# LANL-Bioinformatics/PCRamp

Hardware: AMD Instinct MI355X
Metric: primer-pair x target amplification evals/sec (higher is better)
Workload: dtype u32

## Files before the change

### pcramp_amd/csrc/pcr_device.hip

```cpp
#include <hip/hip_runtime.h>
#include <cstring>
#include <rocprim/device/device_radix_sort.hpp>

#include <stdint.h>
#include <string.h>
#include <math.h>
#include <stdlib.h>
#include <string>
#include <vector>
#include <chrono>
#include <algorithm>
#include <unordered_map>
#include <type_traits>
#include <thread>
#include <mutex>
#include <condition_variable>
#include <functional>
#include <memory>
#include <atomic>
#include <cassert>
#include <sched.h>
#include <pthread.h>

#include "../../include/pcramp_hip.h"
// ... 463 lines not shown
		for(uint32_t j = k >> 1;j > 0;j >>= 1){
			for(uint32_t i = tid;i < np2;i += FINBIG_THREADS){
				const uint32_t l = i ^ j;
				if(l > i){
					const uint64_t a = fin_keys[i], b = fin_keys[l];
					const bool up = ((i & k) == 0);
					if((a > b) == up){ fin_keys[i] = b; fin_keys[l] = a; }
				}
			}
			__syncthreads();
		}
	}
	const uint32_t chunk = (np2 + FINBIG_THREADS - 1)/FINBIG_THREADS;
	const uint32_t lo = min(np2, tid*chunk), hi = min(np2, lo + chunk);
	uint32_t cnt = 0;
	for(uint32_t i = lo;i < hi;++i){
		const uint64_t k = fin_keys[i];
		if(k != ~0ull && (i == 0 || fin_keys[i - 1] != k)) ++cnt;
	}
	part[tid] = cnt;
	__syncthreads();
	if(tid == 0){
		uint32_t run = 0;
		for(int t = 0;t < FINBIG_THREADS;++t){ const uint32_t c = part[t]; part[t] = run; run += c; }
		seg_hi[seq] = seq*cap + run;
	}
	__syncthreads();
	uint32_t rank = part[tid];
	for(uint32_t i = lo;i < hi;++i){
		const uint64_t k = fin_keys[i];
		if(k != ~0ull && (i == 0 || fin_keys[i - 1] != k)){
			DevEntry e;
			materialise_entry(k, planes, blk_off, irr, irr_off, e);
			db[(size_t)seq*cap + rank] = e;
			++rank;
		}
	}
}

#include "pcr_screen.inc"

#include "pcr_sw.inc"
#include "pcr_thermo.inc"

constexpr uint32_t N_TOUCHED_UNKNOWN = 0xFFFFFFFFu;
constexpr uint32_t EPOCH_LIMIT = (1u << 24) - 1;

struct SeqSet {
	uint32_t n = 0;
	std::vector<std::vector<uint8_t> > packed;
	std::vector<uint64_t> len, blk_off, nblk_real;
	std::vector<float> weight; DevBuf<float> d_weight; bool weight_dirty = true;
	std::vector<uint8_t> active;
	std::vector<std::vector<pcrhost::IrrEntry> > irr_host;
	uint64_t total_blocks = 0;
	uint32_t n_tiles = 0, n_irr = 0;
	bool ctrl_clean = false;
	bool touched_from_seg = false;
	uint32_t bucket_cap = 64;
	DevBuf<uint32_t> irr_perm; uint32_t irr_size_count[256];
	DevBuf<uint4> planes;
	DevBuf<uint32_t> valid, nib, tb, blk_seq, tile_seq, tile_pos0, irr_off, degen_tiles;
	uint32_t *valid_d() const { return valid.p + S2_VALID_FRONT; }
	uint32_t *tb_d() const { return tb.p + S2_TB_FRONT; }
	DevBuf<uint8_t> tile_degen; uint32_t n_degen_tiles = 0;
	DevBuf<TileDesc> tile_desc;
	DevBuf<uint64_t> d_len, d_blk_off, d_nblk_real;
	DevBuf<uint8_t> d_active;
	std::vector<uint8_t> has_eos; DevBuf<uint8_t> d_has_eos;
	DevBuf<IrrDev> irr;
	DevBuf<IrrScan> irr_scan;
	DevBuf<uint32_t> irx_first, irx_last, irx_words, irx_sums; bool irx_valid = false, irx_usable = false;
	uint32_t irr_n_multi = 0;
	DevBuf<uint32_t> pix_first, pix_last, pix_sums, blk_info, blk_local, blk_tile0; DevBuf<uint4> pix_ent; std::vector<uint32_t> pix_start_h; uint64_t pix_generation = 0; bool pix_valid = false, pix_usable = false;
	DevBuf<uint8_t> codes; DevBuf<uint64_t> d_code_off; bool have_codes = false;
	bool have_db = false;
	uint32_t n_entries = 0;
	uint32_t db_cap = 0;
	uint64_t n_slots = 0;
	DevBuf<DevEntry> db;
	DevBuf<uint32_t> touched;
	DevBuf<uint32_t> ctrl;
	uint32_t n_touched = 0;
	bool touched_built = false;
	uint32_t *d_seg_hi = nullptr;
};

}

struct HostPool {
	std::vector<std::thread> th;
	std::mutex m; std::condition_variable cv_go, cv_done;
	std::function<void(unsigned)> fn; unsigned n_parts = 0, next = 0, pending = 0; uint64_t gen = 0; bool stop = false;
	explicit HostPool(unsigned n_workers){ for(unsigned i = 0;i < n_workers;++i) th.emplace_back([this]{ work(); }); }
	~HostPool(){ { std::lock_guard<std::mutex> lk(m); stop = true; } cv_go.notify_all(); for(std::thread &t : th) t.join(); }
	unsigned size() const { return (unsigned)th.size(); }
	void work()
	{
		uint64_t seen = 0;
		std::unique_lock<std::mutex> lk(m);
		while(true){
			cv_go.wait(lk, [&]{ return stop || gen != seen; });
			if(stop) return;
			seen = gen;
			while(next < n_parts){ const unsigned p = next++; lk.unlock(); fn(p); lk.lock(); }
			if(--pending == 0) cv_done.notify_one();
		}
	}
	void run(unsigned parts, std::function<void(unsigned)> f)
	{
		std::unique_lock<std::mutex> lk(m);
		fn = std::move(f); n_parts = parts; next = 0; pending = (unsigned)th.size(); ++gen;
		cv_go.notify_all();
		while(next < n_parts){ const unsigned p = next++; lk.unlock(); fn(p); lk.lock(); }
		cv_done.wait(lk, [&]{ return pending == 0; });
	}
};

namespace { struct PassJob; struct Launcher; }

struct ItemBufs {
	DevBuf<uint8_t> *tmp; DevBuf<uint32_t> *cnt; DevBuf<uint64_t> *eoff; DevBuf<uint2> *items;
	DevBuf<uint64_t> *joff; DevBuf<float4> *res; DevBuf<uint2> *item_tm; DevBuf<uint32_t> *flag;
};
struct ItemScratch {
	DevBuf<uint8_t> in, tmp; DevBuf<uint32_t> cnt, flag; DevBuf<uint64_t> eoff, joff, ioff; DevBuf<uint2> items, item_tm; DevBuf<float4> res;
	ItemBufs bufs() { return ItemBufs{&tmp, &cnt, &eoff, &items, &joff, &res, &item_tm, &flag}; }
};

struct pcr_ctx {
	int device = 0;
	std::unique_ptr<HostPool> pool_;
	HostPool &host_pool()
	{
		if(!pool_){ const unsigned hw = std::max(1u, std::thread::hardware_concurrency()); pool_.reset(new HostPool(std::min(hw, 16u) - 1u)); }
		return *pool_;
	}
	Stream stream;
	Stream aux_stream;
	std::string design_text;
	DevBuf<uint64_t> split_where;
	pcr_params params;
	pcrhost::PackFilter filt;
	SeqSet sets[PCR_N_SETS];
	DevBuf<uint32_t> best, counters, mask, status;
	int scan_version = 3;
	bool force_seed1 = false;
	struct S2Key { uint32_t a, c, g, t, floor_; bool operator==(const S2Key &o) const { return a == o.a && c == o.c && g == o.g && t == o.t && floor_ == o.floor_; } };
	struct S2KeyHash { size_t operator()(const S2Key &k) const { uint64_t h = 0x9E3779B97F4A7C15ull; for(uint32_t v : {k.a, k.c, k.g, k.t, k.floor_}){ h ^= v; h *= 0x100000001B3ull; h ^= h >> 29; } return (size_t)h; } };
	struct S2Entry { std::vector<uint32_t> seeds;  uint32_t off_mask; bool seedable; uint4 mask;  };
	std::unordered_map<S2Key, S2Entry, S2KeyHash> s2_cache;
	std::vector<pcrhost::Seed> s2_tmp;
	static constexpr int S3_CHUNK_SETS = 4;
	struct S3Chunks { uint64_t gen = 0; uint32_t total = 0; std::vector<uint32_t> run; };
	struct S3Entry : S2Entry { std::vector<uint8_t> spans;  S3Chunks chunks[S3_CHUNK_SETS]; uint32_t next_slot = 0; };
	std::unordered_map<S2Key, S3Entry, S2KeyHash> s3_cache;
	std::vector<pcrhost::FoldSeed> s3_tmp;
	struct S3Launch { Seed3Slices W; uint32_t n_chunks, per_wg, slice_cap, n_irr_wg; };
	int pair_mode = 1; bool s3_pair_attr_set = false;
	bool no_seed3 = false, s3_attr_set = false;
	bool s3_next = true;
	bool s2_attr_set = false; uint32_t s2_dbg = 0; bool no_irr_index = false;
	std::unordered_map<S2Key, S2Entry, S2KeyHash> s1_cache;
	DevBuf<uint32_t> s1_image, s1_heads, s1_multi, s1_part;
	bool host_seed_tables = false;
	DevBuf<Hit> hits;
	DevBuf<uint64_t> bits_fr, bits_rf;
	DevBuf<OligoDev> oligos;
	DevBuf<SwJob> sw_jobs; DevBuf<SwOut> sw_out; DevBuf<uint8_t> sw_q, sw_qlen, sw_t, entry_codes, entry_lens;
	DevBuf<AmpRec> amp_recs, amp_recs2; DevBuf<BgPairDev> bg_pairs;
	DevBuf<uint64_t> amp_keys; DevBuf<uint32_t> amp_pkeys, amp_pair_start; DevBuf<uint8_t> sort_tmp;
	DevBuf<thermo::Job> th_jobs; DevBuf<thermo::JobOut> th_out; DevBuf<int> th_dg; DevBuf<uint2> th_map; DevBuf<uint32_t> th_bad;
	float th_dg_salt = -1.0f;
	DevBuf<unsigned long long> th_dbg; bool th_attr_set = false;
	std::vector<thermo::Job> th_host_jobs; std::vector<thermo::JobOut> th_host_res;
	MappedBuf<uint8_t> sw_pin; Event sw_done[2];
	DevBuf<pcr_amplicon> mx_amp;
	DevBuf<OligoDev> opt_oligos; DevBuf<uint2> opt_jobs; DevBuf<float> opt_cov; DevBuf<uint32_t> opt_loc, opt_tasks;
	DevBuf<Planes> mx_keys; uint32_t mx_n_keys = 0; DevBuf<uint32_t> mx_count;
	DevBuf<uint8_t> pool_in, pool_tmp; DevBuf<uint32_t> pool_cnt, pool_ord; DevBuf<uint64_t> pool_eoff, pool_ioff, pool_keys; DevBuf<uint2> pool_items; DevBuf<pcr_product> pool_rec;
	DevBuf<uint8_t> site_in, site_tmp; DevBuf<uint32_t> site_cnt, site_ord, site_flag; DevBuf<uint64_t> site_eoff, site_joff, site_keys; DevBuf<uint2> site_items; DevBuf<float4> site_res; DevBuf<pcr_site> site_rec;
	bool site_attr_set = false;
	DevBuf<uint8_t> sv_item; DevBuf<uint32_t> sv_ord, sv_var, sv_start, sv_vord, sv_map; DevBuf<pcr_site_variant> sv_rec; DevBuf<uint64_t> sv_vkeys;
	bool sv_attr_set = false;
	DevBuf<uint4> rp_foot; DevBuf<uint64_t> rp_keys; DevBuf<uint32_t> rp_u32; DevBuf<uint8_t> rp_state; DevBuf<pcr_repair_step> rp_rec;
	pcr_comm *shard_comm = nullptr; uint64_t shard_first = 0, shard_n_total = 0; int shard_mode = 0;
	DevBuf<uint64_t> sh_rec, sh_full; DevBuf<uint8_t> sh_stage;
	std::vector<uint64_t> shard_bounds; DevBuf<uint64_t> d_shard_bounds;
	bool design_ready = false; DevBuf<uint64_t> sh_bits;
	std::vector<std::vector<uint8_t> > samp_packed; std::vector<uint64_t> samp_len;
	void drop_shard(){ shard_comm = nullptr; shard_mode = 0; shard_bounds.clear(); design_ready = false; samp_packed.clear(); samp_len.clear(); }
	pcr_comm *trial_comm = nullptr;
	size_t amp_cap = size_t(1) << 20;
	uint32_t n_cu = 256;
	DevBuf<uint64_t> fin_scratch;
	std::vector<uint16_t> seed_count; std::vector<uint8_t> seed_fill, seed_own;
	uint32_t epoch = 0;
	uint32_t debug_epoch = 0;
	bool opt_pm_global = false;
	uint32_t opt_dbg_wg_tasks = 0, opt_dbg_task_cap = 0;
	uint64_t best_seen = 0;
	static constexpr int STAGE_RING = 4;
	struct StageSlot { MappedBuf<uint8_t> buf; Event done; bool busy = false;
	                   uint32_t guard_seq = 0;  };
	StageSlot stage[STAGE_RING]; int stage_next = 0;
	struct DirectSlot { DevBuf<uint8_t> buf{true}; uint32_t guard_seq = 0; };
	DirectSlot dstage[STAGE_RING]; int dstage_next = 0;
	bool direct_ok = false;
	typedef PassMail Mail;
	static constexpr uint32_t MAIL_RING = 8;
	MappedBuf<Mail> mail;
	uint32_t mail_seq = 0;
	MappedBuf<uint8_t> ret;
	MappedBuf<uint8_t> in;
	MappedBuf<uint32_t> ret_flag; uint32_t ret_seq = 0;
	struct Pending {
		uint32_t seq; int which; std::vector<pcr_pair> pairs; int opt5, opt3; float thr; uint32_t min_len;
		pcr_amplify_args args; uint64_t *d_fr, *d_rf;
	};
	std::vector<Pending> pending;
	bool launch_thread = true;
	Launcher *launcher = nullptr; pcrq::Client lq_client; uint64_t n_pipelined = 0;
	std::mutex job_m; std::vector<PassJob *> job_free, job_all;
	DevBuf<uint8_t> arena;
	const uint4 *d_cand_fwd = nullptr, *d_cand_rc = nullptr; const uint32_t *d_cand_floor = nullptr;
	const OligoDev *d_oligos = nullptr;
	bool debug_log = false;
	bool timing = false; double t_host[8] = {0, 0, 0, 0, 0, 0, 0, 0}; uint64_t n_timed = 0;
	bool prof = false; uint32_t prof_stride = 1, prof_pass = 0;
	std::vector<std::pair<Event, Event> > prof_events;
	double prof_ms = 0.0; uint64_t prof_launches = 0;
	std::vector<std::pair<Event, Event> > prof_events_k[PCR_PROF_KERNELS];
	double prof_ms_k[PCR_PROF_KERNELS] = {0.0, 0.0, 0.0}; uint64_t prof_launches_k[PCR_PROF_KERNELS] = {0, 0, 0};
	DevBuf<uint8_t> pdim_in, pdim_tmp; DevBuf<float4> pdim_res; DevBuf<pcr_pool_dimer> pdim_rec, pdim_out; DevBuf<uint32_t> pdim_keep, pdim_off, pdim_flag;
	bool pdim_attr_set = false;
	DevBuf<uint32_t> ptm_ord; DevBuf<uint64_t> ptm_keys, ptm_bits; DevBuf<pcr_product_tm> ptm_rec;
	DevBuf<uint32_t> pph_hcnt, pph_ord; DevBuf<uint64_t> pph_hoff, pph_keys, pph_bits; DevBuf<uint4> pph_prod; DevBuf<pcr_probe_hit> pph_rec;
	DevBuf<uint4> pam_iv, pam_stat; DevBuf<uint32_t> pam_u32; DevBuf<uint64_t> pam_u64; DevBuf<pcr_amplicon_info> pam_info; DevBuf<uint8_t> pam_tmp, pam_packed;
	uint32_t bg_max_pairs = 0;
	uint32_t amp_dbg_hash_bits = 0;
	DevBuf<uint4> ppc_iv; DevBuf<uint32_t> ppc_pos, ppc_u32; DevBuf<uint64_t> ppc_u64; DevBuf<pcr_probe_candidate> ppc_rec; DevBuf<uint8_t> ppc_tmp;
	DevBuf<uint32_t> anp_pairseq; DevBuf<uint64_t> anp_out; DevBuf<float> anp_melt;
	DevBuf<uint8_t> pcf_din; DevBuf<uint32_t> pcf_vals, pcf_ucell, pcf_dkeep, pcf_keep, pcf_koff;
	DevBuf<uint64_t> pcf_aoff, pcf_keys; DevBuf<float4> pcf_dres;
	DevBuf<uint4> pcf_uagg, pcf_dense; DevBuf<pcr_pool_dimer> pcf_drec; DevBuf<float> pcf_dmat; DevBuf<pcr_pool_conflict> pcf_rec, pcf_out;
	ItemScratch shared;
	DevBuf<uint2> pe3_end; DevBuf<uint32_t> pe3_before, pe3_ord; DevBuf<uint64_t> pe3_sum, pe3_keys, pe3_bits; DevBuf<uint8_t> pe3_tmp;
	DevBuf<pcr_product_end3> pe3_rec;
};

namespace {

int drain(pcr_ctx *ctx);
int flush_launcher(pcr_ctx *ctx);
void detach_launcher(pcr_ctx *ctx);
void free_jobs(pcr_ctx *ctx);

struct ProfScope {
	pcr_ctx *ctx; int k; Event e0, e1;
	ProfScope(pcr_ctx *c, int kernel, bool on = true) : ctx(c), k(kernel)
	{
		if(!on || !ctx->prof || k < 0 || k >= PCR_PROF_KERNELS) return;
		if(e0.create() != hipSuccess || e1.create() != hipSuccess){ e0.release(); return; }
		(void)hipEventRecord(e0, ctx->stream);
	}
	void finish()
	{
		if(!e0) return;
		(void)hipEventRecord(e1, ctx->stream);
		((k == PCR_PROF_SCAN) ? ctx->prof_events : ctx->prof_events_k[k]).emplace_back(std::move(e0), std::move(e1));
	}
	~ProfScope() { finish(); }
};
constexpr int PCR_SET_SCRATCH = 3;
inline bool set_ok(pcr_set which) { return (unsigned)which <= (unsigned)PCR_SET_MULTIPLEX; }
#define CHECK_SET(which) do{ if(!set_ok(which)){ g_err = "unknown sequence set (PCR_SET_TARGET, PCR_SET_BACKGROUND or PCR_SET_MULTIPLEX)"; return PCR_ERR_ARG; } }while(0)
#define FLUSH(ctx) do{ if((ctx)->launcher){ const int frc_ = flush_launcher(ctx); if(frc_ != PCR_OK) return frc_; } }while(0)
#define DRAIN(ctx) do{ FLUSH(ctx); if(!(ctx)->pending.empty()){ const int drc_ = drain(ctx); if(drc_ != PCR_OK) return drc_; } }while(0)

struct HostTimer {
	pcr_ctx *ctx; int slot; std::chrono::steady_clock::time_point t0;
	HostTimer(pcr_ctx *c, int s) : ctx(c), slot(s) { if(ctx->timing) t0 = std::chrono::steady_clock::now(); }
	void next(int s)
	{
		if(!ctx->timing) return;
		const auto t1 = std::chrono::steady_clock::now();
		ctx->t_host[slot] += std::chrono::duration<double, std::micro>(t1 - t0).count();
		slot = s; t0 = t1;
	}
	~HostTimer() { next(slot); }
};

__global__ void k_apply_splits(const uint64_t *__restrict__ where, uint32_t n, uint32_t *__restrict__ planes , uint32_t *__restrict__ nib)
{
	const uint32_t i = blockIdx.x*blockDim.x + threadIdx.x;
	if(i >= n) return;
	const uint64_t gb = where[2*(size_t)i];
	const uint32_t bit = (uint32_t)where[2*(size_t)i + 1];
	const uint32_t m = ~(1u << bit);
	for(int k = 0;k < 4;++k) atomicAnd(&planes[gb*4 + k], m);
	atomicAnd(&nib[gb*4 + (bit >> 3)], ~(0xFu << ((bit & 7u)*4u)));
}

int upload_irregular(pcr_ctx *ctx, SeqSet &S)
{
	const auto tu0 = std::chrono::steady_clock::now();
	auto ms_since = [&](){ return std::chrono::duration<double, std::milli>(std::chrono::steady_clock::now() - tu0).count(); };
	double t_flat = 0, t_sort = 0, t_scan = 0, t_copy1 = 0;
	size_t total = 0;
	for(uint32_t s = 0;s < S.n;++s) total += S.irr_host[s].size();
	std::vector<IrrDev> flat(total);
	std::vector<uint32_t> off(S.n + 1, 0);
	for(int k = 0;k < 256;++k) S.irr_size_count[k] = 0;
	{
		size_t at = 0;
		for(uint32_t s = 0;s < S.n;++s){
			off[s] = (uint32_t)at;
			const std::vector<pcrhost::IrrEntry> &v = S.irr_host[s];
			for(size_t k = 0;k < v.size();++k){
				const pcrhost::IrrEntry &e = v[k];
				IrrDev &d = flat[at++];
				d.w = e.w; d.loc = e.loc; d.seq = s;
				d.meta = (uint32_t)e.strand | ((uint32_t)e.cws << 8) | ((uint32_t)e.ord << 16);
				d.local_id = (uint32_t)k;
				++S.irr_size_count[e.cws & 0xFF];
			}
		}
	}
	off[S.n] = (uint32_t)flat.size();
	S.n_irr = (uint32_t)flat.size();
	t_flat = ms_since();
	std::vector<uint32_t> perm(flat.size());
	t_sort = ms_since();
	int rc;
	{
		auto spread = [](uint64_t v) -> uint64_t {
			v = (v | (v << 16)) & 0x0000FFFF0000FFFFull; v = (v | (v << 8)) & 0x00FF00FF00FF00FFull; v = (v | (v << 4)) & 0x0F0F0F0F0F0F0F0Full;
			v = (v | (v << 2)) & 0x3333333333333333ull; v = (v | (v << 1)) & 0x5555555555555555ull; return v;
		};
		uint32_t start[256];
		uint32_t run = 0;
		for(int k = 255;k >= 0;--k){ start[k] = run; run += S.irr_size_count[k]; }
		std::vector<IrrScan> scan(perm.size());
		uint32_t n_multi = 0;
		for(size_t i = 0;i < flat.size();++i){
			const IrrDev &d = flat[i];
			const uint32_t at = start[(d.meta >> 8) & 0xFF]++;
			perm[at] = (uint32_t)i;
			const uint32_t multi = (d.w.a & d.w.c) | (d.w.a & d.w.g) | (d.w.a & d.w.t) | (d.w.c & d.w.g) | (d.w.c & d.w.t) | (d.w.g & d.w.t);
			if(multi) ++n_multi;
			const uint32_t lo = d.w.c | d.w.t, hi = d.w.g | d.w.t;
			const uint64_t code = spread(lo) | (spread(hi) << 1);
			IrrScan r; r.w0 = (uint32_t)code; r.w1 = (uint32_t)(code >> 32); r.idx_flags = (uint32_t)i | (multi ? 0x80000000u : 0u); r.seq = d.seq;
			scan[at] = r;
		}
		S.irr_n_multi = n_multi; S.irx_valid = false;
		t_scan = ms_since();
		if((rc = S.irr_scan.ensure_slack(scan.size() + 1)) != PCR_OK) return rc;
		if(!scan.empty()) HIP_TRY(hipMemcpy(S.irr_scan.p, scan.data(), scan.size()*sizeof(IrrScan), hipMemcpyHostToDevice));
	}
	t_copy1 = ms_since();
	if((rc = S.irr_perm.ensure_slack(perm.size() + 1)) != PCR_OK) return rc;
	if(!perm.empty()) HIP_TRY(hipMemcpyAsync(S.irr_perm.p, perm.data(), perm.size()*sizeof(uint32_t), hipMemcpyHostToDevice, ctx->stream));
	if((rc = S.irr.ensure_slack(flat.size())) != PCR_OK) return rc;
	if((rc = S.irr_off.ensure(off.size())) != PCR_OK) return rc;
	if(!flat.empty()) HIP_TRY(hipMemcpyAsync(S.irr.p, flat.data(), flat.size()*sizeof(IrrDev), hipMemcpyHostToDevice, ctx->stream));
	HIP_TRY(hipMemcpyAsync(S.irr_off.p, off.data(), off.size()*sizeof(uint32_t), hipMemcpyHostToDevice, ctx->stream));
	HIP_TRY(hipStreamSynchronize(ctx->stream));
	if(ctx->timing && flat.size() > 100000) fprintf(stderr, "[pcramp] irregular list of %zu words: flat %.1f  order %.1f  scan records %.1f  first copy %.1f  other copies %.1f ms\n", flat.size(), t_flat, t_sort - t_flat, t_scan - t_sort, t_copy1 - t_scan, ms_since() - t_copy1);
	return PCR_OK;
}

void launch_exclusive_scan(pcr_ctx *ctx, uint32_t *counts, uint32_t *starts, uint32_t n, uint32_t *sums)
{
	const uint32_t n_blocks = (n + 4095u)/4096u;
	hipLaunchKernelGGL(k_scan_blocks, dim3(n_blocks), dim3(1024), 0, ctx->stream, counts, starts, n, sums);
	hipLaunchKernelGGL(k_scan_sums, dim3(1), dim3(1024), 0, ctx->stream, sums, n_blocks);
	hipLaunchKernelGGL(k_scan_add, dim3(n_blocks), dim3(1024), 0, ctx->stream, starts, counts, n, sums);
}

constexpr uint32_t IRX_MAX_RUN = 1024;
int ensure_irr_index(pcr_ctx *ctx, SeqSet &S)
{
	if(S.irx_valid) return PCR_OK;
	int rc;
	if((rc = S.irx_first.ensure(IRX_KEYS + 4)) != PCR_OK) return rc;
	if((rc = S.irx_last.ensure(IRX_KEYS + 4)) != PCR_OK) return rc;
	if((rc = S.irx_words.ensure_slack((size_t)24*S.n_irr + 4)) != PCR_OK) return rc;
	const uint32_t n_blocks = (IRX_KEYS + 4095u)/4096u;
	if((rc = S.irx_sums.ensure(n_blocks + 4)) != PCR_OK) return rc;
	HIP_TRY(hipMemsetAsync(S.irx_last.p, 0, (size_t)IRX_KEYS*sizeof(uint32_t), ctx->stream));
	if(S.n_irr){
		hipLaunchKernelGGL(k_irx_count, dim3((S.n_irr + 255)/256), dim3(256), 0, ctx->stream, S.irr.p, S.n_irr, S.irx_last.p);
		HIP_TRY(hipGetLastError());
	}
	{
		uint32_t longest = 0;
		HIP_TRY(hipMemsetAsync(S.irx_sums.p + n_blocks, 0, sizeof(uint32_t), ctx->stream));
		hipLaunchKernelGGL(k_irx_max, dim3(256), dim3(256), 0, ctx->stream, S.irx_last.p, IRX_KEYS, S.irx_sums.p + n_blocks);
		HIP_TRY(hipMemcpyAsync(&longest, S.irx_sums.p + n_blocks, sizeof(uint32_t), hipMemcpyDeviceToHost, ctx->stream));
		HIP_TRY(hipStreamSynchronize(ctx->stream));
		S.irx_usable = longest <= IRX_MAX_RUN;
		if(!S.irx_usable){ S.irx_valid = true; return PCR_OK; }
	}
	launch_exclusive_scan(ctx, S.irx_last.p, S.irx_first.p, IRX_KEYS, S.irx_sums.p);
	HIP_TRY(hipGetLastError());
	if(S.n_irr){
		hipLaunchKernelGGL(k_irx_scatter, dim3((S.n_irr + 255)/256), dim3(256), 0, ctx->stream, S.irr.p, S.n_irr, S.irx_last.p, S.irx_words.p);
		HIP_TRY(hipGetLastError());
	}
	S.irx_valid = true;
	return PCR_OK;
}

int ensure_pos_index(pcr_ctx *ctx, SeqSet &S)
{
	if(S.pix_valid) return PCR_OK;
	S.pix_valid = true; S.pix_usable = false;
	if(S.total_blocks == 0 || S.total_blocks*32 >= (uint64_t(1) << 32) - 64) return PCR_OK;
	int rc;
	if((rc = S.pix_first.ensure(PIX_KEYS + 4)) != PCR_OK) return rc;
	if((rc = S.pix_last.ensure(PIX_KEYS + 4)) != PCR_OK) return rc;
	const uint32_t n_blocks = (PIX_KEYS + 4095u)/4096u;
	if((rc = S.pix_sums.ensure(n_blocks + 4)) != PCR_OK) return rc;
	if((rc = S.pix_ent.ensure(S.total_blocks*32 + 64)) != PCR_OK) return rc;
	{
		if(S.n >= (1u << 30)){ return PCR_OK; }
		if((rc = S.blk_info.ensure(S.total_blocks + 1)) != PCR_OK) return rc;
		if((rc = S.blk_local.ensure(S.total_blocks + 1)) != PCR_OK) return rc;
		std::vector<uint32_t> tile0((size_t)S.n + 1);
		uint64_t t0 = 0;
		for(uint32_t q = 0;q < S.n;++q){ tile0[q] = (uint32_t)t0; t0 += (S.len[q] >= 32) ? (S.len[q] - 7 + TILE_POS - 1)/TILE_POS : 0; }
		tile0[S.n] = (uint32_t)t0;
		if(t0 >= (uint64_t(1) << 32)) return PCR_OK;
		if((rc = S.blk_tile0.ensure((size_t)S.n + 1)) != PCR_OK) return rc;
		HIP_TRY(hipMemcpyAsync(S.blk_tile0.p, tile0.data(), ((size_t)S.n + 1)*sizeof(uint32_t), hipMemcpyHostToDevice, ctx->stream));
		hipLaunchKernelGGL(k_blk_info, dim3((unsigned)((S.total_blocks + 255)/256)), dim3(256), 0, ctx->stream, S.blk_seq.p, S.d_blk_off.p, S.d_len.p,
			S.blk_tile0.p, S.tile_degen.p, S.d_active.p, S.total_blocks, S.blk_info.p, S.blk_local.p);
		HIP_TRY(hipGetLastError());
		HIP_TRY(hipStreamSynchronize(ctx->stream));
	}
	HIP_TRY(hipMemsetAsync(S.pix_last.p, 0, (size_t)PIX_KEYS*sizeof(uint32_t), ctx->stream));
	const unsigned grid = (unsigned)((S.total_blocks + 255)/256);
// ... 255 lines not shown
	HIP_TRY(hipMemcpyAsync(&n, S.ctrl.p + 3, sizeof(uint32_t), hipMemcpyDeviceToHost, ctx->stream));
	HIP_TRY(hipStreamSynchronize(ctx->stream));
	S.n_touched = n; S.n_entries = n ? 1 : 0; S.touched_built = true;
	return PCR_OK;
}

int amplify_launch(pcr_ctx *ctx, SeqSet &S, const pcr_pair *pairs, uint32_t n_pairs, const pcr_amplify_args *a,
	uint64_t *d_fr, uint64_t *d_rf, const FusedAmp *fa = nullptr)
{
	{ const int erc = ensure_touched(ctx, S); if(erc != PCR_OK) return erc; }
	if(!S.have_db){ g_err = "pcr_amplify: no word DB (call pcr_select_words first)"; return PCR_ERR_STATE; }
	const uint64_t words = (S.n + 63)/64;
	const size_t bits_bytes = (size_t)n_pairs*words*sizeof(uint64_t);
	if(S.n_entries == 0 || n_pairs == 0){
		if(bits_bytes){
			HIP_TRY(hipMemsetAsync(d_fr, 0, bits_bytes, ctx->stream));
			HIP_TRY(hipMemsetAsync(d_rf, 0, bits_bytes, ctx->stream));
		}
		return PCR_OK;
	}
	HostTimer timer(ctx, 4);
	int rc;
	const bool prestaged = fa && fa->staged;
	if(prestaged) ctx->d_oligos = fa->d_oligos;
	else{
		std::vector<OligoDev> ol;
		build_oligos(pairs, n_pairs, a, ol);
		Stager st(ctx);
		if((rc = st.begin(ol.size()*sizeof(OligoDev) + 64)) != PCR_OK) return rc;
		ctx->d_oligos = st.put(ol.data(), ol.size());
		const bool vec_ok = ((uintptr_t)d_fr % 16 == 0) && ((uintptr_t)d_rf % 16 == 0) && (bits_bytes % 16 == 0);
		if(!vec_ok){
			HIP_TRY(hipMemsetAsync(d_fr, 0, bits_bytes, ctx->stream));
			HIP_TRY(hipMemsetAsync(d_rf, 0, bits_bytes, ctx->stream));
		}
		if((rc = vec_ok ? st.ship(d_fr, bits_bytes, d_rf, bits_bytes) : st.ship()) != PCR_OK) return rc;
	}
	timer.next(5);
	const uint32_t mask_words = (2*n_pairs + 31)/32;
	if((rc = ctx->mask.ensure((size_t)S.n_slots*mask_words)) != PCR_OK) return rc;
	if((rc = ctx->status.ensure(1)) != PCR_OK) return rc;
	const bool dev_n = S.n_touched == N_TOUCHED_UNKNOWN;
	const uint32_t *n_dev = dev_n ? S.ctrl.p + 3 : nullptr;
	const uint32_t n_t = dev_n ? 0u : S.n_touched, n_db = n_t*S.db_cap;
	const unsigned threads = dev_n ? 256 : 128;
	const unsigned grid = dev_n ? (unsigned)std::min<uint64_t>(((uint64_t)S.n*S.db_cap + threads - 1)/threads, 1024) : (n_db + threads - 1)/threads;
	const unsigned mgrid = dev_n ? std::min<unsigned>((S.n + MATCH_WAVES - 1)/MATCH_WAVES, 1024u) : (n_t + MATCH_WAVES - 1)/MATCH_WAVES;
	hipLaunchKernelGGL(k_match, dim3(std::max(mgrid, 1u)), dim3(64*MATCH_WAVES), 0, ctx->stream, S.db.p, n_t, n_dev, S.db_cap,
		S.touched.p, S.d_seg_hi, ctx->d_oligos, 2*n_pairs, mask_words, ctx->mask.p, ctx->status.p,
		prestaged ? fa->pub_counters : (const uint32_t *)nullptr, prestaged ? ctx->mail.dev + (fa->pub_seq % pcr_ctx::MAIL_RING) : (pcr_ctx::Mail *)nullptr,
		prestaged ? fa->pub_seq : 0u);
	HIP_TRY(hipGetLastError());
	hipLaunchKernelGGL(k_pair, dim3(grid), dim3(threads), 0, ctx->stream, S.db.p, n_db, n_dev, S.db_cap, S.touched.p, S.d_seg_hi, ctx->mask.p,
		mask_words, ctx->d_oligos, n_pairs, S.planes.p, S.d_blk_off.p, S.d_len.p, S.d_active.p, a->amp_min, a->amp_max,
		a->ident_threshold, a->use_taq_mama, d_fr, d_rf, words, ctx->status.p);
	HIP_TRY(hipGetLastError());
	return PCR_OK;
}

template<int NSLOT, int KLO>
int launch_scan2_nw(pcr_ctx *ctx, SeqSet &S, uint32_t nw, uint32_t group0, uint32_t n_groups, uint32_t gw, uint32_t ncand, const HitSink &sink,
	const uint32_t *d_tab, const uint32_t *d_bias, const uint32_t *tile_ids, uint32_t n_tiles, const uint32_t *orient_ids)
{
#define SCAN2_ARGS S.nib.p, S.planes.p, S.valid_d(), S.d_blk_off.p, S.d_len.p, S.d_active.p, S.tile_seq.p, S.tile_pos0.p, \
	d_tab, d_bias, group0, gw, tile_ids, orient_ids, ctx->d_cand_fwd, ctx->d_cand_rc, ctx->d_cand_floor, ncand, sink
	const dim3 grid(n_tiles, n_groups), block(SCAN2_THREADS);
	switch(nw){
		case 1: hipLaunchKernelGGL((k_scan2<1, NSLOT, KLO>), grid, block, 0, ctx->stream, SCAN2_ARGS); break;
		case 2: hipLaunchKernelGGL((k_scan2<2, NSLOT, KLO>), grid, block, 0, ctx->stream, SCAN2_ARGS); break;
		case 3: hipLaunchKernelGGL((k_scan2<3, NSLOT, KLO>), grid, block, 0, ctx->stream, SCAN2_ARGS); break;
		case 4: hipLaunchKernelGGL((k_scan2<4, NSLOT, KLO>), grid, block, 0, ctx->stream, SCAN2_ARGS); break;
		case 5: hipLaunchKernelGGL((k_scan2<5, NSLOT, KLO>), grid, block, 0, ctx->stream, SCAN2_ARGS); break;
		case 6: hipLaunchKernelGGL((k_scan2<6, NSLOT, KLO>), grid, block, 0, ctx->stream, SCAN2_ARGS); break;
		case 7: hipLaunchKernelGGL((k_scan2<7, NSLOT, KLO>), grid, block, 0, ctx->stream, SCAN2_ARGS); break;
		default: hipLaunchKernelGGL((k_scan2<8, NSLOT, KLO>), grid, block, 0, ctx->stream, SCAN2_ARGS); break;
	}
#undef SCAN2_ARGS
	HIP_TRY(hipGetLastError());
	return PCR_OK;
}

int launch_scan2(pcr_ctx *ctx, SeqSet &S, const Scan2Tables &T, uint32_t ncand, const HitSink &sink,
	const uint32_t *d_tab, const uint32_t *d_bias, const uint32_t *tile_ids, uint32_t n_tiles, const uint32_t *orient_ids)
{
	if(n_tiles == 0 || T.n_groups == 0) return PCR_OK;
	const uint32_t full = (T.last_words == T.gw) ? T.n_groups : T.n_groups - 1;
	int rc = PCR_OK;
	if(full){
		rc = (T.nslot == 26) ? launch_scan2_nw<26, 3>(ctx, S, T.gw, 0, full, T.gw, ncand, sink, d_tab, d_bias, tile_ids, n_tiles, orient_ids)
			: launch_scan2_nw<32, 0>(ctx, S, T.gw, 0, full, T.gw, ncand, sink, d_tab, d_bias, tile_ids, n_tiles, orient_ids);
		if(rc != PCR_OK) return rc;
	}
	if(full < T.n_groups){
		rc = (T.nslot == 26) ? launch_scan2_nw<26, 3>(ctx, S, T.last_words, full, 1, T.gw, ncand, sink, d_tab, d_bias, tile_ids, n_tiles, orient_ids)
			: launch_scan2_nw<32, 0>(ctx, S, T.last_words, full, 1, T.gw, ncand, sink, d_tab, d_bias, tile_ids, n_tiles, orient_ids);
	}
	return rc;
}

int count_entries(pcr_ctx *ctx, SeqSet &S)
{
	uint64_t total = 0;
	if(S.n_touched){
		std::vector<uint32_t> hi(S.n);
		HIP_TRY(hipMemcpyAsync(hi.data(), S.d_seg_hi, S.n*sizeof(uint32_t), hipMemcpyDeviceToHost, ctx->stream));
		HIP_TRY(hipStreamSynchronize(ctx->stream));
		for(uint32_t q = 0;q < S.n;++q){ if(hi[q]) total += hi[q] - (uint64_t)q*S.db_cap; }
	}
	S.n_entries = (uint32_t)total;
	return PCR_OK;
}

}

extern "C" {

const char *pcr_last_error(void) { return g_err.c_str(); }

pcr_ctx *pcr_create(int device, void *hip_stream, const pcr_params *params)
{
	int count = 0;
	if(hipGetDeviceCount(&count) != hipSuccess || count <= 0){
		g_err = "pcr_create: no HIP device available (this library has no CPU fallback)";
		return nullptr;
	}
	if(device < 0 || device >= count){ g_err = "pcr_create: bad device index"; return nullptr; }
	if(hipSetDevice(device) != hipSuccess){ g_err = "pcr_create: hipSetDevice failed"; return nullptr; }
	hipDeviceProp_t prop;
	if(hipGetDeviceProperties(&prop, device) != hipSuccess){ g_err = "pcr_create: hipGetDeviceProperties failed"; return nullptr; }
	if(std::string(prop.gcnArchName).find("gfx950") == std::string::npos){
		g_err = std::string("pcr_create: device is ") + prop.gcnArchName + ", this build targets gfx950 only";
		return nullptr;
	}
	pcr_ctx *ctx = new pcr_ctx();
	ctx->device = device;
	if(hip_stream) ctx->stream.borrow((hipStream_t)hip_stream);
	else if(ctx->stream.create() != hipSuccess){ g_err = "pcr_create: hipStreamCreate failed"; delete ctx; return nullptr; }
	if(params){ ctx->params = *params; }
	else{ ctx->params.pack_max_degen = 256; ctx->params.pack_min_gc = 0.0f; ctx->params.pack_max_gc = 1.0f; }
	{ hipDeviceProp_t prop; if(hipGetDeviceProperties(&prop, device) == hipSuccess && prop.multiProcessorCount > 0) ctx->n_cu = (uint32_t)prop.multiProcessorCount; }
	if(const char *v = getenv("PCRAMP_TIMING")) ctx->timing = v[0] == '1';
	ctx->debug_log = getenv("PCRAMP_DEBUG") != nullptr;
	if(const char *v = getenv("PCRAMP_DEBUG_EPOCH")) ctx->debug_epoch = (uint32_t)strtoul(v, nullptr, 0);
	if(const char *v = getenv("PCRAMP_OPT_PM")) ctx->opt_pm_global = v[0] == 'g';
	if(const char *v = getenv("PCRAMP_DEBUG_OPT_TASKS")){ unsigned a = 0, b = 0; if(sscanf(v, "%u,%u", &a, &b) >= 1){ ctx->opt_dbg_wg_tasks = a; ctx->opt_dbg_task_cap = b; } }
	if(const char *v = getenv("PCRAMP_DEBUG_AMP_HASH_BITS")) ctx->amp_dbg_hash_bits = (uint32_t)strtoul(v, nullptr, 0);
	if(const char *v = getenv("PCRAMP_DEBUG_AMP_CAP")) ctx->amp_cap = std::max<size_t>(16, (size_t)strtoull(v, nullptr, 0));
	if(const char *v = getenv("PCRAMP_SEED")) ctx->force_seed1 = v[0] == '1';
	if(const char *v = getenv("PCRAMP_SEED_TABLES")) ctx->host_seed_tables = v[0] == 'h';
	if(const char *v = getenv("PCRAMP_S2DBG")) ctx->s2_dbg = (uint32_t)atoi(v);
	if(const char *v = getenv("PCRAMP_IRR_INDEX")) ctx->no_irr_index = v[0] == '0';
	if(const char *v = getenv("PCRAMP_SEED3")) ctx->no_seed3 = v[0] == '0';
	if(const char *v = getenv("PCRAMP_S3_NEXT")) ctx->s3_next = v[0] != '0';
	if(const char *v = getenv("PCRAMP_LAUNCH_THREAD")) ctx->launch_thread = v[0] != '0';
	if(const char *v = getenv("PCRAMP_PAIR")) ctx->pair_mode = (v[0] == '0') ? 0 : (strcmp(v, "force") == 0) ? 2 : 1;
	if(const char *v = getenv("PCRAMP_SCAN")){ if(v[0] == '1') ctx->scan_version = 1; else if(v[0] == '2') ctx->scan_version = 2; }
	{
		const char *v = getenv("PCRAMP_STAGE");
		if(!(v && v[0] == 'k') && prop.isLargeBar){
			DevBuf<uint32_t> probe(true); MappedBuf<uint32_t> back; const std::string err_before = g_err;
			constexpr uint32_t PROBE_WORDS = 1024;
			if(probe.ensure(PROBE_WORDS) == PCR_OK && back.ensure(PROBE_WORDS*sizeof(uint32_t)) == PCR_OK){
				hipPointerAttribute_t at;
				bool ok = hipPointerGetAttributes(&at, probe.p) == hipSuccess;
				for(int round = 0;ok && round < 2;++round){
					volatile uint32_t *w = (volatile uint32_t *)probe.p;
					for(uint32_t i = 0;i < PROBE_WORDS;++i){ w[i] = 0x9E3779B9u*(i + 1) + (uint32_t)round; back.host[i] = 0; }
					__builtin_ia32_sfence();
					hipLaunchKernelGGL(k_stage, dim3(1), dim3(256), 0, ctx->stream, (const uint4 *)probe.p, (uint4 *)back.dev, PROBE_WORDS/4,
						(uint4 *)nullptr, 0u, (uint4 *)nullptr, 0u, (uint4 *)nullptr, 0u);
					ok = hipGetLastError() == hipSuccess && hipStreamSynchronize(ctx->stream) == hipSuccess;
					for(uint32_t i = 0;ok && i < PROBE_WORDS;++i) ok = back.host[i] == 0x9E3779B9u*(i + 1) + (uint32_t)round;
				}
				ctx->direct_ok = ok;
			}
			else{ (void)hipGetLastError(); g_err = err_before; }
		}
	}
	ctx->filt.max_degen = ctx->params.pack_max_degen;
	ctx->filt.set_gc(ctx->params.pack_min_gc, ctx->params.pack_max_gc);
	if(hipMemcpyToSymbol(HIP_SYMBOL(c_taq_mama), h_taq_mama, sizeof(h_taq_mama)) != hipSuccess ||
	   hipMemcpyToSymbol(HIP_SYMBOL(thermo::c_H), PCR_NN_H, sizeof(PCR_NN_H)) != hipSuccess ||
	   hipMemcpyToSymbol(HIP_SYMBOL(thermo::c_S), PCR_NN_S, sizeof(PCR_NN_S)) != hipSuccess ||
	   hipMemcpyToSymbol(HIP_SYMBOL(thermo::c_loop_S), PCR_LOOP_S, sizeof(PCR_LOOP_S)) != hipSuccess ||
	   hipMemcpyToSymbol(HIP_SYMBOL(thermo::c_bulge_S), PCR_BULGE_S, sizeof(PCR_BULGE_S)) != hipSuccess ||
	   hipMemcpyToSymbol(HIP_SYMBOL(thermo::c_hairpin_S), PCR_HAIRPIN_S, sizeof(PCR_HAIRPIN_S)) != hipSuccess ||
	   hipMemcpyToSymbol(HIP_SYMBOL(thermo::c_special_H), PCR_SPECIAL_H, sizeof(PCR_SPECIAL_H)) != hipSuccess ||
	   hipMemcpyToSymbol(HIP_SYMBOL(thermo::c_special_S), PCR_SPECIAL_S, sizeof(PCR_SPECIAL_S)) != hipSuccess ||
	   hipMemcpyToSymbol(HIP_SYMBOL(thermo::c_special_key), PCR_SPECIAL_KEY, sizeof(PCR_SPECIAL_KEY)) != hipSuccess ||
	   hipMemcpyToSymbol(HIP_SYMBOL(thermo::c_wc), PCR_WC, sizeof(PCR_WC)) != hipSuccess){
		g_err = "pcr_create: hipMemcpyToSymbol failed"; delete ctx; return nullptr;
	}
	if(ctx->mail.ensure(sizeof(pcr_ctx::Mail)*pcr_ctx::MAIL_RING) != PCR_OK){ g_err = "pcr_create: mapped host allocation failed"; delete ctx; return nullptr; }
	memset((void *)ctx->mail.host, 0, sizeof(pcr_ctx::Mail)*pcr_ctx::MAIL_RING);
	return ctx;
}

void pcr_destroy(pcr_ctx *ctx)
{
	if(!ctx) return;
	(void)hipSetDevice(ctx->device);
	(void)flush_launcher(ctx);
	detach_launcher(ctx);
	(void)hipStreamSynchronize(ctx->stream);
	if(ctx->aux_stream) (void)hipStreamSynchronize(ctx->aux_stream);
	ctx->pending.clear();
	free_jobs(ctx);
	if(ctx->timing && ctx->n_timed){
		const double n = (double)ctx->n_timed;
		fprintf(stderr, "[pcramp] host us/pass by stage: A (plan, caller's thread) %.1f  B (stage + launch, %s) %.1f  (%llu of %llu passes pipelined, queue depth <= %u)\n",
			ctx->t_host[0]/n, ctx->n_pipelined ? "launcher thread" : "caller's thread", (ctx->t_host[1] + ctx->t_host[2])/n,
			(unsigned long long)ctx->n_pipelined, (unsigned long long)ctx->n_timed, ctx->lq_client.max_depth);
		fprintf(stderr, "[pcramp] host us/pass: plan %.1f  stage %.1f  launch %.1f  wait %.1f | amplify prep %.1f  launch %.1f  (%llu passes)\n",
			ctx->t_host[0]/n, ctx->t_host[1]/n, ctx->t_host[2]/n, ctx->t_host[3]/n, ctx->t_host[4]/n, ctx->t_host[5]/n, (unsigned long long)ctx->n_timed);
	}
	delete ctx;
}

uint32_t pcr_num_sequences(pcr_ctx *ctx, pcr_set which) { return (ctx && set_ok(which)) ? ctx->sets[which].n : 0; }
uint64_t pcr_bitset_words(pcr_ctx *ctx, pcr_set which) { return (ctx && set_ok(which)) ? (ctx->sets[which].n + 63)/64 : 0; }

int pcr_staging_mode(pcr_ctx *ctx) { return (ctx && ctx->direct_ok) ? 1 : 0; }

int pcr_launcher_stats(pcr_ctx *ctx, uint64_t *passes_pipelined, uint32_t *max_queue_depth)
{
	if(!ctx){ g_err = "null ctx"; return PCR_ERR_ARG; }
	if(passes_pipelined) *passes_pipelined = ctx->n_pipelined;
	if(max_queue_depth) *max_queue_depth = ctx->lq_client.max_depth;
	return PCR_OK;
}

int pcr_live_resources(uint64_t out[4])
{
	if(!out){ g_err = "pcr_live_resources: bad argument"; return PCR_ERR_ARG; }
	for(int k = 0;k < 4;++k) out[k] = pcrown::g_live[k].load();
	return PCR_OK;
}

int pcr_synchronize(pcr_ctx *ctx)
{
	if(!ctx){ g_err = "null ctx"; return PCR_ERR_ARG; }
	HIP_TRY(hipSetDevice(ctx->device));
	DRAIN(ctx);
	HIP_TRY(hipStreamSynchronize(ctx->stream));
	return PCR_OK;
}

static int load_sequences_impl(pcr_ctx *ctx, int which, const uint8_t *packed4, const uint64_t *byte_offsets,
	const uint64_t *lengths, const float *weights, uint32_t n);

int pcr_load_sequences(pcr_ctx *ctx, pcr_set which, const uint8_t *packed4, const uint64_t *byte_offsets,
	const uint64_t *lengths, const float *weights, uint32_t n)
{
	if(!set_ok(which)){ g_err = "pcr_load_sequences: unknown sequence set"; return PCR_ERR_ARG; }
	return load_sequences_impl(ctx, (int)which, packed4, byte_offsets, lengths, weights, n);
}

static int load_sequences_impl(pcr_ctx *ctx, int which, const uint8_t *packed4, const uint64_t *byte_offsets,
	const uint64_t *lengths, const float *weights, uint32_t n)
{
	if(!ctx || which < 0 || which >= PCR_N_SETS || (n && (!packed4 || !byte_offsets || !lengths))){
		g_err = "pcr_load_sequences: bad argument"; return PCR_ERR_ARG;
	}
	DRAIN(ctx);
	if(n >= (1u << 24)){ g_err = "pcr_load_sequences: at most 2^24-1 sequences per GPU shard"; return PCR_ERR_CAPACITY; }
	HIP_TRY(hipSetDevice(ctx->device));
	HIP_TRY(hipStreamSynchronize(ctx->stream));
	SeqSet &S = ctx->sets[which];
	S.have_db = false; S.n_entries = 0; S.have_codes = false;
	S.n = n;
	S.packed.assign(n, std::vector<uint8_t>());
	S.len.assign(lengths, lengths + n);
	if(which == PCR_SET_TARGET) ctx->drop_shard();
	if(which == PCR_SET_TARGET || which == PCR_SET_BACKGROUND) ctx->trial_comm = nullptr;
	S.weight.assign(n, 1.0f);
	if(weights) S.weight.assign(weights, weights + n);
	S.weight_dirty = true;
	S.ctrl_clean = false; S.touched_from_seg = false;
	S.active.assign(n, 1);
	S.has_eos.assign(n, 0);
	S.blk_off.assign(n + 1, 0);
	S.nblk_real.assign(n, 0);
	S.irr_host.assign(n, std::vector<pcrhost::IrrEntry>());
	uint64_t total_bytes = 0, total_blocks = 0, n_tiles = 0;
	std::vector<uint64_t> dev_byte_off(n);
	for(uint32_t s = 0;s < n;++s){
		if(lengths[s] >= (uint64_t(1) << 31)){ g_err = "pcr_load_sequences: sequence longer than 2^31-1 bases"; return PCR_ERR_CAPACITY; }
		const uint64_t nb = (lengths[s] + 1)/2;
		S.packed[s].assign(packed4 + byte_offsets[s], packed4 + byte_offsets[s] + nb);
		if((lengths[s] & 1) && nb) S.packed[s][nb - 1] &= 0xF0;
		{
			const std::vector<uint8_t> &b = S.packed[s];
			bool eos = false;
			const uint64_t full = lengths[s]/2;
			for(uint64_t k = 0;k < full && !eos;++k) eos = ((b[k] & 0xF0) == 0) || ((b[k] & 0x0F) == 0);
			if(!eos && (lengths[s] & 1)) eos = ((b[full] & 0xF0) == 0);
			S.has_eos[s] = eos ? 1 : 0;
		}
		dev_byte_off[s] = total_bytes;
		total_bytes += nb;
		S.blk_off[s] = total_blocks;
		S.nblk_real[s] = (lengths[s] + 31)/32;
		total_blocks += S.nblk_real[s] + 2;
		if(lengths[s] >= 32) n_tiles += (lengths[s] - 7 + TILE_POS - 1)/TILE_POS;
	}
	S.blk_off[n] = total_blocks;
	S.total_blocks = total_blocks;
	if(n_tiles >= (uint64_t(1) << 31)){ g_err = "pcr_load_sequences: too many tiles"; return PCR_ERR_CAPACITY; }
	S.n_tiles = (uint32_t)n_tiles;

	std::vector<uint32_t> blk_seq(total_blocks), tile_seq(n_tiles), tile_pos0(n_tiles);
	uint64_t t = 0;
	S.pix_valid = false; S.pix_usable = false;
	for(uint32_t s = 0;s < n;++s){
		for(uint64_t b = S.blk_off[s];b < S.blk_off[s + 1];++b) blk_seq[b] = s;
		if(lengths[s] >= 32){
			const uint64_t nt = (lengths[s] - 7 + TILE_POS - 1)/TILE_POS;
			for(uint64_t k = 0;k < nt;++k, ++t){ tile_seq[t] = s; tile_pos0[t] = (uint32_t)(k*TILE_POS); }
		}
		pcrhost::PackedSeq q; q.buf = S.packed[s].data(); q.len = lengths[s];
		if(!pcrhost::irregular_words(q, ctx->filt, S.irr_host[s])){
			g_err = "pcr_load_sequences: more than 64 irregular words share one (loc, strand)"; return PCR_ERR_CAPACITY;
		}
	}

	int rc;
	DevBuf<uint8_t> d_packed; DevBuf<uint64_t> d_byte_off;
	if((rc = d_packed.ensure(total_bytes)) != PCR_OK) return rc;
	if((rc = d_byte_off.ensure(n)) != PCR_OK) return rc;
	if((rc = S.planes.ensure(total_blocks)) != PCR_OK) return rc;
	if((rc = S.valid.ensure(S2_VALID_FRONT + total_blocks + S2_TAIL_BLOCKS)) != PCR_OK) return rc;
	if((rc = S.nib.ensure(total_blocks*4 + 8)) != PCR_OK) return rc;
	if((rc = S.tb.ensure(S2_TB_FRONT + (total_blocks + S2_TAIL_BLOCKS)*2 + 8)) != PCR_OK) return rc;
	if((rc = S.tile_degen.ensure(n_tiles + 1)) != PCR_OK) return rc;
	if((rc = S.degen_tiles.ensure(n_tiles + 1)) != PCR_OK) return rc;
	if((rc = S.blk_seq.ensure(total_blocks)) != PCR_OK) return rc;
	if((rc = S.tile_seq.ensure(n_tiles)) != PCR_OK) return rc;
	if((rc = S.tile_pos0.ensure(n_tiles)) != PCR_OK) return rc;
	if((rc = S.d_len.ensure(n)) != PCR_OK) return rc;
	if((rc = S.d_blk_off.ensure(n + 1)) != PCR_OK) return rc;
	if((rc = S.d_nblk_real.ensure(n)) != PCR_OK) return rc;
	if((rc = S.d_active.ensure(n)) != PCR_OK) return rc;
	if((rc = S.d_has_eos.ensure(n)) != PCR_OK) return rc;
#define H2D(dst, src, bytes) do{ if((bytes) > 0){ hipError_t e_ = hipMemcpy(dst, src, bytes, hipMemcpyHostToDevice); \
	if(e_ != hipSuccess){ g_err = std::string("hipMemcpy: ") + hipGetErrorString(e_); return PCR_ERR_DEVICE; } } }while(0)
	{
		std::vector<uint8_t> flat(total_bytes);
		for(uint32_t s = 0;s < n;++s){ if(!S.packed[s].empty()) memcpy(flat.data() + dev_byte_off[s], S.packed[s].data(), S.packed[s].size()); }
		H2D(d_packed.p, flat.data(), flat.size());
	}
	H2D(d_byte_off.p, dev_byte_off.data(), n*sizeof(uint64_t));
	H2D(S.blk_seq.p, blk_seq.data(), total_blocks*sizeof(uint32_t));
	H2D(S.tile_seq.p, tile_seq.data(), n_tiles*sizeof(uint32_t));
	H2D(S.tile_pos0.p, tile_pos0.data(), n_tiles*sizeof(uint32_t));
	H2D(S.d_len.p, S.len.data(), n*sizeof(uint64_t));
	H2D(S.d_blk_off.p, S.blk_off.data(), (n + 1)*sizeof(uint64_t));
	H2D(S.d_nblk_real.p, S.nblk_real.data(), n*sizeof(uint64_t));
	H2D(S.d_active.p, S.active.data(), n);
	H2D(S.d_has_eos.p, S.has_eos.data(), n);
#undef H2D
	{
		hipError_t e_ = hipMemsetAsync(S.valid.p, 0, S2_VALID_FRONT*sizeof(uint32_t), ctx->stream);
		if(e_ == hipSuccess) e_ = hipMemsetAsync(S.valid_d() + total_blocks, 0, S2_TAIL_BLOCKS*sizeof(uint32_t), ctx->stream);
		if(e_ == hipSuccess) e_ = hipMemsetAsync(S.tb.p, 0, S2_TB_FRONT*sizeof(uint32_t), ctx->stream);
		if(e_ == hipSuccess) e_ = hipMemsetAsync(S.tb_d() + total_blocks*2, 0, (S2_TAIL_BLOCKS*2 + 8)*sizeof(uint32_t), ctx->stream);
		if(e_ != hipSuccess){ g_err = std::string("load: padding memset: ") + hipGetErrorString(e_); return PCR_ERR_DEVICE; }
	}
// ... 444 lines not shown
```

### pcramp_amd/csrc/pcr_host.hpp

```cpp
#ifndef PCR_HOST_HPP
#define PCR_HOST_HPP

#include <stdint.h>
#include <algorithm>
#include <deque>
#include <vector>

namespace pcrhost {

struct Planes {
	uint32_t a, c, g, t;
};

inline uint32_t bitrev32(uint32_t v)
{
	v = ((v >> 1) & 0x55555555u) | ((v & 0x55555555u) << 1);
	v = ((v >> 2) & 0x33333333u) | ((v & 0x33333333u) << 2);
	v = ((v >> 4) & 0x0F0F0F0Fu) | ((v & 0x0F0F0F0Fu) << 4);
	v = ((v >> 8) & 0x00FF00FFu) | ((v & 0x00FF00FFu) << 8);
	return (v >> 16) | (v << 16);
}

inline unsigned word_get(const uint64_t w[2], int k) { return (unsigned)(w[k >> 4] >> ((15 - (k & 15))*4)) & 0xF; }

// ... 524 lines not shown
	}
};

inline bool orientation_seeds(const Planes &m, uint32_t floor_, uint32_t orient, std::vector<Seed> &out, int *max_exact_pos = nullptr, int Q = SEED_Q)
{
	if(max_exact_pos) *max_exact_pos = -1;
	const uint32_t occ = m.a | m.c | m.g | m.t;
	const int size = __builtin_popcount(occ);
	if(size == 0 || floor_ == 0 || floor_ > (uint32_t)size) return floor_ > (uint32_t)size;
	const int k = size - (int)floor_;
	const int first = __builtin_ctz(occ);
	if((occ >> first) != ((size == 32) ? 0xFFFFFFFFu : ((1u << size) - 1u))) return false;
	unsigned slot_set[32];
	for(int j = 0;j < first;++j) slot_set[j] = 0;
	for(int j = first;j < first + size;++j) slot_set[j] = planes_nibble(m, j);
	for(int j = first + size;j < 32;++j) slot_set[j] = 0;

	auto window = [&](int pos, int len, unsigned *sets) -> int {
		const int ws = std::min(pos, 32 - Q);
		for(int j = 0;j < Q;++j){ const int sl = ws + j; sets[j] = (sl >= pos && sl < pos + len) ? slot_set[sl] : 15u; }
		return ws;
	};
	SeedLayout best = { 0, 0, 0, 0 }; bool have = false; unsigned best_codes = 0;
	for(int n2 = 0;3*(n2 - 1) < k + 1;++n2){
		for(int n1 = 0;3*n2 + 2*(n1 - 1) < k + 1;++n1){
			const int n0 = std::max(0, k + 1 - 3*n2 - 2*n1);
			if(n0 + n1 + n2 == 0) continue;
			for(int n1s = 0;n1s <= n1;++n1s){
				const int rest = size - Q*(n1 - n1s) - (Q - 1)*n1s - Q*n2;
				if(rest < 0 || (n0 > 0 && rest/n0 < MIN_SEED_BLOCK)) continue;
				const SeedLayout lay = { n0, n1, n1s, n2 };
				unsigned codes = 0;
				lay.each(first, size, Q, [&](int pos, int len, int budget){
					unsigned sets[SEED_Q_MAX];
					window(pos, len, sets);
					if(codes <= MAX_SEED_CODES) codes += seed_block_codes(sets, Q, budget);
				});
				if(codes > MAX_SEED_CODES) continue;
				if(!have || codes < best_codes){ have = true; best = lay; best_codes = codes; }
			}
		}
	}
	if(!have) return false;
	best.each(first, size, Q, [&](int pos, int len, int budget){
		unsigned sets[SEED_Q_MAX];
		const int ws = window(pos, len, sets);
		seed_emit_block(sets, Q, orient, (uint32_t)ws, budget, out);
		if(len < Q && max_exact_pos) *max_exact_pos = std::max(*max_exact_pos, pos);
	});
	return true;
}

struct FoldSeed { uint32_t code; uint8_t off, lo, hi; };

inline unsigned seed_block_fold_cost(const unsigned *sets, int budget, unsigned &n_seeds)
{
	unsigned d[9], n[3] = { 1, 0, 0 };
	for(int j = 0;j < 9;++j){ d[j] = (unsigned)__builtin_popcount(sets[j]); n[0] *= d[j]; }
	if(n[0] == 0 || sets[9] == 0){ n_seeds = 0; return 0; }
	if(budget >= 1){
		for(int j = 0;j < 9;++j){
			if(d[j] == 4) continue;
			const unsigned cj = n[0]/d[j]*(4 - d[j]);
			n[1] += cj;
			if(budget >= 2){ for(int i = j + 1;i < 9;++i){ if(d[i] < 4) n[2] += cj/d[i]*(4 - d[i]); } }
		}
	}
	const unsigned last = sets[9];
	const unsigned span = (unsigned)(32 - __builtin_clz(last)) - (unsigned)__builtin_ctz(last);
	unsigned cost = 0; n_seeds = 0;
	for(int m = 0;m <= budget;++m){ n_seeds += n[m]; cost += n[m]*((m < budget && last != 15u) ? 4u : span); }
	return cost;
}

inline void fold_seeds(const std::vector<Seed> &q10, std::vector<FoldSeed> &out)
{
	std::vector<uint32_t> key(q10.size());
	for(size_t i = 0;i < q10.size();++i) key[i] = ((uint32_t)q10[i].off << 20) | ((q10[i].code & 0x3FFFFu) << 2) | (q10[i].code >> 18);
	std::sort(key.begin(), key.end());
	for(size_t i = 0;i < key.size();){
		unsigned set = 0; size_t j = i;
		for(;j < key.size() && (key[j] >> 2) == (key[i] >> 2);++j) set |= 1u << (key[j] & 3u);
		FoldSeed f; f.code = (key[i] >> 2) & 0x3FFFFu; f.off = (uint8_t)(key[i] >> 20);
		f.lo = (uint8_t)__builtin_ctz(set); f.hi = (uint8_t)(31 - __builtin_clz(set));
		out.push_back(f);
		i = j;
	}
}

inline bool orientation_fold_seeds(const Planes &m, uint32_t floor_, std::vector<FoldSeed> &out, std::vector<Seed> &tmp, unsigned *cost4 = nullptr)
{
	const int Q = 10;
	if(cost4) *cost4 = 0;
	const uint32_t occ = m.a | m.c | m.g | m.t;
	const int size = __builtin_popcount(occ);
	if(size == 0 || floor_ == 0 || floor_ > (uint32_t)size) return floor_ > (uint32_t)size;
	const int k = size - (int)floor_, first = __builtin_ctz(occ);
	if(size < Q || (occ >> first) != ((size == 32) ? 0xFFFFFFFFu : ((1u << size) - 1u))) return false;
	unsigned slot_set[32];
	for(int j = 0;j < 32;++j) slot_set[j] = (j >= first && j < first + size) ? planes_nibble(m, j) : 0u;
	auto window = [&](int pos, int len, unsigned *sets) -> int {
		const int ws = std::min(pos, 32 - Q);
		for(int j = 0;j < Q;++j){ const int sl = ws + j; sets[j] = (sl >= pos && sl < pos + len) ? slot_set[sl] : 15u; }
		return ws;
	};
	SeedLayout best = { 0, 0, 0, 0 }; bool have = false; unsigned best_cost = 0;
	for(int n2 = 0;3*(n2 - 1) < k + 1;++n2){
		for(int n1 = 0;3*n2 + 2*(n1 - 1) < k + 1;++n1){
			const int n0 = std::max(0, k + 1 - 3*n2 - 2*n1);
			if(n0 + n1 + n2 == 0) continue;
			for(int n1s = 0;n1s <= n1;++n1s){
				const int rest = size - Q*(n1 - n1s) - (Q - 1)*n1s - Q*n2;
				if(rest < 0 || (n0 > 0 && rest/n0 < MIN_SEED_BLOCK)) continue;
				const SeedLayout lay = { n0, n1, n1s, n2 };
				unsigned seeds = 0, cost = 0;
				lay.each(first, size, Q, [&](int pos, int len, int budget){
					unsigned sets[SEED_Q_MAX], ns = 0;
					window(pos, len, sets);
					if(seeds <= MAX_SEED_CODES){ cost += seed_block_fold_cost(sets, budget, ns); seeds += ns; }
				});
				if(seeds > MAX_SEED_CODES) continue;
				if(!have || cost < best_cost){ have = true; best = lay; best_cost = cost; }
			}
		}
	}
	if(!have) return false;
	tmp.clear();
	best.each(first, size, Q, [&](int pos, int len, int budget){
		unsigned sets[SEED_Q_MAX];
		const int ws = window(pos, len, sets);
		seed_emit_block(sets, Q, 0, (uint32_t)ws, budget, tmp);
	});
	fold_seeds(tmp, out);
	if(cost4) *cost4 = best_cost;
	return true;
}

inline bool orientation_index_seeds(const Planes &m, uint32_t floor_, bool fold, std::vector<FoldSeed> &out, std::vector<Seed> &tmp, unsigned *cost4 = nullptr)
{
	tmp.clear();
	if(!orientation_seeds(m, floor_, 0, tmp, nullptr, 9)) return false;
	const size_t at = out.size();
	const unsigned plain_cost = 4u*(unsigned)tmp.size();
	for(const Seed &sd : tmp){ FoldSeed f; f.code = sd.code; f.off = sd.off; f.lo = 0; f.hi = 3; out.push_back(f); }
	if(cost4) *cost4 = plain_cost;
	if(!fold || tmp.empty()) return true;
	std::vector<FoldSeed> folded; unsigned c4 = 0;
	if(orientation_fold_seeds(m, floor_, folded, tmp, &c4) && c4 < plain_cost){
		out.resize(at);
		out.insert(out.end(), folded.begin(), folded.end());
		if(cost4) *cost4 = c4;
	}
	return true;
}

inline bool move_trials(const Planes &cur, int move, double max_degen, int primer_min, int primer_max, std::vector<Planes> &out)
{
	const int first = planes_start(cur), last = planes_stop(cur), len = planes_size(cur);
	auto with_nibble = [](Planes w, int k, unsigned v){
		const uint32_t bit = 1u << k;
		w.a = (w.a & ~bit) | ((v & 1u) ? bit : 0u); w.c = (w.c & ~bit) | ((v & 2u) ? bit : 0u);
		w.g = (w.g & ~bit) | ((v & 4u) ? bit : 0u); w.t = (w.t & ~bit) | ((v & 8u) ? bit : 0u);
		return w;
	};
	switch(move){
		case 0:
			if(planes_degeneracy(cur) >= max_degen) return true;
			for(int i = first;i <= last;++i){
				const unsigned c = planes_nibble(cur, i);
				for(unsigned b = 1;b <= 8;b <<= 1){
					if(c & b) continue;
					const Planes w = with_nibble(cur, i, c | b);
					if(planes_degeneracy(w) > max_degen) continue;
					out.push_back(w);
				}
			}
			return true;
		case 1:
			for(int i = first;i <= last;++i){
				const unsigned c = planes_nibble(cur, i);
				for(unsigned b = 1;b <= 8;b <<= 1){
					const unsigned d = c & ~b;
					if(!d || d == c) continue;
					out.push_back(with_nibble(cur, i, d));
				}
			}
			return true;
		case 2: if(len != primer_min){ out.push_back(first < 32 ? with_nibble(cur, first, 0) : cur); } return true;
		case 3: if(len != primer_min){ out.push_back(last >= 0 ? with_nibble(cur, last, 0) : cur); } return true;
		case 4:
			if(len == primer_max) return true;
			for(unsigned b = 1;b <= 8;b <<= 1) out.push_back(first - 1 >= 0 && first < 32 ? with_nibble(cur, first - 1, b) : cur);
			return true;
		case 5:
			if(len == primer_max) return true;
			for(unsigned b = 1;b <= 8;b <<= 1) out.push_back(last + 1 < 32 ? with_nibble(cur, last + 1, b) : cur);
			return true;
		default: return false;
	}
}

}
#endif
```

### pcramp_amd/csrc/pcr_scan_seed3.inc

```

constexpr uint32_t PIX_CODES = 1u << 18;
constexpr uint32_t PIX_KEYS = PIX_CODES << 2;
constexpr uint32_t S3_BATCH = 8;

template<bool SCATTER>
__global__ void k_pix_build(const uint32_t *__restrict__ tb, const uint32_t *__restrict__ blk_seq, const uint64_t *__restrict__ blk_off,
	const uint64_t *__restrict__ len, uint64_t total_blocks, uint32_t *__restrict__ count_or_cursor, uint4 *__restrict__ ent)
{
	const uint64_t b = (uint64_t)blockIdx.x*blockDim.x + threadIdx.x;
	if(b >= total_blocks) return;
	const uint32_t seq = blk_seq[b];
	const int64_t p0 = (int64_t)(b - blk_off[seq])*32, L = (int64_t)len[seq];
	uint32_t w[8];
#pragma unroll
	for(int k = 0;k < 8;++k) w[k] = tb[(int64_t)2*(int64_t)b - 2 + k];
#pragma unroll
	for(int i = 0;i < 32;++i){
		if(p0 + i + 9 > L) break;
		const uint32_t ten = (i < 16) ? funnel(w[2], w[3], 2*i) : funnel(w[3], w[4], 2*(i - 16));
		const uint32_t code = ((ten & S2_CODE_MASK) << 2) | ((ten >> 18) & 3u);
		if(SCATTER){
			const uint32_t at = atomicAdd(&count_or_cursor[code], 1u);
			const int jl = (i + 9) >> 4, sl = 2*((i + 9) & 15);
			const int jr = (i + 41) >> 4, sr = 2*((i + 41) & 15);
			const uint32_t l_lo = funnel(w[jl], w[jl + 1], sl), l_hi = funnel(w[jl + 1], w[jl + 2], sl) & 0x3FFFu;
			const uint32_t r_lo = funnel(w[jr], w[jr + 1], sr), r_hi = funnel(w[jr + 1], w[jr + 2], sr) & 0x3FFFu;
			ent[at] = make_uint4((uint32_t)(b*32 + (uint64_t)i), l_lo, l_hi | (r_lo << 14), (r_lo >> 18) | (r_hi << 14));
		}
		else atomicAdd(&count_or_cursor[code], 1u);
	}
}

struct Seed3Tables {
	const uint32_t *seeds;
	const uint32_t *chunk_prefix;
	const uint8_t *spans;
	const uint4 *masks; const uint8_t *floors;
	uint32_t n_seeds, n_or, or_base;
	const uint32_t *pix_first, *pix_last; const uint4 *pix_ent;
	uint32_t n_chunks, per_wg, slice_cap;
	uint32_t n_irr_wg;
};
constexpr uint32_t S3_MAX_WG = 512;
constexpr uint32_t S3_MAX_OR = 448, S3_MAX_SEEDS = 1u << 16;
struct Seed3Slices { uint32_t start[S3_MAX_WG + 1]; };
struct Seed3Set {
	const uint32_t *valid, *blk_info, *blk_local; const uint8_t *active;
};
constexpr uint32_t BLK_SEQ_MASK = 0x3FFFFFFFu, BLK_INACTIVE = 0x40000000u, BLK_DEGEN = 0x80000000u;

__global__ void k_blk_info(const uint32_t *__restrict__ blk_seq, const uint64_t *__restrict__ blk_off, const uint64_t *__restrict__ len,
	const uint32_t *__restrict__ tile0, const uint8_t *__restrict__ tile_degen, const uint8_t *__restrict__ active, uint64_t total_blocks,
	uint32_t *__restrict__ blk_info, uint32_t *__restrict__ blk_local)
{
	const uint64_t b = (uint64_t)blockIdx.x*blockDim.x + threadIdx.x;
	if(b >= total_blocks) return;
	const uint32_t q = blk_seq[b];
	const uint64_t bl = b - blk_off[q], tile = bl >> 5;
	const uint32_t nt = tile0[q + 1] - tile0[q];
	const bool degen = tile < nt && tile_degen[tile0[q] + tile];
	blk_info[b] = q | (degen ? 0x80000000u : 0u) | (active[q] ? 0u : 0x40000000u);
	blk_local[b] = (uint32_t)bl;
}

__global__ void k_blk_active(uint32_t *__restrict__ blk_info, const uint32_t *__restrict__ blk_seq, const uint8_t *__restrict__ active, uint64_t total_blocks)
{
	const uint64_t b = (uint64_t)blockIdx.x*blockDim.x + threadIdx.x;
	if(b >= total_blocks) return;
	const uint32_t v = blk_info[b] & ~BLK_INACTIVE;
	blk_info[b] = v | (active[blk_seq[b]] ? 0u : BLK_INACTIVE);
}

__device__ __forceinline__ void s3_irregular(const Seed3Tables &T3, const Seed3Set &Q, const IrrArgs2 &IA, const uint4 *__restrict__ cand_fwd,
	const uint32_t *__restrict__ cand_floor, HitSink sink, uint32_t gw, uint32_t n_gw, uint32_t lane)
{
	for(uint32_t i0 = gw*16u;i0 < T3.n_seeds;i0 += n_gw*16u){
		const uint32_t i = i0 + lane;
		const uint32_t sdv = (lane < 16u && i < T3.n_seeds) ? T3.seeds[i] : S2_END;
		const uint32_t orient = T3.or_base + (sdv & 0x1FFu);
		uint32_t first = 0, cnt = 0;
		if(sdv != S2_END && !(orient & 1u)){
			const uint32_t key = (((sdv >> 9) & 31u) << 18) | (sdv >> 14);
			first = IA.ix_first[key]; cnt = IA.ix_last[key] - first;
		}
		const uint32_t incl = s2_scan(cnt);
		const uint32_t total = s2_rl(incl, 63);
		for(uint32_t t0 = 0;t0 < total;t0 += 64u){
			const uint32_t t = t0 + lane;
			uint32_t lo = 0;
#pragma unroll
			for(uint32_t stp = 32u;stp;stp >>= 1){ if((uint32_t)__shfl((int)incl, (int)(lo + stp - 1u)) <= t) lo += stp; }
			const int sl = (int)min(lo, 63u);
			const uint32_t s_incl = (uint32_t)__shfl((int)incl, sl), s_cnt = (uint32_t)__shfl((int)cnt, sl), s_first = (uint32_t)__shfl((int)first, sl);
			const uint32_t c = (uint32_t)__shfl((int)orient, sl) >> 1;
			if(t >= total) continue;
			const IrrDev e = IA.irr[IA.ix_words[s_first + (t - (s_incl - s_cnt))]];
			if(((e.meta >> 8) & 0xFFu) < IA.min_cws || !Q.active[e.seq]) continue;
			const uint32_t n = match_count(e.w.a, e.w.c, e.w.g, e.w.t, cand_fwd[c]);
			if(n >= cand_floor[c]) record_hit(sink, e.seq, c, make_key(e.seq, e.loc, e.meta & 0xFF, 1, (e.meta >> 16) & 0xFF), n);
		}
	}
}

template<uint32_t S3_THREADS>
__global__ __launch_bounds__(S3_THREADS) __attribute__((amdgpu_waves_per_eu(8, 8))) void k_seed3(Seed3Tables T3, Seed3Set Q, IrrArgs2 IA, const uint4 *__restrict__ cand_fwd, const uint32_t *__restrict__ cand_floor,
	HitSink sink, S2Clear Z, Seed3Slices W)
{
#include "pcr_scan_seed3_pass.inc"
}

struct Seed3Row {
	Seed3Tables T3; Seed3Set Q; IrrArgs2 IA; const uint4 *cand_fwd; const uint32_t *cand_floor; HitSink sink; S2Clear Z;
};
struct Seed3HalfSlices { uint32_t start[S3_MAX_WG/2 + 1]; };
template<uint32_t S3_THREADS>
__global__ __launch_bounds__(S3_THREADS) __attribute__((amdgpu_waves_per_eu(8, 8))) void k_seed3_pair(Seed3Row A, Seed3HalfSlices WA, Seed3Row B, Seed3HalfSlices WB)
{
	if(blockIdx.y == 0){
		const Seed3Tables &T3 = A.T3; const Seed3Set &Q = A.Q; const IrrArgs2 &IA = A.IA; const uint4 *const cand_fwd = A.cand_fwd; const uint32_t *const cand_floor = A.cand_floor;
		const HitSink &sink = A.sink; const S2Clear &Z = A.Z; const Seed3HalfSlices &W = WA;
#include "pcr_scan_seed3_pass.inc"
	}
	else{
		const Seed3Tables &T3 = B.T3; const Seed3Set &Q = B.Q; const IrrArgs2 &IA = B.IA; const uint4 *const cand_fwd = B.cand_fwd; const uint32_t *const cand_floor = B.cand_floor;
		const HitSink &sink = B.sink; const S2Clear &Z = B.Z; const Seed3HalfSlices &W = WB;
#include "pcr_scan_seed3_pass.inc"
	}
}
```

### pcramp_amd/csrc/pcr_scan_seed3_pass.inc

```
	extern __shared__ uint4 s3_dyn[];
	uint4 *const masks = s3_dyn;
	uint32_t *const prefix = (uint32_t *)(masks + T3.n_or);
	uint32_t *const seeds = prefix + T3.slice_cap;
	uint8_t *const floors = (uint8_t *)(seeds + T3.slice_cap);
	uint8_t *const spans = floors + ((T3.n_or + 15u) & ~15u);
	const uint32_t wave = (uint32_t)__builtin_amdgcn_readfirstlane((int)(threadIdx.x >> 6)), lane = threadIdx.x & 63u;
	for(uint32_t i = blockIdx.x*S3_THREADS + threadIdx.x;i < Z.n0;i += gridDim.x*S3_THREADS) Z.z0[i] = make_uint4(0, 0, 0, 0);
	for(uint32_t i = blockIdx.x*S3_THREADS + threadIdx.x;i < Z.n1;i += gridDim.x*S3_THREADS) Z.z1[i] = make_uint4(0, 0, 0, 0);
	if(Z.ctrl && blockIdx.x == 0 && threadIdx.x == 0){ Z.ctrl[1] = 0; Z.ctrl[3] = 0; }
	for(uint32_t i = threadIdx.x;i < T3.n_or;i += S3_THREADS){ masks[i] = T3.masks[i]; floors[i] = T3.floors[i]; }
	constexpr uint32_t S3_WAVES = S3_THREADS/64;
	if(blockIdx.x < T3.n_irr_wg){
		if(IA.ix_first) s3_irregular(T3, Q, IA, cand_fwd, cand_floor, sink, blockIdx.x*S3_WAVES + wave, T3.n_irr_wg*S3_WAVES, lane);
		return;
	}
	const uint32_t wg = blockIdx.x - T3.n_irr_wg, n_wg = gridDim.x - T3.n_irr_wg;
	const uint32_t s_lo = W.start[wg];
	const uint32_t n_slice = min(min(W.start[wg + 1] + 2u, T3.n_seeds + 1u) - s_lo, T3.slice_cap);
	for(uint32_t i = threadIdx.x;i < n_slice;i += S3_THREADS){ prefix[i] = T3.chunk_prefix[s_lo + i]; const bool in = s_lo + i < T3.n_seeds; seeds[i] = in ? T3.seeds[s_lo + i] : 0u; spans[i] = in ? T3.spans[s_lo + i] : (uint8_t)0; }
	__syncthreads();
	const uint32_t gw = wg*S3_WAVES + wave, n_gw = n_wg*S3_WAVES;
	const uint32_t q_lo = wg*T3.per_wg, q_hi = min(q_lo + T3.per_wg, T3.n_chunks);
	for(uint32_t q0 = q_lo + wave;q0 < q_hi;q0 += S3_WAVES*S3_BATCH){
		uint32_t c_first = 0, c_cnt = 0, c_sd = 0;
		{
			const uint32_t q = q0 + lane*S3_WAVES;
			if(lane < S3_BATCH && q < q_hi){
				uint32_t lo = 0, hi = n_slice - 1u;
				while(hi - lo > 1u){ const uint32_t mid = (lo + hi) >> 1; if(prefix[mid] <= q) lo = mid; else hi = mid; }
				c_sd = seeds[lo];
				const uint32_t key = (c_sd >> 14) << 2, sp = spans[lo];
				const uint32_t f = T3.pix_first[key + (sp & 3u)], e = T3.pix_last[key + (sp >> 2)], j0 = (q - prefix[lo])*64u;
				c_first = f + j0; c_cnt = (e - f) - j0;
			}
		}
		uint4 en[S3_BATCH];
#pragma unroll
		for(int b = 0;b < (int)S3_BATCH;++b){
			const uint32_t first = s2_rl(c_first, b), cnt = s2_rl(c_cnt, b);
			en[b] = make_uint4(0xFFFFFFFFu, 0, 0, 0);
			if(lane < cnt) en[b] = T3.pix_ent[first + lane];
		}
		uint32_t cnt_b[S3_BATCH], g[S3_BATCH]; bool pass_b[S3_BATCH];
#pragma unroll
		for(int b = 0;b < (int)S3_BATCH;++b){
			const uint32_t sdv = s2_rl(c_sd, b);
			const uint32_t off = (sdv >> 9) & 31u, local = sdv & 0x1FFu, code = sdv >> 14;
			g[b] = en[b].x;
			const uint32_t r_lo = funnel(en[b].z, en[b].w, 14);
			const uint4 cx = make_uint4(en[b].y << 2, (funnel(en[b].y, en[b].z, 30) & 0xFFFFu) | (code << 16), (code >> 16) | (r_lo << 2), en[b].w >> 12);
			const uint32_t in = 24u - off, sh = 2u*(in & 15u);
			const uint32_t a0 = (in < 16u) ? funnel(cx.x, cx.y, sh) : funnel(cx.y, cx.z, sh);
			const uint32_t a1 = (in < 16u) ? funnel(cx.y, cx.z, sh) : funnel(cx.z, cx.w, sh);
			cnt_b[b] = (uint32_t)__popc(s2_mux(a0, a1, masks[local]));
			pass_b[b] = g[b] != 0xFFFFFFFFu && cnt_b[b] >= floors[local] && g[b] >= off;
		}
		uint32_t vw[S3_BATCH], info[S3_BATCH], bl[S3_BATCH];
#pragma unroll
		for(int b = 0;b < (int)S3_BATCH;++b){
			vw[b] = 0; info[b] = 0; bl[b] = 0;
			if(pass_b[b]){
				const uint32_t ws = g[b] - ((s2_rl(c_sd, b) >> 9) & 31u);
				vw[b] = Q.valid[ws >> 5]; info[b] = Q.blk_info[ws >> 5]; bl[b] = Q.blk_local[ws >> 5];
			}
		}
#pragma unroll
		for(int b = 0;b < (int)S3_BATCH;++b){
			if(!pass_b[b]) continue;
			const uint32_t sdv = s2_rl(c_sd, b);
			const uint32_t ws = g[b] - ((sdv >> 9) & 31u), seq = info[b] & BLK_SEQ_MASK;
			if(!((vw[b] >> (ws & 31u)) & 1u) || (info[b] & (BLK_DEGEN | BLK_INACTIVE))) continue;
			const uint32_t p_local = bl[b]*32u + (ws & 31u);
			const uint32_t orient = T3.or_base + (sdv & 0x1FFu), c = orient >> 1;
			if(orient & 1u) record_hit(sink, seq, c, make_key(seq, (int32_t)p_local + 31, 2, 0, 0), cnt_b[b]);
			else record_hit(sink, seq, c, make_key(seq, (int32_t)p_local, 1, 0, 0), cnt_b[b]);
		}
	}
	if(IA.ix_first && T3.n_irr_wg == 0) s3_irregular(T3, Q, IA, cand_fwd, cand_floor, sink, gw, n_gw, lane);
```

### pcramp_amd/csrc/pcr_select.inc

```
namespace {

struct PlanLists {
	std::vector<uint32_t> s2_seeds; std::vector<uint4> s2_masks; std::vector<uint8_t> s2_floors;
	std::vector<uint32_t> s2_group_end, s2_group_offmask, s2_group_or, s2_group_nor;
	std::vector<pcr_ctx::S3Launch> s3_launch;
	std::vector<uint32_t> s3_prefix;
	std::vector<uint8_t> s3_spans;
	std::vector<uint32_t> s1_seeds;
	void clear()
	{
		s2_seeds.clear(); s2_masks.clear(); s2_floors.clear(); s2_group_end.clear(); s2_group_offmask.clear(); s2_group_or.clear(); s2_group_nor.clear();
		s3_launch.clear(); s3_prefix.clear(); s3_spans.clear(); s1_seeds.clear();
	}
};

inline uint32_t spread16(uint32_t v)
{
	v &= 0xFFFFu;
	v = (v | (v << 8)) & 0x00FF00FFu; v = (v | (v << 4)) & 0x0F0F0F0Fu;
	v = (v | (v << 2)) & 0x33333333u; return (v | (v << 1)) & 0x55555555u;
}

constexpr uint32_t S2_MAX_GROUPS = 4096;
bool plan_seed2(pcr_ctx *ctx, PlanLists &L, const std::vector<pcrhost::Candidate> &cand, std::vector<uint32_t> &or_seed, std::vector<uint32_t> &or_plain, uint32_t &irr_off_mask,
	const SeqSet *S3 = nullptr)
{
	std::vector<uint32_t> &pf = L.s3_prefix;
	pf.clear();
	uint32_t pf_run = 0;
	const uint32_t n_or = 2*(uint32_t)cand.size();
	std::vector<uint32_t> &out = L.s2_seeds;
	out.clear(); L.s2_group_end.clear(); L.s2_group_offmask.clear(); L.s2_group_or.clear(); L.s2_group_nor.clear();
	irr_off_mask = 0;
	L.s2_masks.resize(n_or);
	if(ctx->s2_cache.size() > 16384) ctx->s2_cache.clear();
	size_t group_begin = 0; uint32_t group_mask = 0, group_or0 = 0, group_last = 0;
	auto fits = [&](size_t n, uint32_t g_or){
		if(S3) return g_or <= S3_MAX_OR && n <= S3_MAX_SEEDS;
		return g_or <= S2_MAX_OR && n <= S2_MAX_SEEDS && sizeof(S2Shared) + 17*(size_t)g_or + 8*n + 1024 <= 160*1024;
	};
	auto mask_of = [](const Planes &m){
		return make_uint4(spread16(m.a) | (spread16(m.a >> 16) << 1), spread16(m.c) | (spread16(m.c >> 16) << 1),
		                  spread16(m.g) | (spread16(m.g >> 16) << 1), spread16(m.t) | (spread16(m.t >> 16) << 1));
	};
	std::vector<uint8_t> &spans = L.s3_spans;
	spans.clear();
	if(ctx->s3_cache.size() > 16384) ctx->s3_cache.clear();
	for(uint32_t o = 0;o < n_or;++o){
		const pcrhost::Candidate &c = cand[o >> 1];
		const Planes &m = (o & 1u) ? c.rc : c.fwd;
		const pcr_ctx::S2Key key = {m.a, m.c, m.g, m.t, c.floor_};
		pcr_ctx::S3Entry *e3 = nullptr; const pcr_ctx::S2Entry *e2 = nullptr;
		if(S3){
			auto it = ctx->s3_cache.find(key);
			if(it == ctx->s3_cache.end()){
				pcr_ctx::S3Entry e; e.off_mask = 0;
				ctx->s3_tmp.clear(); ctx->s2_tmp.clear();
				e.seedable = pcrhost::orientation_index_seeds(m, c.floor_, ctx->s3_next, ctx->s3_tmp, ctx->s2_tmp);
				e.mask = mask_of(m);
				e.seeds.reserve(ctx->s3_tmp.size()); e.spans.reserve(ctx->s3_tmp.size());
				for(const pcrhost::FoldSeed &sd : ctx->s3_tmp){
					e.seeds.push_back((sd.code << 14) | ((uint32_t)sd.off << 9)); e.spans.push_back((uint8_t)(sd.lo | (sd.hi << 2))); e.off_mask |= 1u << sd.off;
				}
				it = ctx->s3_cache.emplace(key, std::move(e)).first;
			}
			e3 = &it->second; e2 = e3;
		}
		else{
			auto it = ctx->s2_cache.find(key);
			if(it == ctx->s2_cache.end()){
				pcr_ctx::S2Entry e; e.off_mask = 0;
				ctx->s2_tmp.clear();
				e.seedable = pcrhost::orientation_seeds(m, c.floor_, 0, ctx->s2_tmp, nullptr, S2_Q);
				e.mask = mask_of(m);
				e.seeds.reserve(ctx->s2_tmp.size());
				for(const pcrhost::Seed &sd : ctx->s2_tmp){ e.seeds.push_back((sd.code << 14) | ((uint32_t)sd.off << 9)); e.off_mask |= 1u << sd.off; }
				it = ctx->s2_cache.emplace(key, std::move(e)).first;
			}
			e2 = &it->second;
		}
		const pcr_ctx::S2Entry &e = *e2;
		L.s2_masks[o] = e.mask;
		if(!e.seedable){ or_plain.push_back(o); continue; }
		or_seed.push_back(o);
		if(!fits(out.size() - group_begin + e.seeds.size(), o - group_or0 + 1)){
			if(!fits(e.seeds.size(), 1) || L.s2_group_end.size() + 1 >= S2_MAX_GROUPS) return false;
			L.s2_group_end.push_back((uint32_t)out.size()); L.s2_group_offmask.push_back(group_mask); L.s2_group_or.push_back(group_or0); L.s2_group_nor.push_back(group_last - group_or0 + 1);
			group_begin = out.size(); group_mask = 0; group_or0 = o;
			if(S3){ pf.push_back(pf_run); pf_run = 0; }
		}
		group_last = o;
		const size_t at = out.size();
		out.resize(at + e.seeds.size());
		for(size_t k = 0;k < e.seeds.size();++k) out[at + k] = e.seeds[k] | (o - group_or0);
		if(S3){
			spans.insert(spans.end(), e3->spans.begin(), e3->spans.end());
			pcr_ctx::S3Chunks *ch = nullptr;
			for(pcr_ctx::S3Chunks &x : e3->chunks){ if(x.gen == S3->pix_generation){ ch = &x; break; } }
			if(!ch){
				ch = &e3->chunks[e3->next_slot]; e3->next_slot = (e3->next_slot + 1u) % pcr_ctx::S3_CHUNK_SETS;
				ch->run.resize(e.seeds.size());
				const uint32_t *const start = S3->pix_start_h.data();
				uint32_t run = 0;
				for(size_t k = 0;k < e.seeds.size();++k){
					const uint32_t key4 = (e.seeds[k] >> 14) << 2, sp = e3->spans[k];
					ch->run[k] = run; run += (start[key4 + (sp >> 2) + 1u] - start[key4 + (sp & 3u)] + 63u) >> 6;
				}
				ch->total = run; ch->gen = S3->pix_generation;
			}
			const size_t pa = pf.size();
			pf.resize(pa + ch->run.size());
			for(size_t k = 0;k < ch->run.size();++k) pf[pa + k] = pf_run + ch->run[k];
			pf_run += ch->total;
		}
		if(!(o & 1u)){ irr_off_mask |= e.off_mask; group_mask |= e.off_mask; }
	}
	L.s2_group_end.push_back((uint32_t)out.size()); L.s2_group_offmask.push_back(group_mask); L.s2_group_or.push_back(group_or0);
	L.s2_group_nor.push_back(or_seed.empty() ? 0u : group_last - group_or0 + 1);
	if(S3) pf.push_back(pf_run);
	return true;
}

constexpr size_t S3_LDS_BUDGET = 120*1024;
constexpr uint32_t S3_WG_THREADS = 1024;
uint32_t seed3_grid(const pcr_ctx *ctx) { return std::min<uint32_t>(2*ctx->n_cu, S3_MAX_WG); }
bool plan_seed3_slices(pcr_ctx *ctx, PlanLists &PL, bool with_irr)
{
	const uint32_t G_all = seed3_grid(ctx), seeds_per_turn = 16u*(S3_WG_THREADS/64);
	PL.s3_launch.resize(PL.s2_group_end.size());
	size_t g_begin = 0, g_prefix = 0;
	for(size_t g = 0;g < PL.s2_group_end.size();++g){
		const uint32_t ns = PL.s2_group_end[g] - (uint32_t)g_begin;
		g_begin = PL.s2_group_end[g];
		const uint32_t *P = PL.s3_prefix.data() + g_prefix;
		g_prefix += (size_t)ns + 1;
		pcr_ctx::S3Launch &L = PL.s3_launch[g];
		L.n_irr_wg = with_irr ? std::min<uint32_t>((ns + seeds_per_turn - 1u)/seeds_per_turn, G_all/4u) : 0u;
		const uint32_t G = (G_all - L.n_irr_wg) & ~1u;
		L.n_chunks = P[ns]; L.per_wg = std::max<uint32_t>(1u, (L.n_chunks + G - 1u)/G); L.slice_cap = 2;
		if(ns == 0) continue;
		uint32_t at = 0;
		for(uint32_t w = 0;w <= G;++w){
			const uint64_t target = (uint64_t)w*L.per_wg;
			while(at + 1u < ns && P[at + 1u] <= target) ++at;
			L.W.start[w] = at;
		}
		for(uint32_t w = G + 1;w <= S3_MAX_WG;++w) L.W.start[w] = at;
		for(uint32_t w = 0;w < G;++w) L.slice_cap = std::max(L.slice_cap, std::min(L.W.start[w + 1] + 2u, ns + 1u) - L.W.start[w]);
		if(17*(size_t)PL.s2_group_nor[g] + 9*(size_t)L.slice_cap + 64 > S3_LDS_BUDGET) return false;
	}
	return true;
}

void plan_seed1(pcr_ctx *ctx, PlanLists &L, const std::vector<pcrhost::Candidate> &cand, std::vector<uint32_t> &or_seed, std::vector<uint32_t> &or_plain, uint32_t &irr_off_mask)
{
	const uint32_t n_or = 2*(uint32_t)cand.size();
	std::vector<uint32_t> &out = L.s1_seeds;
	out.clear();
	irr_off_mask = 0;
	if(ctx->s1_cache.size() > 16384) ctx->s1_cache.clear();
	std::vector<const pcr_ctx::S2Entry *> ent(n_or);
	size_t total = 0;
	for(uint32_t o = 0;o < n_or;++o){
		const pcrhost::Candidate &c = cand[o >> 1];
		const Planes &m = (o & 1u) ? c.rc : c.fwd;
		const pcr_ctx::S2Key key = {m.a, m.c, m.g, m.t, c.floor_};
		auto it = ctx->s1_cache.find(key);
		if(it == ctx->s1_cache.end()){
			pcr_ctx::S2Entry e; e.off_mask = 0;
			ctx->s2_tmp.clear();
			e.seedable = pcrhost::orientation_seeds(m, c.floor_, 0, ctx->s2_tmp);
			e.seeds.reserve(ctx->s2_tmp.size());
			for(const pcrhost::Seed &sd : ctx->s2_tmp){ e.seeds.push_back(sd.code | ((uint32_t)sd.off << 16)); e.off_mask |= 1u << sd.off; }
			it = ctx->s1_cache.emplace(key, std::move(e)).first;
		}
		ent[o] = &it->second;
		if(ent[o]->seedable) total += ent[o]->seeds.size();
	}
	std::vector<uint8_t> drop(n_or, 0);
	if(total > S1_MAX_SEEDS){
		std::vector<uint32_t> by_len;
		for(uint32_t o = 0;o < n_or;++o){ if(ent[o]->seedable) by_len.push_back(o); }
		std::stable_sort(by_len.begin(), by_len.end(), [&](uint32_t x, uint32_t y){ return ent[x]->seeds.size() > ent[y]->seeds.size(); });
		for(size_t i = 0;i < by_len.size() && total > S1_MAX_SEEDS;++i){ drop[by_len[i]] = 1; total -= ent[by_len[i]]->seeds.size(); }
	}
	out.resize(total);
	size_t at = 0;
	for(uint32_t o = 0;o < n_or;++o){
		const pcr_ctx::S2Entry &e = *ent[o];
		if(!e.seedable || drop[o]){ or_plain.push_back(o); continue; }
		or_seed.push_back(o);
		const uint32_t tag = o << 21;
		for(size_t k = 0;k < e.seeds.size();++k) out[at + k] = e.seeds[k] | tag;
		at += e.seeds.size();
		if(!(o & 1u)) irr_off_mask |= e.off_mask;
	}
}

struct HostSeedPlan {
	std::vector<pcrhost::Seed> seeds;
	std::vector<std::vector<std::pair<uint16_t, int8_t> > > inheritors;
	size_t n_inherited = 0;
	std::vector<uint32_t> image, heads, multi;
};

int plan_seed_host(pcr_ctx *ctx, const std::vector<pcrhost::Candidate> &cand, HostSeedPlan &H, std::vector<uint32_t> &or_seed, std::vector<uint32_t> &or_plain,
	uint32_t &irr_off_mask)
{
	const uint32_t n_or = 2*(uint32_t)cand.size();
	struct OrientInfo { uint32_t begin, end; int max_exact_pos; bool seeded; };
	std::vector<OrientInfo> info;
	std::vector<pcrhost::Seed> &seeds = H.seeds;
	std::vector<std::vector<std::pair<uint16_t, int8_t> > > &inheritors = H.inheritors;
	size_t &n_inherited = H.n_inherited;
	std::vector<uint32_t> &image = H.image, &heads = H.heads, &multi = H.multi;
	info.assign(n_or, OrientInfo());
	inheritors.assign(n_or, std::vector<std::pair<uint16_t, int8_t> >());
	seeds.reserve((size_t)n_or*32);
	for(uint32_t o = 0;o < n_or;++o){
		const pcrhost::Candidate &c = cand[o >> 1];
		OrientInfo &me = info[o];
		me.begin = (uint32_t)seeds.size(); me.max_exact_pos = -1;
		const uint32_t bo = 2*c.base + (o & 1u);
		const int32_t sh = (o & 1u) ? -c.shift : c.shift;
		if(c.base != (o >> 1) && info[bo].seeded && info[bo].max_exact_pos <= 24 && info[bo].max_exact_pos + sh <= 24){
			inheritors[bo].push_back(std::make_pair((uint16_t)o, (int8_t)sh));
			n_inherited += info[bo].end - info[bo].begin;
			me.seeded = true; me.max_exact_pos = (info[bo].max_exact_pos < 0) ? -1 : info[bo].max_exact_pos + sh;
		}
		else me.seeded = pcrhost::orientation_seeds((o & 1) ? c.rc : c.fwd, c.floor_, o, seeds, &me.max_exact_pos);
		me.end = (uint32_t)seeds.size();
		if(me.seeded) or_seed.push_back(o); else or_plain.push_back(o);
	}
	if(or_seed.empty()) return PCR_OK;
	if(ctx->seed_count.size() != 65536){ ctx->seed_count.assign(65536, 0); ctx->seed_own.assign(65536, 0); }
	std::vector<uint16_t> &count = ctx->seed_count;
	bool overflow = false;
	uint32_t distinct = 0;
	std::vector<uint8_t> &own = ctx->seed_own;
	for(;;){
		image.assign(SEED_IMAGE_WORDS, 0u);
		overflow = false; distinct = 0;
		for(const pcrhost::Seed &sd : seeds){
			uint16_t &c = count[sd.code];
			if(c == 0){ image[sd.code >> 5] |= 1u << (sd.code & 31); ++distinct; }
			c = (uint16_t)(c + 1 + (inheritors.empty() ? 0 : inheritors[sd.orient].size()));
			if(c > 255){ overflow = true; break; }
			++own[sd.code];
		}
		if(distinct > SEED_MAX_DISTINCT) overflow = true;
		if(!overflow || n_inherited || or_seed.size() < 2) break;
		for(const pcrhost::Seed &sd : seeds){ count[sd.code] = 0; own[sd.code] = 0; }
		std::vector<uint32_t> by_len(or_seed);
		std::stable_sort(by_len.begin(), by_len.end(), [&](uint32_t x, uint32_t y){ return info[x].end - info[x].begin > info[y].end - info[y].begin; });
		const size_t n_drop = (by_len.size() + 3)/4;
		std::vector<uint8_t> drop(n_or, 0);
		for(size_t i = 0;i < n_drop;++i) drop[by_len[i]] = 1;
		std::vector<pcrhost::Seed> kept; kept.reserve(seeds.size());
		for(uint32_t o = 0;o < n_or;++o){
			const uint32_t b = info[o].begin, e = info[o].end;
			info[o].begin = (uint32_t)kept.size();
			if(!drop[o]) kept.insert(kept.end(), seeds.begin() + b, seeds.begin() + e);
			info[o].end = (uint32_t)kept.size();
			if(drop[o]) info[o].seeded = false;
		}
		seeds.swap(kept);
		or_seed.clear(); or_plain.clear();
		for(uint32_t o = 0;o < n_or;++o){ if(info[o].seeded) or_seed.push_back(o); else or_plain.push_back(o); }
	}
	for(const pcrhost::Seed &sd : seeds){
		if(sd.orient & 1u) continue;
		irr_off_mask |= 1u << sd.off;
		if(!inheritors.empty()){ for(const std::pair<uint16_t, int8_t> &in : inheritors[sd.orient]) irr_off_mask |= 1u << (sd.off + in.second); }
	}
	if(overflow){
		or_plain.clear(); or_seed.clear(); image.clear();
		for(uint32_t o = 0;o < n_or;++o) or_plain.push_back(o);
	}
	else{
		uint16_t *rank16 = (uint16_t *)(image.data() + SEED_BITMAP_WORDS);
		uint32_t run = 0;
		for(uint32_t w = 0;w < SEED_BITMAP_WORDS;++w){ rank16[w] = (uint16_t)run; run += (uint32_t)__builtin_popcount(image[w]); }
		heads.assign(distinct, 0u);
		uint32_t n_multi = 0;
		for(const pcrhost::Seed &sd : seeds){
			const uint32_t h = rank16[sd.code >> 5] + (uint32_t)__builtin_popcount(image[sd.code >> 5] & ((1u << (sd.code & 31)) - 1u));
			if(count[sd.code] == 1){ heads[h] = SEED_SINGLE | ((uint32_t)sd.orient << 8) | sd.off; continue; }
			if(heads[h] == 0){ heads[h] = 0x40000000u | n_multi; n_multi += own[sd.code]; }
		}
		std::vector<uint32_t> raw(n_multi, 0u);
		std::vector<uint8_t> &fill = ctx->seed_fill; fill.assign(distinct, 0);
		for(const pcrhost::Seed &sd : seeds){
			if(count[sd.code] == 1) continue;
			const uint32_t h = rank16[sd.code >> 5] + (uint32_t)__builtin_popcount(image[sd.code >> 5] & ((1u << (sd.code & 31)) - 1u));
			const uint32_t start = heads[h] & 0x3FFFFFFFu;
			raw[start + fill[h]++] = (uint32_t)sd.orient | ((uint32_t)sd.off << 24);
		}
		multi.clear(); multi.reserve(n_multi + n_multi/2 + 16);
		for(uint32_t h = 0;h < distinct;++h){
			if(heads[h] & SEED_SINGLE) continue;
			const uint32_t start = heads[h] & 0x3FFFFFFFu, n = fill[h];
			const uint32_t out0 = (uint32_t)multi.size();
			uint32_t header_at = 0, members = 0, cur_base = 0xFFFFFFFFu; int32_t cur_boff = -1;
			for(uint32_t e = 0;e < n;++e){
				const uint32_t sd = raw[start + e], orient = sd & 0xFFFFu, off = sd >> 24;
				const pcrhost::Candidate &c = cand[orient >> 1];
				const int32_t sh = (orient & 1u) ? -c.shift : c.shift;
				int32_t boff = (int32_t)off - sh;
				uint32_t base_orient = 2*c.base + (orient & 1u);
				if(boff < 0 || boff > 24){ boff = (int32_t)off; base_orient = orient; }
				if(members && base_orient == cur_base && boff == cur_boff && members < 256){
					multi.push_back(sd); ++members;
					multi[header_at] = SEED_GROUP | cur_base | ((uint32_t)cur_boff << 16) | ((members - 1) << 21);
				}
				else{
					header_at = (uint32_t)multi.size(); members = 1; cur_base = base_orient; cur_boff = boff;
					multi.push_back(SEED_GROUP | cur_base | ((uint32_t)cur_boff << 16));
					multi.push_back(sd);
				}
				if(!inheritors.empty()){
					for(const std::pair<uint16_t, int8_t> &in : inheritors[orient]){
						if(members == 256){
							header_at = (uint32_t)multi.size(); members = 0;
							multi.push_back(SEED_GROUP | cur_base | ((uint32_t)cur_boff << 16));
						}
						multi.push_back((uint32_t)in.first | ((uint32_t)((int32_t)off + in.second) << 24)); ++members;
						multi[header_at] = SEED_GROUP | cur_base | ((uint32_t)cur_boff << 16) | ((members - 1) << 21);
					}
				}
			}
			heads[h] = (out0 << 9) | ((uint32_t)multi.size() - out0);
		}
		n_multi = (uint32_t)multi.size();
		if(n_multi >= (1u << 22)){ ctx->seed_count.clear(); g_err = "pcr_select_words: seed table too large"; return PCR_ERR_CAPACITY; }
	}
	return PCR_OK;
}


enum class ScanForm { Popcount, BitSliced, Seed1Host, Seed1Dev, Seed2, Seed3 };
inline const char *form_name(ScanForm f)
{
	static const char *const names[] = { "popcount", "bitsliced", "seed1-host", "seed1-dev", "seed2", "seed3" };
	return names[(int)f];
}
inline bool is_seed1(ScanForm f) { return f == ScanForm::Seed1Host || f == ScanForm::Seed1Dev; }
inline bool is_seed2(ScanForm f) { return f == ScanForm::Seed2 || f == ScanForm::Seed3; }

struct ScanPlan {
	ScanForm form = ScanForm::BitSliced;
	std::vector<uint32_t> or_seed, or_plain;
	uint32_t irr_off_mask = 0;
	HostSeedPlan H;
	bool s3_with_irr = false;
	bool need_plain = false, need_seedset = false;
	size_t n_seeds = 0;
	uint32_t n_live = 0, min_len = 0;
	void reset()
	{
		form = ScanForm::BitSliced; or_seed.clear(); or_plain.clear(); irr_off_mask = 0;
		H.seeds.clear(); H.inheritors.clear(); H.n_inherited = 0; H.image.clear(); H.heads.clear(); H.multi.clear();
		s3_with_irr = need_plain = need_seedset = false; n_seeds = 0; n_live = min_len = 0;
	}
};

inline uint32_t live_irregular(const SeqSet &S, uint32_t min_oligo_length)
{
	uint32_t n_live = 0;
	for(uint32_t k = std::min<uint32_t>(min_oligo_length, 256);k < 256;++k) n_live += S.irr_size_count[k];
	return n_live;
}

int irr_index_usable(pcr_ctx *ctx, SeqSet &S, bool &usable)
{
	usable = false;
	if(S.irr_n_multi != 0 || (uint64_t)24*S.n_irr >= (uint64_t(1) << 32)) return PCR_OK;
	const int rc = ensure_irr_index(ctx, S);
	usable = rc == PCR_OK && S.irx_usable;
	return rc;
}

int choose_scan_form(pcr_ctx *ctx, SeqSet &S, const std::vector<pcrhost::Candidate> &cand, int optimize_5, int optimize_3, uint32_t min_oligo_length, ScanPlan &P, PlanLists &L)
{
	const uint32_t n_or = 2*(uint32_t)cand.size();
	std::vector<uint32_t> &or_seed = P.or_seed, &or_plain = P.or_plain;
	P.min_len = min_oligo_length; P.n_live = live_irregular(S, min_oligo_length);
	int rc;
	const bool no_shifts = ctx->scan_version == 3 && !optimize_5 && !optimize_3;
	const bool seed2_ok = no_shifts && !ctx->force_seed1 && n_or <= 65535;
	bool want_seed3 = false;
	if(seed2_ok && !ctx->no_seed3 && !ctx->no_irr_index && ctx->s2_dbg == 0){
		bool worth = true;
		if(!S.pix_valid){
			std::vector<uint32_t> os, op; uint32_t om = 0;
			worth = plan_seed2(ctx, L, cand, os, op, om, nullptr) && op.empty() && !os.empty();
		}
		if(worth){
			if((rc = ensure_pos_index(ctx, S)) != PCR_OK) return rc;
			bool irr_ok = P.n_live == 0;
			if(S.pix_usable && !irr_ok && (rc = irr_index_usable(ctx, S, irr_ok)) != PCR_OK) return rc;
			want_seed3 = S.pix_usable && irr_ok; P.s3_with_irr = P.n_live > 0;
		}
	}
	bool use_seed2 = false;
	if(seed2_ok){
		use_seed2 = plan_seed2(ctx, L, cand, or_seed, or_plain, P.irr_off_mask, want_seed3 ? &S : nullptr);
		if(want_seed3 && !(use_seed2 && or_plain.empty() && !or_seed.empty() && plan_seed3_slices(ctx, L, P.s3_with_irr))){
			or_seed.clear(); or_plain.clear();
			use_seed2 = plan_seed2(ctx, L, cand, or_seed, or_plain, P.irr_off_mask, nullptr);
		}
		if(use_seed2 && !or_plain.empty() && (n_or <= S1_MAX_OR || or_seed.empty())) use_seed2 = false;
		if(!use_seed2){ or_seed.clear(); or_plain.clear(); P.irr_off_mask = 0; }
	}
	const bool use_seed3 = use_seed2 && want_seed3 && or_plain.empty() && !or_seed.empty()
		&& L.s3_prefix.size() == L.s2_seeds.size() + L.s2_group_end.size() && L.s3_spans.size() == L.s2_seeds.size();
	if(use_seed2){ P.form = use_seed3 ? ScanForm::Seed3 : ScanForm::Seed2; P.n_seeds = L.s2_seeds.size(); }
	else if(no_shifts && !ctx->host_seed_tables && n_or <= S1_MAX_OR){
		plan_seed1(ctx, L, cand, or_seed, or_plain, P.irr_off_mask);
		P.form = ScanForm::Seed1Dev; P.n_seeds = L.s1_seeds.size();
	}
	else if(ctx->scan_version == 3 && n_or <= 65535){
		const int prc = plan_seed_host(ctx, cand, P.H, or_seed, or_plain, P.irr_off_mask);
		if(ctx->seed_count.size() == 65536){ for(const pcrhost::Seed &sd : P.H.seeds){ ctx->seed_count[sd.code] = 0; ctx->seed_own[sd.code] = 0; } }
		if(prc != PCR_OK) return prc;
		P.form = ScanForm::Seed1Host; P.n_seeds = P.H.seeds.size() + P.H.n_inherited;
	}
	else{
		for(uint32_t o = 0;o < n_or;++o) or_plain.push_back(o);
		P.form = (ctx->scan_version == 1) ? ScanForm::Popcount : ScanForm::BitSliced;
	}
	if(or_seed.empty() && P.form != ScanForm::Popcount) P.form = ScanForm::BitSliced;
	P.need_plain = (ctx->scan_version != 1) && !or_plain.empty();
	P.need_seedset = !or_seed.empty() && S.n_degen_tiles > 0;
	return PCR_OK;
}

struct PassJob {
	pcr_ctx *ctx = nullptr; int which = 0, opt5 = 0, opt3 = 0; float thr = 0.0f; uint32_t min_len = 0; bool async = false;
	pcr_amplify_args args = {}; FusedAmp fa = {}; bool has_fa = false;
	uint32_t seq = 0;
	bool begun = false, ctrl_was_clean = false;
	std::vector<pcrhost::Candidate> cand; ScanPlan P; PlanLists L;
	std::vector<uint4> hf, hr; std::vector<uint32_t> hfl;
	std::vector<OligoDev> ol;
	bool fuse = false; size_t bits_bytes = 0;
	Seed3HalfSlices pair_W; uint32_t pair_slice_cap = 0;
	void reset()
	{
		seq = 0; begun = ctrl_was_clean = false; has_fa = false; fa = FusedAmp(); async = false;
		cand.clear(); P.reset(); L.clear(); hf.clear(); hr.clear(); hfl.clear(); ol.clear(); fuse = false; bits_bytes = 0;
	}
};

struct Scan2Staged { Scan2Tables T; const uint32_t *d_tab = nullptr, *d_bias = nullptr, *d_map = nullptr; };
struct StagedTables {
	SeedTables ST = {};
	Seed2Tables ST2 = {};
	const uint32_t *d_s3_prefix = nullptr; const uint8_t *d_s3_spans = nullptr;
	Scan2Staged plain, seedset;
	bool lean = false, fuse = false;
	size_t bits_bytes = 0;
};

void stage_scan2(Stager &st, const std::vector<uint32_t> &orients, Scan2Staged &B)
{
	B.d_tab = st.put(B.T.tab.data(), B.T.tab.size());
	B.d_bias = st.put(B.T.bias.data(), B.T.bias.size());
	std::vector<uint32_t> m(orients);
	m.resize((m.size() + 255) & ~size_t(255), 0xFFFFFFFFu);
	B.d_map = st.put(m.data(), m.size());
}

void prepare_tables(const SeqSet &S, PassJob &J, FusedAmp *fa)
{
	const std::vector<pcrhost::Candidate> &cand = J.cand;
	const uint32_t ncand = (uint32_t)cand.size(), n_or = 2*ncand;
	J.hf.resize(ncand); J.hr.resize(ncand); J.hfl.resize(ncand);
	for(uint32_t c = 0;c < ncand;++c){
		J.hf[c] = make_uint4(cand[c].fwd.a, cand[c].fwd.c, cand[c].fwd.g, cand[c].fwd.t);
		J.hr[c] = make_uint4(cand[c].rc.a, cand[c].rc.c, cand[c].rc.g, cand[c].rc.t);
		J.hfl[c] = cand[c].floor_;
	}
	if(is_seed2(J.P.form)){
		std::vector<uint8_t> &floors2 = J.L.s2_floors;
		floors2.assign(((size_t)n_or + 15) & ~size_t(15), 0);
		for(uint32_t o = 0;o < n_or;++o) floors2[o] = (uint8_t)std::min<uint32_t>(cand[o >> 1].floor_, 255u);
	}
	J.fuse = false; J.bits_bytes = 0; J.ol.clear();
	if(fa && fa->n_pairs){
		J.bits_bytes = (size_t)fa->n_pairs*((S.n + 63)/64)*sizeof(uint64_t);
		J.fuse = ((uintptr_t)fa->d_fr % 16 == 0) && ((uintptr_t)fa->d_rf % 16 == 0) && (J.bits_bytes % 16 == 0);
		if(J.fuse) build_oligos(fa->pairs, fa->n_pairs, fa->a, J.ol);
	}
}

int stage_tables(pcr_ctx *ctx, SeqSet &S, const PassJob &J, FusedAmp *fa, bool async, bool ctrl_was_clean, StagedTables &T)
{
	const std::vector<pcrhost::Candidate> &cand = J.cand;
	const ScanPlan &P = J.P; const PlanLists &L = J.L;
	const uint32_t ncand = (uint32_t)cand.size(), n_or = 2*ncand;
	const bool seed2 = is_seed2(P.form), seed3 = P.form == ScanForm::Seed3;
	const bool build_tables = P.form == ScanForm::Seed1Dev;
	const HostSeedPlan &H = P.H;
	int rc;
	if(P.need_plain) build_scan2_tables(cand, P.or_plain, T.plain.T);
	if(P.need_seedset) build_scan2_tables(cand, P.or_seed, T.seedset.T);
	size_t bytes = ncand*(2*sizeof(uint4) + sizeof(uint32_t)) + 1024;
	bytes += (T.plain.T.tab.size() + T.plain.T.bias.size() + P.or_plain.size() + 256)*sizeof(uint32_t);
	bytes += (T.seedset.T.tab.size() + T.seedset.T.bias.size() + P.or_seed.size() + 256)*sizeof(uint32_t);
	bytes += (H.image.size() + H.heads.size() + H.multi.size() + 64)*sizeof(uint32_t);
	if(seed2){
		bytes += L.s2_masks.size()*sizeof(uint4) + L.s2_floors.size() + L.s2_seeds.size()*sizeof(uint32_t) + 512;
		if(seed3) bytes += L.s3_prefix.size()*sizeof(uint32_t) + L.s3_spans.size() + 128;
	}
	if(build_tables) bytes += L.s1_seeds.size()*sizeof(uint32_t) + 256;
	T.bits_bytes = J.bits_bytes; T.fuse = J.fuse;
	if(T.fuse) bytes += J.ol.size()*sizeof(OligoDev) + 64;
	const uint32_t guard_seq = J.seq ? J.seq : ctx->mail_seq + 1;
	const uint64_t gen = S.ctrl.generation;
	if((rc = S.ctrl.ensure(8 + 2*(size_t)S.n + 4)) != PCR_OK) return rc;
	T.lean = ctx->direct_ok && async && T.fuse && seed2 && !P.or_seed.empty() && ctrl_was_clean && gen == S.ctrl.generation
		&& S.bucket_cap == POST_CAP && 2*fa->n_pairs <= 32*POST_MASK_WORDS;
	if(ctx->debug_log) fprintf(stderr, "[pcramp] staging: %s\n", T.lean ? "lean (tables written into device memory, no staging launch)" : "k_stage");
	Stager st(ctx);
	if((rc = T.lean ? st.begin_direct(bytes) : st.begin(bytes)) != PCR_OK) return rc;
	ctx->d_cand_fwd = st.put(J.hf.data(), ncand);
	ctx->d_cand_rc = st.put(J.hr.data(), ncand);
	ctx->d_cand_floor = st.put(J.hfl.data(), ncand);
	if(P.need_plain) stage_scan2(st, P.or_plain, T.plain);
	if(P.need_seedset) stage_scan2(st, P.or_seed, T.seedset);
	if(!H.image.empty()){
		T.ST.image = st.put(H.image.data(), H.image.size());
		T.ST.heads = st.put(H.heads.data(), H.heads.size());
		T.ST.multi = H.multi.empty() ? T.ST.heads : st.put(H.multi.data(), H.multi.size());
	}
	const uint32_t *d_s1_seeds = nullptr;
	if(build_tables){
		d_s1_seeds = st.put(L.s1_seeds.data(), L.s1_seeds.size());
		if((rc = ctx->s1_image.ensure(SEED_IMAGE_WORDS)) != PCR_OK) return rc;
		if((rc = ctx->s1_heads.ensure(2*(size_t)S1_MAX_SEEDS)) != PCR_OK) return rc;
		if((rc = ctx->s1_multi.ensure(S1_MAX_SEEDS)) != PCR_OK) return rc;
		T.ST.image = ctx->s1_image.p; T.ST.heads = ctx->s1_heads.p; T.ST.multi = ctx->s1_multi.p; T.ST.flat = 1;
	}
	if(seed2){
		T.ST2.seeds = st.put(L.s2_seeds.data(), L.s2_seeds.size());
		T.ST2.masks = st.put(L.s2_masks.data(), L.s2_masks.size());
		T.ST2.floors = st.put(L.s2_floors.data(), L.s2_floors.size());
		T.ST2.n_seeds = (uint32_t)L.s2_seeds.size(); T.ST2.n_or = n_or;
		if(seed3){ T.d_s3_prefix = st.put(L.s3_prefix.data(), L.s3_prefix.size()); T.d_s3_spans = st.put(L.s3_spans.data(), L.s3_spans.size()); }
	}
	const size_t ctrl_bytes = (8 + 2*(size_t)S.n)*sizeof(uint32_t);
	if(T.fuse){
		fa->d_oligos = st.put(J.ol.data(), J.ol.size());
		fa->staged = true;
		if(T.lean) st.seal(guard_seq);
		else if((rc = st.ship(S.ctrl.p, ctrl_bytes, fa->d_fr, T.bits_bytes, fa->d_rf, T.bits_bytes, guard_seq)) != PCR_OK) return rc;
	}
	else if((rc = st.ship(S.ctrl.p, ctrl_bytes, nullptr, 0, nullptr, 0, guard_seq)) != PCR_OK) return rc;
	if(build_tables){
		if((rc = ctx->s1_part.ensure(2*S1_GROUPS)) != PCR_OK) return rc;
		hipLaunchKernelGGL(k_seed_tables<false>, dim3(S1_GROUPS), dim3(S1_BUILD_THREADS), 0, ctx->stream, d_s1_seeds, (uint32_t)L.s1_seeds.size(),
			ctx->s1_part.p, ctx->s1_image.p, ctx->s1_heads.p, ctx->s1_multi.p);
		hipLaunchKernelGGL(k_seed_tables<true>, dim3(S1_GROUPS), dim3(S1_BUILD_THREADS), 0, ctx->stream, d_s1_seeds, (uint32_t)L.s1_seeds.size(),
			ctx->s1_part.p, ctx->s1_image.p, ctx->s1_heads.p, ctx->s1_multi.p);
		HIP_TRY(hipGetLastError());
	}
	return PCR_OK;
}


int launch_popcount(pcr_ctx *ctx, SeqSet &S, const HitSink &sink)
{
	hipLaunchKernelGGL(k_scan, dim3(S.n_tiles), dim3(SCAN_THREADS), 0, ctx->stream, S.planes.p, S.valid_d(),
		S.d_blk_off.p, S.d_len.p, S.d_active.p, S.tile_seq.p, S.tile_pos0.p, ctx->d_cand_fwd, ctx->d_cand_rc,
		ctx->d_cand_floor, sink.ncand, sink);
	HIP_TRY(hipGetLastError());
	return PCR_OK;
}

int launch_seed1(pcr_ctx *ctx, SeqSet &S, const ScanPlan &P, const StagedTables &T, const HitSink &sink)
{
	const uint32_t ncand = sink.ncand;
	const bool cand_lds = ncand <= SEED_CAND_LDS;
	const auto kernel = cand_lds ? k_seed<true> : k_seed<false>;
	const size_t dyn = cand_lds ? (size_t)ncand*(2*sizeof(uint4) + sizeof(uint32_t)) : 0;
	int per_cu = 0;
	const hipError_t oe = hipOccupancyMaxActiveBlocksPerMultiprocessor(&per_cu, kernel, SEED_THREADS, dyn);
	const size_t lds_wg = ((sizeof(SeedShared) + dyn + 4095)/4096)*4096;
	per_cu = std::max(1, std::min<int>(per_cu, (int)((160*1024)/lds_wg)));
	const uint32_t resident = (oe == hipSuccess) ? (uint32_t)per_cu*ctx->n_cu : SEED_MAX_GRID;
	const uint32_t tiles_per_wg = SEED_WAVES*SEED_TILES_PER_WAVE;
	const dim3 sgrid(std::min<uint32_t>((S.n_tiles + tiles_per_wg - 1)/tiles_per_wg, resident)), sblock(SEED_THREADS);
	IrrArgs IA; IA.irr = S.irr.p; IA.perm = S.irr_perm.p; IA.n_live = P.n_live; IA.off_mask = P.or_plain.empty() ? P.irr_off_mask : 0u;
	const uint32_t irr_wgs = (P.n_live + IRR_THREADS*IRR_PER_LANE - 1)/(IRR_THREADS*IRR_PER_LANE);
	const dim3 fgrid(sgrid.x + irr_wgs);
	if(ctx->debug_log) fprintf(stderr, "[pcramp] k_seed: %d workgroups per CU x %u CUs\n", per_cu, ctx->n_cu);
	hipLaunchKernelGGL(kernel, fgrid, sblock, dyn, ctx->stream, S.tb_d(), S.planes.p, S.valid_d(), S.d_blk_off.p, S.d_nblk_real.p, S.d_len.p, S.d_active.p,
		S.tile_seq.p, S.tile_pos0.p, S.tile_degen.p, S.n_tiles, T.ST, ctx->d_cand_fwd, ctx->d_cand_rc, ctx->d_cand_floor, ncand, IA, sgrid.x, sink);
	HIP_TRY(hipGetLastError());
	return PCR_OK;
}

void seed3_args(SeqSet &S, const Seed2Tables &Tg, const uint32_t *d_chunk_prefix, const uint8_t *d_spans, const pcr_ctx::S3Launch &L3, const IrrArgs2 &IA, Seed3Tables &T3, Seed3Set &Q3)
{
	T3.seeds = Tg.seeds; T3.spans = d_spans; T3.chunk_prefix = d_chunk_prefix; T3.masks = Tg.masks; T3.floors = Tg.floors;
	T3.n_seeds = Tg.n_seeds; T3.n_or = Tg.n_or; T3.or_base = Tg.or_base;
	T3.pix_first = S.pix_first.p; T3.pix_last = S.pix_last.p; T3.pix_ent = S.pix_ent.p;
	Q3 = Seed3Set{ S.valid_d(), S.blk_info.p, S.blk_local.p, S.d_active.p };
	T3.n_chunks = L3.n_chunks; T3.per_wg = L3.per_wg; T3.slice_cap = L3.slice_cap;
	T3.n_irr_wg = IA.ix_first ? L3.n_irr_wg : 0u;
}
inline size_t seed3_lds(const Seed3Tables &T3)
{
	return (size_t)T3.n_or*sizeof(uint4) + 2*(size_t)T3.slice_cap*sizeof(uint32_t) + (((size_t)T3.n_or + 15) & ~size_t(15)) + (((size_t)T3.slice_cap + 15) & ~size_t(15)) + 16;
}

int launch_seed3_group(pcr_ctx *ctx, SeqSet &S, const Seed2Tables &Tg, const uint32_t *d_chunk_prefix, const uint8_t *d_spans, const pcr_ctx::S3Launch &L3, const IrrArgs2 &IA,
	const HitSink &sink, const S2Clear &Z)
{
	Seed3Tables T3; Seed3Set Q3;
	seed3_args(S, Tg, d_chunk_prefix, d_spans, L3, IA, T3, Q3);
	const size_t dyn3 = seed3_lds(T3);
	if(!ctx->s3_attr_set){
		HIP_TRY(hipFuncSetAttribute((const void *)k_seed3<S3_WG_THREADS>, hipFuncAttributeMaxDynamicSharedMemorySize, 128*1024));
		ctx->s3_attr_set = true;
	}
	hipLaunchKernelGGL(k_seed3<S3_WG_THREADS>, dim3(seed3_grid(ctx)), dim3(S3_WG_THREADS), dyn3, ctx->stream, T3, Q3, IA, ctx->d_cand_fwd, ctx->d_cand_floor, sink, Z, L3.W);
	return PCR_OK;
}

IrrArgs2 group_irr_args(SeqSet &S, const ScanPlan &P, uint32_t group_offmask, bool first_launch, bool irr_by_index)
{
	IrrArgs2 IA; IA.scan = S.irr_scan.p; IA.irr = S.irr.p; IA.n_live = P.n_live;
	IA.off_mask = group_offmask;
	IA.exhaustive = first_launch ? 1u : 0u;
	IA.ix_first = IA.ix_last = IA.ix_words = nullptr; IA.min_cws = std::min<uint32_t>(P.min_len, 255u);
	if(!P.or_plain.empty()){
		IA.off_mask = 0;
		if(!first_launch) IA.n_live = 0;
	}
	else if(irr_by_index){
		IA.ix_first = S.irx_first.p; IA.ix_last = S.irx_last.p; IA.ix_words = S.irx_words.p; IA.n_live = 0;
	}
	return IA;
}
S2Clear group_clear(const StagedTables &T, const FusedAmp *fa, const HitSink &sink, bool first_launch)
{
	S2Clear Z = { nullptr, 0u, nullptr, 0u, nullptr };
	if(T.lean && first_launch){
		Z.z0 = (uint4 *)fa->d_fr; Z.z1 = (uint4 *)fa->d_rf; Z.n0 = Z.n1 = (uint32_t)(T.bits_bytes/16); Z.ctrl = sink.counters;
	}
	return Z;
}

int launch_seed_groups(pcr_ctx *ctx, SeqSet &S, const ScanPlan &P, const PlanLists &L, const StagedTables &T, const FusedAmp *fa, const HitSink &sink)
{
	const bool seed3 = P.form == ScanForm::Seed3;
	const uint32_t tiles_per_wg = S2_WAVES*2;
	const dim3 sgrid(std::max<uint32_t>(1u, std::min<uint32_t>((S.n_tiles + tiles_per_wg - 1)/tiles_per_wg, ctx->n_cu))), sblock(S2_THREADS);
	int rc;
	if(!ctx->s2_attr_set){
		HIP_TRY(hipFuncSetAttribute((const void *)k_seed2<false>, hipFuncAttributeMaxDynamicSharedMemorySize, (int)(160*1024 - sizeof(S2Shared))));
		HIP_TRY(hipFuncSetAttribute((const void *)k_seed2<true>, hipFuncAttributeMaxDynamicSharedMemorySize, (int)(160*1024 - sizeof(S2Shared))));
		ctx->s2_attr_set = true;
	}
	const auto k_seed2_of_ctx = ctx->s2_dbg ? k_seed2<true> : k_seed2<false>;
	bool irr_by_index = P.s3_with_irr;
	if(!seed3){
		irr_by_index = P.or_plain.empty() && P.n_live > 0 && !ctx->no_irr_index;
		for(size_t g = 0, b = 0;g < L.s2_group_end.size();++g){ if((size_t)L.s2_group_end[g] - b > (size_t)sgrid.x*S2_THREADS) irr_by_index = false; b = L.s2_group_end[g]; }
		if(irr_by_index && (rc = irr_index_usable(ctx, S, irr_by_index)) != PCR_OK) return rc;
	}
	uint32_t g_begin = 0, g_prefix = 0;
	bool first_launch = true;
	for(size_t g = 0;g < L.s2_group_end.size();++g){
		Seed2Tables Tg = T.ST2;
		const uint32_t or0 = L.s2_group_or[g], g_or = L.s2_group_nor[g];
		const uint8_t *const d_spans = seed3 ? T.d_s3_spans + g_begin : nullptr;
		Tg.seeds = T.ST2.seeds + g_begin; Tg.n_seeds = L.s2_group_end[g] - g_begin;
		Tg.masks = T.ST2.masks + (size_t)or0; Tg.floors = T.ST2.floors + or0; Tg.n_or = g_or; Tg.or_base = or0;
		g_begin = L.s2_group_end[g];
		if(Tg.n_seeds == 0){ g_prefix += 1u; continue; }
		const size_t dyn = (size_t)g_or*sizeof(uint4) + (((size_t)g_or + 15) & ~size_t(15)) + 8*((size_t)Tg.n_seeds + 64) + 16;
		const IrrArgs2 IA = group_irr_args(S, P, L.s2_group_offmask[g], first_launch, irr_by_index);
		if(ctx->debug_log) fprintf(stderr, "[pcramp] k_seed2: %u workgroups, %u seeds of orientations %u..%u (group %zu of %zu), %zu + %zu B of LDS\n", sgrid.x, Tg.n_seeds,
			or0, or0 + g_or - 1, g + 1, L.s2_group_end.size(), sizeof(S2Shared), dyn);
		const S2Clear Z = group_clear(T, fa, sink, first_launch);
		if(seed3){
			if((rc = launch_seed3_group(ctx, S, Tg, T.d_s3_prefix + g_prefix, d_spans, L.s3_launch[g], IA, sink, Z)) != PCR_OK) return rc;
			g_prefix += Tg.n_seeds + 1u;
		}
		else hipLaunchKernelGGL(k_seed2_of_ctx, sgrid, sblock, dyn, ctx->stream, S.tb_d(), S.valid_d(), S.tile_desc.p, S.n_tiles, Tg, S.d_active.p, ctx->d_cand_fwd, ctx->d_cand_floor,
			sink.ncand, IA, sink, ctx->s2_dbg, Z);
		HIP_TRY(hipGetLastError());
		first_launch = false;
	}
	return PCR_OK;
}

int launch_irregular(pcr_ctx *ctx, SeqSet &S, const ScanPlan &P, const HitSink &sink)
{
	const unsigned irr_grid = (P.n_live + IRR_THREADS*IRR_PER_LANE - 1)/(IRR_THREADS*IRR_PER_LANE);
	hipLaunchKernelGGL(k_scan_irr, dim3(irr_grid), dim3(IRR_THREADS), 0, ctx->stream, S.irr.p, S.irr_perm.p, P.n_live,
		S.d_active.p, ctx->d_cand_fwd, ctx->d_cand_floor, sink.ncand, sink);
	HIP_TRY(hipGetLastError());
	return PCR_OK;
}

int launch_scans(pcr_ctx *ctx, SeqSet &S, const ScanPlan &P, const PlanLists &L, const StagedTables &T, const FusedAmp *fa, const HitSink &sink)
{
	int rc = PCR_OK;
	const uint32_t ncand = sink.ncand;
	if(S.n_tiles){
		ProfScope scan_prof(ctx, PCR_PROF_SCAN, ctx->prof && (ctx->prof_pass++ % ctx->prof_stride) == 0);
		if(P.need_plain && (rc = launch_scan2(ctx, S, T.plain.T, ncand, sink, T.plain.d_tab, T.plain.d_bias, nullptr, S.n_tiles, T.plain.d_map)) != PCR_OK) return rc;
		if(P.form == ScanForm::Popcount) rc = launch_popcount(ctx, S, sink);
		else if(is_seed1(P.form)) rc = launch_seed1(ctx, S, P, T, sink);
		else if(is_seed2(P.form)) rc = launch_seed_groups(ctx, S, P, L, T, fa, sink);
		if(rc != PCR_OK) return rc;
		if(P.need_seedset && (rc = launch_scan2(ctx, S, T.seedset.T, ncand, sink, T.seedset.d_tab, T.seedset.d_bias, S.degen_tiles.p, S.n_degen_tiles,
			T.seedset.d_map)) != PCR_OK) return rc;
		scan_prof.finish();
	}
	const bool irr_taken = S.n_tiles && (is_seed1(P.form) || is_seed2(P.form));
	if(P.n_live && !irr_taken) rc = launch_irregular(ctx, S, P, sink);
	return rc;
}


PostRow post_row_args(pcr_ctx *ctx, SeqSet &S, const HitSink &sink, const FusedAmp *fa, uint32_t seq)
{
	PostRow R;
	R.hits = sink.hits; R.seq_count = sink.seq_count; R.best = sink.best; R.ncand = sink.ncand; R.planes = S.planes.p; R.blk_off = S.d_blk_off.p;
	R.irr = S.irr.p; R.irr_off = S.irr_off.p; R.db = S.db.p; R.seg_hi = S.d_seg_hi; R.counters = sink.counters; R.epoch = sink.epoch; R.n_seq = S.n;
	R.oligos = fa->d_oligos; R.n_pairs = fa->n_pairs; R.mask_words = (2*fa->n_pairs + 31)/32; R.len = S.d_len.p; R.active = S.d_active.p;
	R.amp_min = fa->a->amp_min; R.amp_max = fa->a->amp_max; R.ident_thr = fa->a->ident_threshold; R.use_taq = fa->a->use_taq_mama;
	R.bits_fr = fa->d_fr; R.bits_rf = fa->d_rf; R.bit_words = (uint64_t)((S.n + 63)/64); R.pub_mail = ctx->mail.dev + (seq % pcr_ctx::MAIL_RING); R.pub_seq = seq;
	return R;
}
template<class K>
void launch_post(K kernel, uint32_t waves, pcr_ctx *ctx, SeqSet &S, const HitSink &sink, const FusedAmp *fa, uint32_t seq)
{
	const PostRow R = post_row_args(ctx, S, sink, fa, seq);
	hipLaunchKernelGGL(kernel, dim3((S.n + waves - 1)/waves), dim3(64*waves), 0, ctx->stream, R.hits, R.seq_count, R.best, R.ncand, R.planes,
		R.blk_off, R.irr, R.irr_off, R.db, R.seg_hi, R.counters, R.epoch, R.n_seq,
		R.oligos, R.n_pairs, R.mask_words, R.len, R.active, R.amp_min, R.amp_max,
		R.ident_thr, R.use_taq, R.bits_fr, R.bits_rf, R.bit_words, R.pub_mail, R.pub_seq);
}
int fused_tail(pcr_ctx *ctx, SeqSet &S, const HitSink &sink, FusedAmp *fa, uint32_t reserved_seq)
{
	const uint32_t seq = reserved_seq ? reserved_seq : ++ctx->mail_seq;
	if(sink.cap == POST_CAP){
		launch_post(k_post<8>, 8, ctx, S, sink, fa, seq);
		S.ctrl_clean = true; S.touched_from_seg = true;
	}
	else if(sink.cap == 128) launch_post(k_post_big<128, 4>, 4, ctx, S, sink, fa, seq);
	else launch_post(k_post_big<256, 4>, 4, ctx, S, sink, fa, seq);
	HIP_TRY(hipGetLastError());
	fa->posted = true;
	S.touched_built = false;
	return PCR_OK;
}

template<class K, class... Extra>
void launch_finalize(K kernel, dim3 grid, dim3 block, size_t lds, pcr_ctx *ctx, SeqSet &S, const HitSink &sink, Extra... extra)
{
	hipLaunchKernelGGL(kernel, grid, block, lds, ctx->stream, sink.hits, sink.seq_count, sink.cap, sink.best, sink.ncand, S.planes.p, S.d_blk_off.p, S.irr.p,
		S.irr_off.p, S.db.p, S.d_seg_hi, sink.counters, sink.epoch, S.touched.p, extra...);
}
template<bool ALL = false>
int plain_tail(pcr_ctx *ctx, SeqSet &S, const HitSink &sink, bool async, FusedAmp *fa)
{
	int rc;
	hipLaunchKernelGGL(k_touched, dim3((S.n + 255)/256), dim3(256), 0, ctx->stream, sink.seq_count, S.n, sink.counters, S.touched.p);
	HIP_TRY(hipGetLastError());
	S.touched_built = true;
	uint32_t np2 = 1; while(np2 < sink.cap) np2 <<= 1;
	if(np2 <= 1024) launch_finalize(k_finalize<FIN_WAVES, ALL>, dim3((S.n + FIN_WAVES - 1)/FIN_WAVES), dim3(64*FIN_WAVES), (size_t)FIN_WAVES*np2*sizeof(uint64_t), ctx, S, sink);
	else if(np2 <= MAX_BUCKET_CAP) launch_finalize(k_finalize<1, ALL>, dim3(S.n), dim3(64), (size_t)np2*sizeof(uint64_t), ctx, S, sink);
	else{
		if((rc = ctx->fin_scratch.ensure((size_t)S.n*np2)) != PCR_OK) return rc;
		launch_finalize(k_finalize_big<ALL>, dim3(S.n), dim3(FINBIG_THREADS), 0, ctx, S, sink, ctx->fin_scratch.p);
	}
	HIP_TRY(hipGetLastError());
	++ctx->mail_seq;
	if(async && fa && fa->staged){ fa->pub_seq = ctx->mail_seq; fa->pub_counters = sink.counters; }
	else{
		hipLaunchKernelGGL(k_publish, dim3(1), dim3(64), 0, ctx->stream, sink.counters, ctx->mail.dev + (ctx->mail_seq % pcr_ctx::MAIL_RING), ctx->mail_seq);
		HIP_TRY(hipGetLastError());
	}
	return PCR_OK;
}

uint32_t resized_buckets(bool overflowed, uint32_t cap, uint32_t largest_fill, int attempt)
{
	if(overflowed){
		uint32_t want = cap*2;
		while(want < largest_fill && want < MAX_BUCKET_CAP_GLOBAL) want *= 2;
		return want;
	}
	if(cap <= 64 || attempt >= 12) return 0;
	uint32_t want = 64;
	while(want < largest_fill + largest_fill/16) want *= 2;
	return (want*4 <= cap) ? want : 0;
}

inline bool fused_tail_fits(uint32_t cap, uint32_t n_pairs) { return (cap == POST_CAP || cap == 128 || cap == 256) && 2*n_pairs <= 32*POST_MASK_WORDS; }
inline bool buckets_fit(uint64_t n_slots) { return n_slots < (uint64_t(1) << 32) && n_slots*(sizeof(Hit) + sizeof(DevEntry)) <= (uint64_t(96) << 30); }

inline bool begin_pass(SeqSet &S)
{
	S.have_db = false; S.n_entries = 0;
	const bool ctrl_was_clean = S.ctrl_clean;
	S.ctrl_clean = false; S.touched_from_seg = false;
	return ctrl_was_clean;
}

int plan_pass(pcr_ctx *ctx, PassJob &J, const pcr_pair *pairs, uint32_t n_pairs)
{
	SeqSet &S = ctx->sets[J.which];
	HostTimer timer(ctx, 0);
	if(ctx->timing) ++ctx->n_timed;
	pcrhost::build_candidates((const uint64_t *)pairs, n_pairs, J.opt5 != 0, J.opt3 != 0, J.thr, J.cand);
	const uint32_t ncand = (uint32_t)J.cand.size();
	if(S.n == 0 || ncand == 0) return PCR_OK;
	int rc;
	if((rc = choose_scan_form(ctx, S, J.cand, J.opt5, J.opt3, J.min_len, J.P, J.L)) != PCR_OK) return rc;
	if(ctx->debug_log) fprintf(stderr, "[pcramp] scan plan: form=%s, %u candidates, %zu seeded orientations (%zu seeds), %zu plain, %u/%u IUPAC tiles, %u-slot buckets\n",
		form_name(J.P.form), ncand, J.P.or_seed.size(), J.P.n_seeds, J.P.or_plain.size(), S.n_degen_tiles, S.n_tiles, S.bucket_cap);
	prepare_tables(S, J, J.has_fa ? &J.fa : nullptr);
	return PCR_OK;
}

bool plans_without_device_work(const pcr_ctx *ctx, const SeqSet &S, int opt5, int opt3, uint32_t min_len)
{
	if(ctx->scan_version != 3 || opt5 || opt3 || ctx->force_seed1) return false;
	const bool may_want_seed3 = !ctx->no_seed3 && !ctx->no_irr_index && ctx->s2_dbg == 0;
	if(may_want_seed3 && !S.pix_valid) return false;
	if(live_irregular(S, min_len) == 0 || ctx->no_irr_index) return true;
	return S.irr_n_multi != 0 || (uint64_t)24*S.n_irr >= (uint64_t(1) << 32) || S.irx_valid;
}

bool pass_is_pipelinable(const pcr_ctx *ctx, const PassJob &J)
{
	const SeqSet &S = ctx->sets[J.which];
	return J.async && J.has_fa && J.fuse && S.n != 0 && !J.cand.empty() && is_seed2(J.P.form)
		&& fused_tail_fits(S.bucket_cap, J.fa.n_pairs) && buckets_fit((uint64_t)S.n*S.bucket_cap);
}


int stage_pass(pcr_ctx *ctx, PassJob &J, bool ctrl_was_clean, StagedTables &T)
{
	SeqSet &S = ctx->sets[J.which];
	int rc;
	if((rc = ctx->best.ensure((size_t)S.n*J.cand.size())) != PCR_OK) return rc;
	if(ctx->best.generation != ctx->best_seen){
		HIP_TRY(hipMemsetAsync(ctx->best.p, 0, ctx->best.cap*sizeof(uint32_t), ctx->stream));
		ctx->best_seen = ctx->best.generation; ctx->epoch = std::min(ctx->debug_epoch, EPOCH_LIMIT);
	}
	if((rc = stage_tables(ctx, S, J, J.has_fa ? &J.fa : nullptr, J.async, ctrl_was_clean, T)) != PCR_OK) return rc;
	if((rc = S.touched.ensure(S.n)) != PCR_OK) return rc;
	S.d_seg_hi = S.ctrl.p + 8 + S.n;
	return PCR_OK;
}

int size_attempt(pcr_ctx *ctx, SeqSet &S, const PassJob &J, int attempt, HitSink &sink)
{
	int rc;
	const uint32_t cap = S.bucket_cap;
	const uint64_t n_slots = (uint64_t)S.n*cap;
	if(!buckets_fit(n_slots)){
		assert(J.seq == 0);
		S.bucket_cap = 64;
		g_err = "pcr_select_words: the per-sequence hit buckets would not fit (too many tied sites per sequence)"; return PCR_ERR_CAPACITY;
	}
	if((rc = ctx->hits.ensure(n_slots)) != PCR_OK) return rc;
	if((rc = S.db.ensure(n_slots)) != PCR_OK) return rc;
	if(attempt > 0) HIP_TRY(hipMemsetAsync(S.ctrl.p, 0, (8 + 2*(size_t)S.n)*sizeof(uint32_t), ctx->stream));
	if(ctx->epoch >= EPOCH_LIMIT){
		HIP_TRY(hipMemsetAsync(ctx->best.p, 0, ctx->best.cap*sizeof(uint32_t), ctx->stream));
		ctx->epoch = 0;
	}
	++ctx->epoch;
	sink.best = ctx->best.p; sink.hits = ctx->hits.p; sink.seq_count = S.ctrl.p + 8;
	sink.counters = S.ctrl.p; sink.cap = cap; sink.ncand = (uint32_t)J.cand.size(); sink.epoch = ctx->epoch;
	return PCR_OK;
}

inline void pass_enqueued(SeqSet &S, uint32_t cap)
{
	S.db_cap = cap; S.n_slots = (uint64_t)S.n*cap;
	S.n_touched = N_TOUCHED_UNKNOWN; S.n_entries = 1; S.have_db = true;
}

int run_pass(pcr_ctx *ctx, PassJob &J, uint64_t *n_entries_out)
{
	SeqSet &S = ctx->sets[J.which];
	FusedAmp *const fa = J.has_fa ? &J.fa : nullptr;
	const bool async = J.async;
	const bool ctrl_was_clean = J.begun ? J.ctrl_was_clean : begin_pass(S);
	const ScanPlan &P = J.P;
	const uint32_t ncand = (uint32_t)J.cand.size();
	if(S.n == 0 || ncand == 0){ S.have_db = true; S.n_touched = 0; return PCR_OK; }
	HostTimer timer(ctx, 1);
	int rc;
	StagedTables T;
	if((rc = stage_pass(ctx, J, ctrl_was_clean, T)) != PCR_OK) return rc;

	timer.next(2);
	uint32_t h_counters[4];
	for(int attempt = 0;;++attempt){
		const uint32_t cap = S.bucket_cap;
		const uint64_t n_slots = (uint64_t)S.n*cap;
		HitSink sink;
		if((rc = size_attempt(ctx, S, J, attempt, sink)) != PCR_OK) return rc;
		const bool fused = async && fa && fa->staged && fused_tail_fits(cap, fa->n_pairs);
		if(J.seq && !fused){ g_err = "pcr_screen_device: a pipelined pass lost its fused tail"; return PCR_ERR_STATE; }
		if((rc = launch_scans(ctx, S, P, J.L, T, fa, sink)) != PCR_OK) return rc;
		if((rc = fused ? fused_tail(ctx, S, sink, fa, J.seq) : plain_tail(ctx, S, sink, async, fa)) != PCR_OK) return rc;
		if(async){ pass_enqueued(S, cap); return PCR_OK; }
		timer.next(3);
		if((rc = mail_wait(ctx, ctx->mail_seq, h_counters)) != PCR_OK) return rc;
		timer.next(2);
		S.db_cap = cap; S.n_slots = n_slots;
		const bool overflowed = (h_counters[0] & 1u) != 0;
		if(overflowed && (attempt >= 12 || cap >= MAX_BUCKET_CAP_GLOBAL)){ g_err = "pcr_select_words: more than 65536 candidate sites in one sequence (per-sequence bucket limit)"; return PCR_ERR_CAPACITY; }
		const uint32_t want = resized_buckets(overflowed, cap, h_counters[2], attempt);
		if(!want) break;
		S.bucket_cap = want;
	}
	if(ctx->debug_log) fprintf(stderr, "[pcramp] pass done: %u-slot buckets, largest fill %u, %u sequences with entries\n", S.db_cap, h_counters[2], h_counters[3]);
	S.n_touched = h_counters[3];
	S.n_entries = S.n_touched ? 1 : 0;
	S.have_db = true;
	if(n_entries_out){
		if((rc = count_entries(ctx, S)) != PCR_OK) return rc;
		*n_entries_out = S.n_entries;
	}
	return PCR_OK;
}


bool pass_is_pairable(const pcr_ctx *ctx, const PassJob &J)
{
	const SeqSet &S = ctx->sets[J.which];
	return ctx->pair_mode != 0 && pass_is_pipelinable(ctx, J) && J.P.form == ScanForm::Seed3 && J.L.s2_group_end.size() == 1 && J.L.s2_group_end[0] != 0
		&& !J.P.need_plain && !J.P.need_seedset && S.n_tiles != 0 && S.bucket_cap == POST_CAP
		&& !(ctx->prof && ctx->prof_pass % ctx->prof_stride == 0);
}

bool pair_slices(const pcr_ctx *ctx, PassJob &J)
{
	const pcr_ctx::S3Launch &L3 = J.L.s3_launch[0];
	const uint32_t ns = J.L.s2_group_end[0], G = (seed3_grid(ctx) - L3.n_irr_wg) & ~1u, Gh = G/2;
	uint32_t *const st = J.pair_W.start;
	for(uint32_t w = 0;w <= Gh;++w) st[w] = L3.W.start[2*w];
	for(uint32_t w = Gh + 1;w <= S3_MAX_WG/2;++w) st[w] = st[Gh];
	uint32_t cap = 2;
	for(uint32_t w = 0;w < Gh;++w) cap = std::max(cap, std::min(st[w + 1] + 2u, ns + 1u) - st[w]);
	J.pair_slice_cap = cap;
	return 17*(size_t)J.L.s2_group_nor[0] + 9*(size_t)cap + 64 <= S3_LDS_BUDGET;
}

bool passes_can_pair(PassJob &A, PassJob &B)
{
	if(A.ctx == B.ctx || !pass_is_pairable(A.ctx, A) || !pass_is_pairable(B.ctx, B)) return false;
	const uintptr_t a[2] = { (uintptr_t)A.fa.d_fr, (uintptr_t)A.fa.d_rf }, b[2] = { (uintptr_t)B.fa.d_fr, (uintptr_t)B.fa.d_rf };
	for(int i = 0;i < 2;++i) for(int j = 0;j < 2;++j){ if(a[i] < b[j] + B.bits_bytes && b[j] < a[i] + A.bits_bytes) return false; }
	return pair_slices(A.ctx, A) && pair_slices(B.ctx, B);
}

struct PairHalf { pcr_ctx *ctx; PassJob *J; SeqSet *S; StagedTables T; HitSink sink; Seed3Row scan; PostRow post; };
int prepare_half(PairHalf &H)
{
	pcr_ctx *const ctx = H.ctx; PassJob &J = *H.J; SeqSet &S = *H.S;
	const bool ctrl_was_clean = begin_pass(S);
	int rc;
	HostTimer timer(ctx, 1);
	if((rc = stage_pass(ctx, J, ctrl_was_clean, H.T)) != PCR_OK) return rc;
	timer.next(2);
	if((rc = size_attempt(ctx, S, J, 0, H.sink)) != PCR_OK) return rc;
	if(!J.fa.staged || H.sink.cap != POST_CAP){ g_err = "pcr_screen_device: a paired pass lost its fused tail"; return PCR_ERR_STATE; }
	if(ctx->prof) ++ctx->prof_pass;
	const PlanLists &L = J.L;
	Seed2Tables Tg = H.T.ST2;
	Tg.n_seeds = L.s2_group_end[0]; Tg.masks = H.T.ST2.masks + (size_t)L.s2_group_or[0]; Tg.floors = H.T.ST2.floors + L.s2_group_or[0];
	Tg.n_or = L.s2_group_nor[0]; Tg.or_base = L.s2_group_or[0];
	H.scan.IA = group_irr_args(S, J.P, L.s2_group_offmask[0], true, J.P.s3_with_irr);
	seed3_args(S, Tg, H.T.d_s3_prefix, H.T.d_s3_spans, L.s3_launch[0], H.scan.IA, H.scan.T3, H.scan.Q);
	H.scan.T3.per_wg *= 2u; H.scan.T3.slice_cap = J.pair_slice_cap; H.scan.T3.n_irr_wg = (H.scan.T3.n_irr_wg + 1u)/2u;
	H.scan.cand_fwd = ctx->d_cand_fwd; H.scan.cand_floor = ctx->d_cand_floor; H.scan.sink = H.sink;
	H.scan.Z = group_clear(H.T, &J.fa, H.sink, true);
	H.post = post_row_args(ctx, S, H.sink, &J.fa, J.seq);
	return PCR_OK;
}

int run_pass_pair(PassJob &JA, PassJob &JB)
{
	PairHalf H[2];
	H[0].ctx = JA.ctx; H[0].J = &JA; H[1].ctx = JB.ctx; H[1].J = &JB;
	int rc;
	for(PairHalf &h : H){
		h.S = &h.ctx->sets[h.J->which];
		if((rc = prepare_half(h)) != PCR_OK) return rc;
	}
	pcr_ctx *const ctx = JA.ctx;
	HostTimer timer(ctx, 2);
	const uint32_t Gx = seed3_grid(ctx)/2;
	const size_t dyn3 = std::max(seed3_lds(H[0].scan.T3), seed3_lds(H[1].scan.T3));
	if(!ctx->s3_pair_attr_set){
		HIP_TRY(hipFuncSetAttribute((const void *)k_seed3_pair<S3_WG_THREADS>, hipFuncAttributeMaxDynamicSharedMemorySize, 128*1024));
		ctx->s3_pair_attr_set = true;
	}
	const uint32_t Px = (std::max(H[0].S->n, H[1].S->n) + 7u)/8u;
	if(ctx->debug_log) fprintf(stderr, "[pcramp] paired launch: passes %u + %u, scan grid %u x 2 (irregular workgroups %u + %u, slice_cap' %u + %u, %zu B of LDS), tail grid %u x 2\n",
		JA.seq, JB.seq, Gx, H[0].scan.T3.n_irr_wg, H[1].scan.T3.n_irr_wg, H[0].scan.T3.slice_cap, H[1].scan.T3.slice_cap, dyn3, Px);
	hipLaunchKernelGGL(k_seed3_pair<S3_WG_THREADS>, dim3(Gx, 2), dim3(S3_WG_THREADS), dyn3, ctx->stream, H[0].scan, JA.pair_W, H[1].scan, JB.pair_W);
	HIP_TRY(hipGetLastError());
	hipLaunchKernelGGL(k_post_pair<8>, dim3(Px, 2), dim3(64*8), 0, ctx->stream, H[0].post, H[1].post);
	HIP_TRY(hipGetLastError());
	for(PairHalf &h : H){
		h.S->ctrl_clean = true; h.S->touched_from_seg = true;
		h.J->fa.posted = true; h.S->touched_built = false;
		pass_enqueued(*h.S, POST_CAP);
	}
	return PCR_OK;
}

void fill_job(pcr_ctx *ctx, PassJob &J, pcr_set which, int optimize_5, int optimize_3, float threshold, uint32_t min_oligo_length, bool async, const FusedAmp *fa)
{
	J.ctx = ctx; J.which = (int)which; J.opt5 = optimize_5; J.opt3 = optimize_3; J.thr = threshold; J.min_len = min_oligo_length; J.async = async;
	J.has_fa = fa != nullptr;
	if(fa){ J.fa = *fa; J.args = *fa->a; J.fa.a = &J.args; }
}

void quiesce_stream(pcr_ctx *ctx);

int select_impl(pcr_ctx *ctx, pcr_set which, const pcr_pair *pairs, uint32_t n_pairs, int optimize_5, int optimize_3,
	float threshold, uint32_t min_oligo_length, uint64_t *n_entries_out, bool async, FusedAmp *fa = nullptr)
{
	if(!ctx || (n_pairs && !pairs)){ g_err = "pcr_select_words: bad argument"; return PCR_ERR_ARG; }
	if(min_oligo_length < 1 || min_oligo_length > 32){ g_err = "pcr_select_words: min_oligo_length must be in [1,32]"; return PCR_ERR_ARG; }
	HIP_TRY(hipSetDevice(ctx->device));
	if(n_entries_out) *n_entries_out = 0;
	assert(ctx->lq_client.queued.load() == 0);
	quiesce_stream(ctx);
	PassJob J;
	fill_job(ctx, J, which, optimize_5, optimize_3, threshold, min_oligo_length, async, fa);
	J.ctrl_was_clean = begin_pass(ctx->sets[which]); J.begun = true;
	int rc = plan_pass(ctx, J, pairs, n_pairs);
	if(rc == PCR_OK) rc = run_pass(ctx, J, n_entries_out);
	if(fa){ const pcr_amplify_args *a = fa->a; *fa = J.fa; fa->a = a; }
	return rc;
}


struct Launcher {
	int device; hipStream_t stream; unsigned refs = 0;
	cpu_set_t near; bool have_near = false;
	struct InFlight { const pcr_ctx *ctx; const PassMail *slot; uint32_t seq; };
	std::mutex inflight_m; std::vector<InFlight> inflight;
	pcrq::LaunchQueue q;
	Launcher(int dev, hipStream_t st, unsigned spin_us);
	void forget_published()
	{
		inflight.erase(std::remove_if(inflight.begin(), inflight.end(), [](const InFlight &f){
			const uint32_t v = __atomic_load_n((const uint32_t *)&f.slot->seq, __ATOMIC_ACQUIRE);
			return v >= f.seq && (v - f.seq) % pcr_ctx::MAIL_RING == 0; }), inflight.end());
	}
	void launched(const PassJob &J)
	{
		std::lock_guard<std::mutex> lk(inflight_m);
		if(inflight.size() >= 4*pcr_ctx::MAIL_RING){ forget_published(); if(inflight.size() >= 4*pcr_ctx::MAIL_RING) inflight.erase(inflight.begin()); }
		inflight.push_back(InFlight{ J.ctx, J.ctx->mail.host + (J.seq % pcr_ctx::MAIL_RING), J.seq });
	}
	size_t backlog()
	{
		std::lock_guard<std::mutex> lk(inflight_m);
		forget_published();
		return inflight.size();
	}
	void forget_handle(const pcr_ctx *ctx)
	{
		std::lock_guard<std::mutex> lk(inflight_m);
		inflight.erase(std::remove_if(inflight.begin(), inflight.end(), [&](const InFlight &f){ return f.ctx == ctx; }), inflight.end());
	}
};
constexpr unsigned PAIR_HOLD_CAP_US = 20000;
std::mutex g_launchers_m;
std::vector<Launcher *> g_launchers;

PassJob *acquire_job(pcr_ctx *ctx)
{
	PassJob *J = nullptr;
	{
		std::lock_guard<std::mutex> lk(ctx->job_m);
		if(!ctx->job_free.empty()){ J = ctx->job_free.back(); ctx->job_free.pop_back(); }
	}
	if(!J){ J = new PassJob(); ctx->job_all.push_back(J); }
	return J;
}
void release_job(pcr_ctx *ctx, PassJob *J)
{
	J->reset();
	std::lock_guard<std::mutex> lk(ctx->job_m);
	ctx->job_free.push_back(J);
}
void free_jobs(pcr_ctx *ctx)
{
	for(PassJob *J : ctx->job_all) delete J;
	ctx->job_all.clear(); ctx->job_free.clear();
}

constexpr unsigned LAUNCH_SPIN_US = 200;

bool read_cpu_list(const std::string &path, cpu_set_t &set)
{
	CPU_ZERO(&set);
	FILE *f = fopen(path.c_str(), "r");
	if(!f) return false;
	char buf[4096]; const bool got = fgets(buf, sizeof(buf), f) != nullptr;
	fclose(f);
	if(!got) return false;
	for(const char *p = buf;*p && *p != '\n';){
		char *e; const long a = strtol(p, &e, 10);
		if(e == p) return false;
		long b = a;
		if(*e == '-'){ p = e + 1; b = strtol(p, &e, 10); if(e == p) return false; }
		for(long c = a;c <= b && c < CPU_SETSIZE;++c) CPU_SET((int)c, &set);
		p = (*e == ',') ? e + 1 : e;
	}
	return true;
}
bool near_cpus(cpu_set_t &out)
{
	const int cpu = sched_getcpu();
	if(cpu < 0) return false;
	const std::string base = "/sys/devices/system/cpu/cpu" + std::to_string(cpu);
	cpu_set_t llc, core, allowed;
	if(!read_cpu_list(base + "/cache/index3/shared_cpu_list", llc)) return false;
	if(!read_cpu_list(base + "/topology/thread_siblings_list", core)) CPU_ZERO(&core);
	CPU_SET(cpu, &core);
	if(sched_getaffinity(0, sizeof(allowed), &allowed) != 0) return false;
	CPU_ZERO(&out);
	for(int c = 0;c < CPU_SETSIZE;++c){ if(CPU_ISSET(c, &llc) && CPU_ISSET(c, &allowed) && !CPU_ISSET(c, &core)) CPU_SET(c, &out); }
	return CPU_COUNT(&out) > 0;
}

Launcher::Launcher(int dev, hipStream_t st, unsigned spin_us) : device(dev), stream(st),
	q([this](void *job, std::string &err) -> int {
		PassJob &J = *(PassJob *)job;
		assert(J.seq != 0 && J.ctx->launcher);
		if(J.ctx->debug_log) fprintf(stderr, "[pcramp] single launch: pass %u of handle %p (%s)\n", J.seq, (void *)J.ctx, pass_is_pairable(J.ctx, J) ? "pairable" : "not pairable");
		const int rc = run_pass(J.ctx, J, nullptr);
		if(rc != PCR_OK) err = g_err;
		else launched(J);
		return rc;
	},
	[](void *job){ PassJob *J = (PassJob *)job; release_job(J->ctx, J); },
	[this]{
		if(have_near) (void)pthread_setaffinity_np(pthread_self(), sizeof(near), &near);
		(void)hipSetDevice(device);
	},
	spin_us)
{
	const char *v = getenv("PCRAMP_LAUNCH_PIN");
	have_near = !(v && v[0] == '0') && near_cpus(near);
	pcrq::LaunchQueue::Pairing pr;
	pr.holdable = [](void *job){ const PassJob &J = *(const PassJob *)job; return pass_is_pairable(J.ctx, J); };
	pr.may_hold = [this](void *job){ return ((const PassJob *)job)->ctx->pair_mode == 2 || backlog() >= 2; };
	pr.can_pair = [](void *a, void *b){
		PassJob &A = *(PassJob *)a, &B = *(PassJob *)b;
		const bool ok = passes_can_pair(A, B);
		if(!ok && A.ctx->debug_log) fprintf(stderr, "[pcramp] pass %u of handle %p does not pair with pass %u of handle %p behind it\n", A.seq, (void *)A.ctx, B.seq, (void *)B.ctx);
		return ok;
	};
	pr.run_pair = [this](void *a, void *b, std::string &err) -> int {
		PassJob &A = *(PassJob *)a, &B = *(PassJob *)b;
		const int rc = run_pass_pair(A, B);
		if(rc != PCR_OK) err = g_err;
		else{ launched(A); launched(B); }
		return rc;
	};
	pr.cap_us = PAIR_HOLD_CAP_US;
	q.set_pairing(std::move(pr));
}

Launcher *attach_launcher(pcr_ctx *ctx)
{
	if(ctx->launcher) return ctx->launcher;
	std::lock_guard<std::mutex> lk(g_launchers_m);
	for(Launcher *L : g_launchers){ if(L->device == ctx->device && L->stream == ctx->stream){ ++L->refs; return ctx->launcher = L; } }
	unsigned spin = LAUNCH_SPIN_US;
	if(const char *v = getenv("PCRAMP_LAUNCH_SPIN_US")) spin = (unsigned)std::min<unsigned long>(strtoul(v, nullptr, 0), 10000ul);
	Launcher *L = new Launcher(ctx->device, ctx->stream, spin);
	if(ctx->debug_log || ctx->timing) fprintf(stderr, "[pcramp] launcher thread for stream %p: caller on cpu %d, launcher %s (%d cpus), spin %u us\n", (void *)ctx->stream,
		sched_getcpu(), L->have_near ? "pinned beside it" : "not pinned", L->have_near ? CPU_COUNT(&L->near) : 0, spin);
	L->refs = 1;
	g_launchers.push_back(L);
	return ctx->launcher = L;
}
void detach_launcher(pcr_ctx *ctx)
{
	Launcher *L = ctx->launcher;
	if(!L) return;
	ctx->launcher = nullptr;
	L->forget_handle(ctx);
	{
		std::lock_guard<std::mutex> lk(g_launchers_m);
		if(--L->refs) return;
		g_launchers.erase(std::find(g_launchers.begin(), g_launchers.end(), L));
	}
	L->q.stop();
	delete L;
}

void quiesce_stream(pcr_ctx *ctx)
{
	if(ctx->launcher){ ctx->launcher->q.wait_empty(); return; }
	std::lock_guard<std::mutex> lk(g_launchers_m);
	for(Launcher *L : g_launchers){ if(L->device == ctx->device && L->stream == ctx->stream){ L->q.wait_empty(); return; } }
}

int flush_launcher(pcr_ctx *ctx)
{
	if(!ctx->launcher) return PCR_OK;
	ctx->launcher->q.flush(&ctx->lq_client);
	int code; std::string msg; uint32_t seq;
	if(!ctx->lq_client.take_error(code, msg, seq)) return PCR_OK;
	std::vector<pcr_ctx::Pending> &pd = ctx->pending;
	pd.erase(std::remove_if(pd.begin(), pd.end(), [&](const pcr_ctx::Pending &q){ return (int32_t)(q.seq - seq) >= 0; }), pd.end());
	g_err = msg;
	return code;
}

int screen_pass(pcr_ctx *ctx, pcr_set which, const pcr_pair *pairs, uint32_t n_pairs, int optimize_5, int optimize_3,
	float select_threshold, uint32_t min_oligo_length, const pcr_amplify_args *args, uint64_t *d_bits_fr, uint64_t *d_bits_rf)
{
	if(min_oligo_length < 1 || min_oligo_length > 32){ g_err = "pcr_select_words: min_oligo_length must be in [1,32]"; return PCR_ERR_ARG; }
	int rc;
	if(ctx->lq_client.poisoned.load(std::memory_order_acquire) && (rc = flush_launcher(ctx)) != PCR_OK) return rc;
	HIP_TRY(hipSetDevice(ctx->device));
	SeqSet &S = ctx->sets[which];
	FusedAmp fa; fa.pairs = pairs; fa.n_pairs = n_pairs; fa.a = args; fa.d_fr = d_bits_fr; fa.d_rf = d_bits_rf;
	PassJob *J = acquire_job(ctx);
	fill_job(ctx, *J, which, optimize_5, optimize_3, select_threshold, min_oligo_length, true, &fa);
	bool inline_pass = !ctx->launch_thread || !plans_without_device_work(ctx, S, optimize_5, optimize_3, min_oligo_length);
	if(inline_pass){
		if((rc = flush_launcher(ctx)) != PCR_OK){ release_job(ctx, J); return rc; }
		J->ctrl_was_clean = begin_pass(S); J->begun = true;
	}
	rc = plan_pass(ctx, *J, pairs, n_pairs);
	if(rc == PCR_OK && !inline_pass && !pass_is_pipelinable(ctx, *J)){
		inline_pass = true;
		rc = flush_launcher(ctx);
	}
	if(rc != PCR_OK){
		if(!J->begun){ (void)flush_launcher(ctx); (void)begin_pass(S); }
		release_job(ctx, J);
		return rc;
	}
	pcr_ctx::Pending p;
	p.which = (int)which; p.pairs.assign(pairs, pairs + n_pairs); p.opt5 = optimize_5; p.opt3 = optimize_3;
	p.thr = select_threshold; p.min_len = min_oligo_length; p.args = *args; p.d_fr = d_bits_fr; p.d_rf = d_bits_rf;
	if(!inline_pass){
		Launcher *L = attach_launcher(ctx);
		p.seq = J->seq = ++ctx->mail_seq;
		J->fa.pairs = nullptr;
		ctx->pending.push_back(std::move(p));
		++ctx->n_pipelined;
		L->q.push(&ctx->lq_client, J, J->seq);
		return PCR_OK;
	}
	assert(ctx->lq_client.queued.load() == 0);
	if(ctx->debug_log) fprintf(stderr, "[pcramp] inline pass of handle %p\n", (void *)ctx);
	quiesce_stream(ctx);
	const uint32_t seq0 = ctx->mail_seq;
	rc = run_pass(ctx, *J, nullptr);
	if(rc == PCR_OK && !J->fa.posted) rc = amplify_launch(ctx, S, pairs, n_pairs, args, d_bits_fr, d_bits_rf, &J->fa);
	release_job(ctx, J);
	if(rc != PCR_OK) return rc;
	if(ctx->mail_seq != seq0){
		p.seq = ctx->mail_seq;
		ctx->pending.push_back(std::move(p));
	}
	return PCR_OK;
}

int drain(pcr_ctx *ctx)
{
	{ const int frc = flush_launcher(ctx); if(frc != PCR_OK) return frc; }
	if(ctx->pending.empty()) return PCR_OK;
	std::vector<pcr_ctx::Pending> pend;
	pend.swap(ctx->pending);
	int rc;
	for(size_t i = 0;i < pend.size();++i){
		uint32_t c[4];
		if((rc = mail_wait(ctx, pend[i].seq, c)) != PCR_OK) return rc;
		SeqSet &S = ctx->sets[pend[i].which];
		if(!(c[0] & 1u)){
			if(c[3] == N_TOUCHED_UNKNOWN_DEV){ S.n_touched = N_TOUCHED_UNKNOWN; S.n_entries = 1; }
			else{ S.n_touched = c[3]; S.n_entries = c[3] ? 1 : 0; }
			continue;
		}
		uint32_t want = S.bucket_cap*2;
		while(want < c[2] && want < MAX_BUCKET_CAP_GLOBAL) want *= 2;
		S.bucket_cap = std::min(want, MAX_BUCKET_CAP_GLOBAL);
		for(size_t j = i;j < pend.size();++j){
			const pcr_ctx::Pending &q = pend[j];
			if((rc = select_impl(ctx, (pcr_set)q.which, q.pairs.data(), (uint32_t)q.pairs.size(), q.opt5, q.opt3, q.thr, q.min_len, nullptr, false)) != PCR_OK) return rc;
			if((rc = amplify_launch(ctx, ctx->sets[q.which], q.pairs.data(), (uint32_t)q.pairs.size(), &q.args, q.d_fr, q.d_rf)) != PCR_OK) return rc;
		}
		break;
	}
	return PCR_OK;
}

}
```

Before: 26.27 billion.

## Keep per-orientation seed3 lists resident in a device seed store across passes

Adds a persistent device-visible seed store (host-mapped buffer) holding each cached orientation's seeds, chunk runs and spans. Plans then emit only small per-orientation records instead of rebuilding and uploading flat seed/prefix/span arrays each pass. The seed3 kernel resolves seed indices through these records, with a binary search or a short forward walk from an encoded record hint in the slice start words. The change also reuses pair vectors and adds sub-phase host timers, at the cost of extra indirection in the kernel, more LDS, and store resets that synchronize the stream.

```diff
diff --git a/pcramp_amd/csrc/pcr_device.hip b/pcramp_amd/csrc/pcr_device.hip
--- a/pcramp_amd/csrc/pcr_device.hip
+++ b/pcramp_amd/csrc/pcr_device.hip
@@ -639,7 +639,7 @@
 	std::unordered_map<S2Key, S2Entry, S2KeyHash> s2_cache;
 	std::vector<pcrhost::Seed> s2_tmp;
 	static constexpr int S3_CHUNK_SETS = 4;
-	struct S3Chunks { uint64_t gen = 0; uint32_t total = 0; std::vector<uint32_t> run; };
+	struct S3Chunks { uint64_t gen = 0; uint32_t total = 0; std::vector<uint32_t> run; uint32_t blk_off = 0, blk_epoch = 0; };
 	struct S3Entry : S2Entry { std::vector<uint8_t> spans;  S3Chunks chunks[S3_CHUNK_SETS]; uint32_t next_slot = 0; };
 	std::unordered_map<S2Key, S3Entry, S2KeyHash> s3_cache;
 	std::vector<pcrhost::FoldSeed> s3_tmp;
@@ -734,6 +734,13 @@
 	ItemScratch shared;
 	DevBuf<uint2> pe3_end; DevBuf<uint32_t> pe3_before, pe3_ord; DevBuf<uint64_t> pe3_sum, pe3_keys, pe3_bits; DevBuf<uint8_t> pe3_tmp;
 	DevBuf<pcr_product_end3> pe3_rec;
+	DevBuf<uint8_t> s3_store{true};
+	size_t s3_store_bytes = size_t(16) << 20, s3_store_used = 0;
+	uint32_t s3_store_epoch = 1; uint64_t s3_store_resets = 0;
+	bool s3_resident = true;
+	std::atomic<bool> s3_store_stale{false};
+	std::vector<std::vector<pcr_pair> > pairs_spare;
+	double t_sub[5] = {0, 0, 0, 0, 0};
 };
 
 namespace {
@@ -776,6 +783,18 @@
 		slot = s; t0 = t1;
 	}
 	~HostTimer() { next(slot); }
+};
+struct SubTimer {
+	pcr_ctx *ctx; std::chrono::steady_clock::time_point t0;
+	explicit SubTimer(pcr_ctx *c) : ctx(c) { restart(); }
+	void restart() { if(ctx->timing) t0 = std::chrono::steady_clock::now(); }
+	void lap(int part)
+	{
+		if(!ctx->timing) return;
+		const auto t1 = std::chrono::steady_clock::now();
+		ctx->t_sub[part] += std::chrono::duration<double, std::micro>(t1 - t0).count();
+		t0 = t1;
+	}
 };
 
 __global__ void k_apply_splits(const uint64_t *__restrict__ where, uint32_t n, uint32_t *__restrict__ planes , uint32_t *__restrict__ nib)
@@ -1337,6 +1356,8 @@
 	if(const char *v = getenv("PCRAMP_IRR_INDEX")) ctx->no_irr_index = v[0] == '0';
 	if(const char *v = getenv("PCRAMP_SEED3")) ctx->no_seed3 = v[0] == '0';
 	if(const char *v = getenv("PCRAMP_S3_NEXT")) ctx->s3_next = v[0] != '0';
+	if(const char *v = getenv("PCRAMP_S3_RESIDENT")) ctx->s3_resident = v[0] != '0';
+	if(const char *v = getenv("PCRAMP_S3_STORE_KB")) ctx->s3_store_bytes = std::max<size_t>(4, std::min<size_t>(strtoull(v, nullptr, 0), size_t(1) << 20)) << 10;
 	if(const char *v = getenv("PCRAMP_LAUNCH_THREAD")) ctx->launch_thread = v[0] != '0';
 	if(const char *v = getenv("PCRAMP_PAIR")) ctx->pair_mode = (v[0] == '0') ? 0 : (strcmp(v, "force") == 0) ? 2 : 1;
 	if(const char *v = getenv("PCRAMP_SCAN")){ if(v[0] == '1') ctx->scan_version = 1; else if(v[0] == '2') ctx->scan_version = 2; }
@@ -1398,6 +1419,8 @@
 			(unsigned long long)ctx->n_pipelined, (unsigned long long)ctx->n_timed, ctx->lq_client.max_depth);
 		fprintf(stderr, "[pcramp] host us/pass: plan %.1f  stage %.1f  launch %.1f  wait %.1f | amplify prep %.1f  launch %.1f  (%llu passes)\n",
 			ctx->t_host[0]/n, ctx->t_host[1]/n, ctx->t_host[2]/n, ctx->t_host[3]/n, ctx->t_host[4]/n, ctx->t_host[5]/n, (unsigned long long)ctx->n_timed);
+		fprintf(stderr, "[pcramp] stage A us/pass: candidates %.1f  seed plan %.1f  slices %.1f  host tables %.1f  enqueue %.1f | seed store: %zu KB used, %llu resets\n",
+			ctx->t_sub[0]/n, ctx->t_sub[1]/n, ctx->t_sub[2]/n, ctx->t_sub[3]/n, ctx->t_sub[4]/n, ctx->s3_store_used >> 10, (unsigned long long)ctx->s3_store_resets);
 	}
 	delete ctx;
 }
diff --git a/pcramp_amd/csrc/pcr_host.hpp b/pcramp_amd/csrc/pcr_host.hpp
--- a/pcramp_amd/csrc/pcr_host.hpp
+++ b/pcramp_amd/csrc/pcr_host.hpp
@@ -700,6 +700,45 @@
 		if(cost4) *cost4 = c4;
 	}
 	return true;
+}
+
+inline void seed3_slice_walk_flat(const uint32_t *P, uint32_t ns, uint32_t per_wg, uint32_t G, uint32_t *start)
+{
+	uint32_t at = 0;
+	for(uint32_t w = 0;w <= G;++w){
+		const uint64_t target = (uint64_t)w*per_wg;
+		while(at + 1u < ns && P[at + 1u] <= target) ++at;
+		start[w] = at;
+	}
+}
+struct Seed3Rec { uint32_t off, n, first_seed, first_chunk; };
+inline void seed3_slice_walk(const Seed3Rec *recs, const uint32_t *const *runs, uint32_t n_rec, uint32_t per_wg, uint32_t G, uint32_t *start, uint32_t *start_rec = nullptr)
+{
+	uint32_t r = 0;
+	while(r < n_rec && recs[r].n == 0) ++r;
+	if(r == n_rec){ for(uint32_t w = 0;w <= G;++w){ start[w] = 0; if(start_rec) start_rec[w] = 0; } return; }
+	uint32_t nx = r + 1;
+	while(nx < n_rec && recs[nx].n == 0) ++nx;
+	uint32_t k = 0;
+	for(uint32_t w = 0;w <= G;++w){
+		const uint64_t target = (uint64_t)w*per_wg;
+		while(nx < n_rec && recs[nx].first_chunk <= target){
+			r = nx; k = 0;
+			do ++nx; while(nx < n_rec && recs[nx].n == 0);
+		}
+		const uint32_t *const run = runs[r];
+		uint32_t lo = k, hi = recs[r].n;
+		while(hi - lo > 1u){ const uint32_t mid = (lo + hi) >> 1; if((uint64_t)recs[r].first_chunk + run[mid] <= target) lo = mid; else hi = mid; }
+		k = lo;
+		start[w] = recs[r].first_seed + k;
+		if(start_rec) start_rec[w] = r;
+	}
+}
+inline uint32_t seed3_slice_cap(const uint32_t *start, uint32_t G, uint32_t ns)
+{
+	uint32_t cap = 2;
+	for(uint32_t w = 0;w < G;++w) cap = std::max(cap, std::min(start[w + 1] + 2u, ns + 1u) - start[w]);
+	return cap;
 }
 
 inline bool move_trials(const Planes &cur, int move, double max_degen, int primer_min, int primer_max, std::vector<Planes> &out)
diff --git a/pcramp_amd/csrc/pcr_scan_seed3.inc b/pcramp_amd/csrc/pcr_scan_seed3.inc
--- a/pcramp_amd/csrc/pcr_scan_seed3.inc
+++ b/pcramp_amd/csrc/pcr_scan_seed3.inc
@@ -37,6 +37,7 @@
 	const uint8_t *spans;
 	const uint4 *masks; const uint8_t *floors;
 	uint32_t n_seeds, n_or, or_base;
+	const uint4 *recs; const uint32_t *store;
 	const uint32_t *pix_first, *pix_last; const uint4 *pix_ent;
 	uint32_t n_chunks, per_wg, slice_cap;
 	uint32_t n_irr_wg;
@@ -44,6 +45,8 @@
 constexpr uint32_t S3_MAX_WG = 512;
 constexpr uint32_t S3_MAX_OR = 448, S3_MAX_SEEDS = 1u << 16;
 struct Seed3Slices { uint32_t start[S3_MAX_WG + 1]; };
+constexpr uint32_t S3_START_MASK = 0xFFFFu;
+static_assert(S3_MAX_SEEDS - 1u <= S3_START_MASK && S3_MAX_OR <= 0x10000u, "a seed index and a local orientation share one word of Seed3Slices");
 struct Seed3Set {
 	const uint32_t *valid, *blk_info, *blk_local; const uint8_t *active;
 };
@@ -71,12 +74,23 @@
 	blk_info[b] = v | (active[blk_seq[b]] ? 0u : BLK_INACTIVE);
 }
 
-__device__ __forceinline__ void s3_irregular(const Seed3Tables &T3, const Seed3Set &Q, const IrrArgs2 &IA, const uint4 *__restrict__ cand_fwd,
+__device__ __forceinline__ uint32_t s3_rec_of(const uint4 *recs, uint32_t n_or, uint32_t s)
+{
+	uint32_t lo = 0, hi = n_or;
+	while(hi - lo > 1u){ const uint32_t mid = (lo + hi) >> 1; if(recs[mid].z <= s) lo = mid; else hi = mid; }
+	return lo;
+}
+
+__device__ __forceinline__ void s3_irregular(const Seed3Tables &T3, const uint4 *recs, const Seed3Set &Q, const IrrArgs2 &IA, const uint4 *__restrict__ cand_fwd,
 	const uint32_t *__restrict__ cand_floor, HitSink sink, uint32_t gw, uint32_t n_gw, uint32_t lane)
 {
 	for(uint32_t i0 = gw*16u;i0 < T3.n_seeds;i0 += n_gw*16u){
 		const uint32_t i = i0 + lane;
-		const uint32_t sdv = (lane < 16u && i < T3.n_seeds) ? T3.seeds[i] : S2_END;
+		uint32_t sdv = S2_END;
+		if(lane < 16u && i < T3.n_seeds){
+			if(T3.recs){ const uint32_t r = s3_rec_of(recs, T3.n_or, i); const uint4 rc = recs[r]; sdv = T3.store[rc.x + (i - rc.z)] | r; }
+			else sdv = T3.seeds[i];
+		}
 		const uint32_t orient = T3.or_base + (sdv & 0x1FFu);
 		uint32_t first = 0, cnt = 0;
 		if(sdv != S2_END && !(orient & 1u)){
diff --git a/pcramp_amd/csrc/pcr_scan_seed3_pass.inc b/pcramp_amd/csrc/pcr_scan_seed3_pass.inc
--- a/pcramp_amd/csrc/pcr_scan_seed3_pass.inc
+++ b/pcramp_amd/csrc/pcr_scan_seed3_pass.inc
@@ -1,6 +1,7 @@
 	extern __shared__ uint4 s3_dyn[];
 	uint4 *const masks = s3_dyn;
-	uint32_t *const prefix = (uint32_t *)(masks + T3.n_or);
+	uint4 *const recs = masks + T3.n_or;
+	uint32_t *const prefix = (uint32_t *)(recs + (T3.recs ? T3.n_or : 0u));
 	uint32_t *const seeds = prefix + T3.slice_cap;
 	uint8_t *const floors = (uint8_t *)(seeds + T3.slice_cap);
 	uint8_t *const spans = floors + ((T3.n_or + 15u) & ~15u);
@@ -8,15 +9,40 @@
 	for(uint32_t i = blockIdx.x*S3_THREADS + threadIdx.x;i < Z.n0;i += gridDim.x*S3_THREADS) Z.z0[i] = make_uint4(0, 0, 0, 0);
 	for(uint32_t i = blockIdx.x*S3_THREADS + threadIdx.x;i < Z.n1;i += gridDim.x*S3_THREADS) Z.z1[i] = make_uint4(0, 0, 0, 0);
 	if(Z.ctrl && blockIdx.x == 0 && threadIdx.x == 0){ Z.ctrl[1] = 0; Z.ctrl[3] = 0; }
-	for(uint32_t i = threadIdx.x;i < T3.n_or;i += S3_THREADS){ masks[i] = T3.masks[i]; floors[i] = T3.floors[i]; }
+	const bool recs_lds = T3.recs && IA.ix_first;
+	for(uint32_t i = threadIdx.x;i < T3.n_or;i += S3_THREADS){ masks[i] = T3.masks[i]; floors[i] = T3.floors[i]; if(recs_lds) recs[i] = T3.recs[i]; }
 	constexpr uint32_t S3_WAVES = S3_THREADS/64;
 	if(blockIdx.x < T3.n_irr_wg){
-		if(IA.ix_first) s3_irregular(T3, Q, IA, cand_fwd, cand_floor, sink, blockIdx.x*S3_WAVES + wave, T3.n_irr_wg*S3_WAVES, lane);
+		if(IA.ix_first){
+			if(recs_lds) __syncthreads();
+			s3_irregular(T3, recs, Q, IA, cand_fwd, cand_floor, sink, blockIdx.x*S3_WAVES + wave, T3.n_irr_wg*S3_WAVES, lane);
+		}
 		return;
 	}
 	const uint32_t wg = blockIdx.x - T3.n_irr_wg, n_wg = gridDim.x - T3.n_irr_wg;
-	const uint32_t s_lo = W.start[wg];
-	const uint32_t n_slice = min(min(W.start[wg + 1] + 2u, T3.n_seeds + 1u) - s_lo, T3.slice_cap);
+	const uint32_t s_lo = W.start[wg] & S3_START_MASK, r_lo = W.start[wg] >> 16;
+	const uint32_t n_slice = min(min((W.start[wg + 1] & S3_START_MASK) + 2u, T3.n_seeds + 1u) - s_lo, T3.slice_cap);
+	if(T3.recs){
+		for(uint32_t i = threadIdx.x;i < n_slice;i += S3_THREADS){
+			const uint32_t s = s_lo + i;
+			uint32_t pv = T3.n_chunks, sv = 0u; uint8_t spv = 0;
+			if(s < T3.n_seeds){
+				const uint32_t r_max = T3.n_or - 1u;
+				const uint4 c0 = T3.recs[r_lo], c1 = T3.recs[min(r_lo + 1u, r_max)], c2 = T3.recs[min(r_lo + 2u, r_max)], c3 = T3.recs[min(r_lo + 3u, r_max)];
+				uint32_t r = r_lo; uint4 rc = c0;
+				if(c1.z <= s){ r = min(r_lo + 1u, r_max); rc = c1; }
+				if(c2.z <= s){ r = min(r_lo + 2u, r_max); rc = c2; }
+				if(c3.z <= s){
+					r = min(r_lo + 3u, r_max); rc = c3;
+					while(r < r_max){ const uint4 nx = T3.recs[r + 1u]; if(nx.z > s) break; ++r; rc = nx; }
+				}
+				const uint32_t *const blk = T3.store + rc.x; const uint32_t k = s - rc.z;
+				sv = blk[k] | r; pv = rc.w + blk[rc.y + k]; spv = ((const uint8_t *)(blk + 2u*rc.y))[k];
+			}
+			prefix[i] = pv; seeds[i] = sv; spans[i] = spv;
+		}
+	}
+	else
 	for(uint32_t i = threadIdx.x;i < n_slice;i += S3_THREADS){ prefix[i] = T3.chunk_prefix[s_lo + i]; const bool in = s_lo + i < T3.n_seeds; seeds[i] = in ? T3.seeds[s_lo + i] : 0u; spans[i] = in ? T3.spans[s_lo + i] : (uint8_t)0; }
 	__syncthreads();
 	const uint32_t gw = wg*S3_WAVES + wave, n_gw = n_wg*S3_WAVES;
@@ -76,4 +102,4 @@
 			else record_hit(sink, seq, c, make_key(seq, (int32_t)p_local, 1, 0, 0), cnt_b[b]);
 		}
 	}
-	if(IA.ix_first && T3.n_irr_wg == 0) s3_irregular(T3, Q, IA, cand_fwd, cand_floor, sink, gw, n_gw, lane);
+	if(IA.ix_first && T3.n_irr_wg == 0) s3_irregular(T3, recs, Q, IA, cand_fwd, cand_floor, sink, gw, n_gw, lane);
diff --git a/pcramp_amd/csrc/pcr_select.inc b/pcramp_amd/csrc/pcr_select.inc
--- a/pcramp_amd/csrc/pcr_select.inc
+++ b/pcramp_amd/csrc/pcr_select.inc
@@ -7,12 +7,37 @@
 	std::vector<uint32_t> s3_prefix;
 	std::vector<uint8_t> s3_spans;
 	std::vector<uint32_t> s1_seeds;
+	bool s3_res = false, s3_store_full = false;
+	uint32_t s3_n_seeds = 0;
+	std::vector<pcrhost::Seed3Rec> s3_recs; std::vector<const uint32_t *> s3_runs; std::vector<uint32_t> s3_group_chunks;
+	struct Upload { uint32_t off, bytes; size_t at; };
+	std::vector<Upload> s3_up; std::vector<uint8_t> s3_up_bytes;
 	void clear()
 	{
 		s2_seeds.clear(); s2_masks.clear(); s2_floors.clear(); s2_group_end.clear(); s2_group_offmask.clear(); s2_group_or.clear(); s2_group_nor.clear();
 		s3_launch.clear(); s3_prefix.clear(); s3_spans.clear(); s1_seeds.clear();
+		s3_res = s3_store_full = false; s3_n_seeds = 0; s3_recs.clear(); s3_runs.clear(); s3_group_chunks.clear(); s3_up.clear(); s3_up_bytes.clear();
 	}
 };
+
+int reset_s3_store(pcr_ctx *ctx, PlanLists &L)
+{
+	const int rc = flush_launcher(ctx);
+	if(rc != PCR_OK) return rc;
+	HIP_TRY(hipStreamSynchronize(ctx->stream));
+	ctx->s3_store_used = 0; ++ctx->s3_store_epoch; ++ctx->s3_store_resets;
+	ctx->s3_store_stale.store(false, std::memory_order_relaxed);
+	L.s3_up.clear(); L.s3_up_bytes.clear();
+	if(ctx->debug_log) fprintf(stderr, "[pcramp] seed store reset (epoch %u)\n", ctx->s3_store_epoch);
+	return PCR_OK;
+}
+void ship_s3_uploads(pcr_ctx *ctx, PlanLists &L)
+{
+	if(L.s3_up.empty()) return;
+	for(const PlanLists::Upload &u : L.s3_up) memcpy(ctx->s3_store.p + u.off, L.s3_up_bytes.data() + u.at, u.bytes);
+	__builtin_ia32_sfence();
+	L.s3_up.clear(); L.s3_up_bytes.clear();
+}
 
 inline uint32_t spread16(uint32_t v)
 {
@@ -23,7 +48,7 @@
 
 constexpr uint32_t S2_MAX_GROUPS = 4096;
 bool plan_seed2(pcr_ctx *ctx, PlanLists &L, const std::vector<pcrhost::Candidate> &cand, std::vector<uint32_t> &or_seed, std::vector<uint32_t> &or_plain, uint32_t &irr_off_mask,
-	const SeqSet *S3 = nullptr)
+	const SeqSet *S3 = nullptr, bool allow_res = true)
 {
 	std::vector<uint32_t> &pf = L.s3_prefix;
 	pf.clear();
@@ -34,6 +59,10 @@
 	irr_off_mask = 0;
 	L.s2_masks.resize(n_or);
 	if(ctx->s2_cache.size() > 16384) ctx->s2_cache.clear();
+	const bool res = S3 && allow_res && ctx->s3_store.p;
+	L.s3_res = res; L.s3_store_full = false; L.s3_recs.clear(); L.s3_runs.clear(); L.s3_group_chunks.clear();
+	if(res){ L.s3_recs.assign(n_or, pcrhost::Seed3Rec{0, 0, 0, 0}); L.s3_runs.assign(n_or, nullptr); }
+	size_t n_flat = 0;
 	size_t group_begin = 0; uint32_t group_mask = 0, group_or0 = 0, group_last = 0;
 	auto fits = [&](size_t n, uint32_t g_or){
 		if(S3) return g_or <= S3_MAX_OR && n <= S3_MAX_SEEDS;
@@ -45,7 +74,6 @@
 	};
 	std::vector<uint8_t> &spans = L.s3_spans;
 	spans.clear();
-	if(ctx->s3_cache.size() > 16384) ctx->s3_cache.clear();
 	for(uint32_t o = 0;o < n_or;++o){
 		const pcrhost::Candidate &c = cand[o >> 1];
 		const Planes &m = (o & 1u) ? c.rc : c.fwd;
@@ -83,18 +111,21 @@
 		L.s2_masks[o] = e.mask;
 		if(!e.seedable){ or_plain.push_back(o); continue; }
 		or_seed.push_back(o);
-		if(!fits(out.size() - group_begin + e.seeds.size(), o - group_or0 + 1)){
+		if(!fits(n_flat - group_begin + e.seeds.size(), o - group_or0 + 1)){
 			if(!fits(e.seeds.size(), 1) || L.s2_group_end.size() + 1 >= S2_MAX_GROUPS) return false;
-			L.s2_group_end.push_back((uint32_t)out.size()); L.s2_group_offmask.push_back(group_mask); L.s2_group_or.push_back(group_or0); L.s2_group_nor.push_back(group_last - group_or0 + 1);
-			group_begin = out.size(); group_mask = 0; group_or0 = o;
-			if(S3){ pf.push_back(pf_run); pf_run = 0; }
+			L.s2_group_end.push_back((uint32_t)n_flat); L.s2_group_offmask.push_back(group_mask); L.s2_group_or.push_back(group_or0); L.s2_group_nor.push_back(group_last - group_or0 + 1);
+			group_begin = n_flat; group_mask = 0; group_or0 = o;
+			if(res) L.s3_group_chunks.push_back(pf_run); else if(S3) pf.push_back(pf_run);
+			if(S3) pf_run = 0;
 		}
 		group_last = o;
-		const size_t at = out.size();
-		out.resize(at + e.seeds.size());
-		for(size_t k = 0;k < e.seeds.size();++k) out[at + k] = e.seeds[k] | (o - group_or0);
+		if(!res){
+			const size_t at = out.size();
+			out.resize(at + e.seeds.size());
+			for(size_t k = 0;k < e.seeds.size();++k) out[at + k] = e.seeds[k] | (o - group_or0);
+		}
 		if(S3){
-			spans.insert(spans.end(), e3->spans.begin(), e3->spans.end());
+			if(!res) spans.insert(spans.end(), e3->spans.begin(), e3->spans.end());
 			pcr_ctx::S3Chunks *ch = nullptr;
 			for(pcr_ctx::S3Chunks &x : e3->chunks){ if(x.gen == S3->pix_generation){ ch = &x; break; } }
 			if(!ch){
@@ -106,22 +137,43 @@
 					const uint32_t key4 = (e.seeds[k] >> 14) << 2, sp = e3->spans[k];
 					ch->run[k] = run; run += (start[key4 + (sp >> 2) + 1u] - start[key4 + (sp & 3u)] + 63u) >> 6;
 				}
-				ch->total = run; ch->gen = S3->pix_generation;
+				ch->total = run; ch->gen = S3->pix_generation; ch->blk_epoch = 0;
 			}
-			const size_t pa = pf.size();
-			pf.resize(pa + ch->run.size());
-			for(size_t k = 0;k < ch->run.size();++k) pf[pa + k] = pf_run + ch->run[k];
+			if(res){
+				const uint32_t n = (uint32_t)e.seeds.size();
+				if(n && ch->blk_epoch != ctx->s3_store_epoch){
+					const size_t bytes = 9*(size_t)n, room = (bytes + 127) & ~size_t(127);
+					if(ctx->s3_store_used + room > ctx->s3_store.cap){ L.s3_store_full = true; return false; }
+					ch->blk_off = (uint32_t)(ctx->s3_store_used/4); ch->blk_epoch = ctx->s3_store_epoch;
+					const size_t at = L.s3_up_bytes.size();
+					L.s3_up.push_back(PlanLists::Upload{(uint32_t)ctx->s3_store_used, (uint32_t)bytes, at});
+					ctx->s3_store_used += room;
+					L.s3_up_bytes.resize(at + bytes);
+					uint8_t *const b = L.s3_up_bytes.data() + at;
+					memcpy(b, e.seeds.data(), 4*(size_t)n); memcpy(b + 4*(size_t)n, ch->run.data(), 4*(size_t)n); memcpy(b + 8*(size_t)n, e3->spans.data(), n);
+				}
+				L.s3_recs[o] = pcrhost::Seed3Rec{ch->blk_off, n, (uint32_t)(n_flat - group_begin), pf_run};
+				L.s3_runs[o] = ch->run.data();
+			}
+			else{
+				const size_t pa = pf.size();
+				pf.resize(pa + ch->run.size());
+				for(size_t k = 0;k < ch->run.size();++k) pf[pa + k] = pf_run + ch->run[k];
+			}
 			pf_run += ch->total;
 		}
+		n_flat += e.seeds.size();
 		if(!(o & 1u)){ irr_off_mask |= e.off_mask; group_mask |= e.off_mask; }
 	}
-	L.s2_group_end.push_back((uint32_t)out.size()); L.s2_group_offmask.push_back(group_mask); L.s2_group_or.push_back(group_or0);
+	L.s2_group_end.push_back((uint32_t)n_flat); L.s2_group_offmask.push_back(group_mask); L.s2_group_or.push_back(group_or0);
 	L.s2_group_nor.push_back(or_seed.empty() ? 0u : group_last - group_or0 + 1);
-	if(S3) pf.push_back(pf_run);
+	if(res) L.s3_group_chunks.push_back(pf_run); else if(S3) pf.push_back(pf_run);
+	L.s3_n_seeds = (uint32_t)n_flat;
 	return true;
 }
 
 constexpr size_t S3_LDS_BUDGET = 120*1024;
+inline size_t seed3_lds_bound(uint32_t n_or, uint32_t slice_cap, bool res) { return (res ? 33 : 17)*(size_t)n_or + 9*(size_t)slice_cap + 64; }
 constexpr uint32_t S3_WG_THREADS = 1024;
 uint32_t seed3_grid(const pcr_ctx *ctx) { return std::min<uint32_t>(2*ctx->n_cu, S3_MAX_WG); }
 bool plan_seed3_slices(pcr_ctx *ctx, PlanLists &PL, bool with_irr)
@@ -132,22 +184,21 @@
 	for(size_t g = 0;g < PL.s2_group_end.size();++g){
 		const uint32_t ns = PL.s2_group_end[g] - (uint32_t)g_begin;
 		g_begin = PL.s2_group_end[g];
-		const uint32_t *P = PL.s3_prefix.data() + g_prefix;
+		const uint32_t *P = PL.s3_res ? nullptr : PL.s3_prefix.data() + g_prefix;
 		g_prefix += (size_t)ns + 1;
 		pcr_ctx::S3Launch &L = PL.s3_launch[g];
 		L.n_irr_wg = with_irr ? std::min<uint32_t>((ns + seeds_per_turn - 1u)/seeds_per_turn, G_all/4u) : 0u;
 		const uint32_t G = (G_all - L.n_irr_wg) & ~1u;
-		L.n_chunks = P[ns]; L.per_wg = std::max<uint32_t>(1u, (L.n_chunks + G - 1u)/G); L.slice_cap = 2;
+		L.n_chunks = PL.s3_res ? PL.s3_group_chunks[g] : P[ns]; L.per_wg = std::max<uint32_t>(1u, (L.n_chunks + G - 1u)/G); L.slice_cap = 2;
 		if(ns == 0) continue;
-		uint32_t at = 0;
-		for(uint32_t w = 0;w <= G;++w){
-			const uint64_t target = (uint64_t)w*L.per_wg;
-			while(at + 1u < ns && P[at + 1u] <= target) ++at;
-			L.W.start[w] = at;
-		}
-		for(uint32_t w = G + 1;w <= S3_MAX_WG;++w) L.W.start[w] = at;
-		for(uint32_t w = 0;w < G;++w) L.slice_cap = std::max(L.slice_cap, std::min(L.W.start[w + 1] + 2u, ns + 1u) - L.W.start[w]);
-		if(17*(size_t)PL.s2_group_nor[g] + 9*(size_t)L.slice_cap + 64 > S3_LDS_BUDGET) return false;
+		const uint32_t or0 = PL.s2_group_or[g];
+		uint32_t start_rec[S3_MAX_WG + 1];
+		if(PL.s3_res) pcrhost::seed3_slice_walk(PL.s3_recs.data() + or0, PL.s3_runs.data() + or0, PL.s2_group_nor[g], L.per_wg, G, L.W.start, start_rec);
+		else pcrhost::seed3_slice_walk_flat(P, ns, L.per_wg, G, L.W.start);
+		L.slice_cap = pcrhost::seed3_slice_cap(L.W.start, G, ns);
+		if(PL.s3_res){ for(uint32_t w = 0;w <= G;++w) L.W.start[w] |= start_rec[w] << 16; }
+		for(uint32_t w = G + 1;w <= S3_MAX_WG;++w) L.W.start[w] = L.W.start[G];
+		if(seed3_lds_bound(PL.s2_group_nor[g], L.slice_cap, PL.s3_res) > S3_LDS_BUDGET) return false;
 	}
 	return true;
 }
@@ -338,6 +389,21 @@
 }
 
 
+int prepare_s3_store(pcr_ctx *ctx, PlanLists &L, bool &res_ok)
+{
+	res_ok = false;
+	bool reset = ctx->s3_store_stale.load(std::memory_order_relaxed);
+	if(ctx->s3_cache.size() > 16384){ ctx->s3_cache.clear(); reset = true; }
+	if(!ctx->s3_resident || !ctx->direct_ok) return PCR_OK;
+	if(!ctx->s3_store.p){
+		const std::string err_before = g_err;
+		if(ctx->s3_store.ensure(ctx->s3_store_bytes) != PCR_OK){ (void)hipGetLastError(); g_err = err_before; ctx->s3_resident = false; return PCR_OK; }
+	}
+	if(reset && (ctx->s3_store_used != 0 || ctx->s3_store_stale.load(std::memory_order_relaxed))){ const int rc = reset_s3_store(ctx, L); if(rc != PCR_OK) return rc; }
+	res_ok = true;
+	return PCR_OK;
+}
+
 enum class ScanForm { Popcount, BitSliced, Seed1Host, Seed1Dev, Seed2, Seed3 };
 inline const char *form_name(ScanForm f)
 {
@@ -386,6 +452,7 @@
 	std::vector<uint32_t> &or_seed = P.or_seed, &or_plain = P.or_plain;
 	P.min_len = min_oligo_length; P.n_live = live_irregular(S, min_oligo_length);
 	int rc;
+	SubTimer sub(ctx);
 	const bool no_shifts = ctx->scan_version == 3 && !optimize_5 && !optimize_3;
 	const bool seed2_ok = no_shifts && !ctx->force_seed1 && n_or <= 65535;
 	bool want_seed3 = false;
@@ -404,8 +471,21 @@
 	}
 	bool use_seed2 = false;
 	if(seed2_ok){
-		use_seed2 = plan_seed2(ctx, L, cand, or_seed, or_plain, P.irr_off_mask, want_seed3 ? &S : nullptr);
-		if(want_seed3 && !(use_seed2 && or_plain.empty() && !or_seed.empty() && plan_seed3_slices(ctx, L, P.s3_with_irr))){
+		bool res_ok = false;
+		if(want_seed3 && (rc = prepare_s3_store(ctx, L, res_ok)) != PCR_OK) return rc;
+		use_seed2 = plan_seed2(ctx, L, cand, or_seed, or_plain, P.irr_off_mask, want_seed3 ? &S : nullptr, res_ok);
+		for(int again = 0;L.s3_store_full && again < 2;++again){
+			or_seed.clear(); or_plain.clear();
+			if(again == 0 && (rc = reset_s3_store(ctx, L)) != PCR_OK) return rc;
+			use_seed2 = plan_seed2(ctx, L, cand, or_seed, or_plain, P.irr_off_mask, &S, again == 0);
+		}
+		bool sliced = false;
+		if(want_seed3){
+			sub.lap(1);
+			sliced = use_seed2 && or_plain.empty() && !or_seed.empty() && plan_seed3_slices(ctx, L, P.s3_with_irr);
+			sub.lap(2);
+		}
+		if(want_seed3 && !sliced){
 			or_seed.clear(); or_plain.clear();
 			use_seed2 = plan_seed2(ctx, L, cand, or_seed, or_plain, P.irr_off_mask, nullptr);
 		}
@@ -413,8 +493,9 @@
 		if(!use_seed2){ or_seed.clear(); or_plain.clear(); P.irr_off_mask = 0; }
 	}
 	const bool use_seed3 = use_seed2 && want_seed3 && or_plain.empty() && !or_seed.empty()
-		&& L.s3_prefix.size() == L.s2_seeds.size() + L.s2_group_end.size() && L.s3_spans.size() == L.s2_seeds.size();
-	if(use_seed2){ P.form = use_seed3 ? ScanForm::Seed3 : ScanForm::Seed2; P.n_seeds = L.s2_seeds.size(); }
+		&& (L.s3_res ? L.s3_group_chunks.size() == L.s2_group_end.size() && L.s3_recs.size() == n_or
+		             : L.s3_prefix.size() == L.s2_seeds.size() + L.s2_group_end.size() && L.s3_spans.size() == L.s2_seeds.size());
+	if(use_seed2){ P.form = use_seed3 ? ScanForm::Seed3 : ScanForm::Seed2; P.n_seeds = L.s3_n_seeds; }
 	else if(no_shifts && !ctx->host_seed_tables && n_or <= S1_MAX_OR){
 		plan_seed1(ctx, L, cand, or_seed, or_plain, P.irr_off_mask);
 		P.form = ScanForm::Seed1Dev; P.n_seeds = L.s1_seeds.size();
@@ -432,6 +513,7 @@
 	if(or_seed.empty() && P.form != ScanForm::Popcount) P.form = ScanForm::BitSliced;
 	P.need_plain = (ctx->scan_version != 1) && !or_plain.empty();
 	P.need_seedset = !or_seed.empty() && S.n_degen_tiles > 0;
+	sub.lap(1);
 	return PCR_OK;
 }
 
@@ -457,6 +539,7 @@
 	SeedTables ST = {};
 	Seed2Tables ST2 = {};
 	const uint32_t *d_s3_prefix = nullptr; const uint8_t *d_s3_spans = nullptr;
+	const uint4 *d_s3_recs = nullptr;
 	Scan2Staged plain, seedset;
 	bool lean = false, fuse = false;
 	size_t bits_bytes = 0;
@@ -511,7 +594,7 @@
 	bytes += (H.image.size() + H.heads.size() + H.multi.size() + 64)*sizeof(uint32_t);
 	if(seed2){
 		bytes += L.s2_masks.size()*sizeof(uint4) + L.s2_floors.size() + L.s2_seeds.size()*sizeof(uint32_t) + 512;
-		if(seed3) bytes += L.s3_prefix.size()*sizeof(uint32_t) + L.s3_spans.size() + 128;
+		if(seed3) bytes += L.s3_prefix.size()*sizeof(uint32_t) + L.s3_spans.size() + L.s3_recs.size()*sizeof(pcrhost::Seed3Rec) + 128;
 	}
 	if(build_tables) bytes += L.s1_seeds.size()*sizeof(uint32_t) + 256;
 	T.bits_bytes = J.bits_bytes; T.fuse = J.fuse;
@@ -543,15 +626,19 @@
 		T.ST.image = ctx->s1_image.p; T.ST.heads = ctx->s1_heads.p; T.ST.multi = ctx->s1_multi.p; T.ST.flat = 1;
 	}
 	if(seed2){
-		T.ST2.seeds = st.put(L.s2_seeds.data(), L.s2_seeds.size());
+		const bool res = seed3 && L.s3_res;
+		static_assert(sizeof(pcrhost::Seed3Rec) == sizeof(uint4), "a record is read as one uint4");
+		T.ST2.seeds = res ? nullptr : st.put(L.s2_seeds.data(), L.s2_seeds.size());
 		T.ST2.masks = st.put(L.s2_masks.data(), L.s2_masks.size());
 		T.ST2.floors = st.put(L.s2_floors.data(), L.s2_floors.size());
-		T.ST2.n_seeds = (uint32_t)L.s2_seeds.size(); T.ST2.n_or = n_or;
-		if(seed3){ T.d_s3_prefix = st.put(L.s3_prefix.data(), L.s3_prefix.size()); T.d_s3_spans = st.put(L.s3_spans.data(), L.s3_spans.size()); }
+		T.ST2.n_seeds = L.s3_n_seeds; T.ST2.n_or = n_or;
+		if(res) T.d_s3_recs = (const uint4 *)st.put(L.s3_recs.data(), L.s3_recs.size());
+		else if(seed3){ T.d_s3_prefix = st.put(L.s3_prefix.data(), L.s3_prefix.size()); T.d_s3_spans = st.put(L.s3_spans.data(), L.s3_spans.size()); }
 	}
 	const size_t ctrl_bytes = (8 + 2*(size_t)S.n)*sizeof(uint32_t);
 	if(T.fuse){
 		fa->d_oligos = st.put(J.ol.data(), J.ol.size());
+		if(ctx->debug_log) fprintf(stderr, "[pcramp] staged %zu bytes (%s lists)\n", st.used, (seed3 && L.s3_res) ? "resident" : "flat");
 		fa->staged = true;
 		if(T.lean) st.seal(guard_seq);
 		else if((rc = st.ship(S.ctrl.p, ctrl_bytes, fa->d_fr, T.bits_bytes, fa->d_rf, T.bits_bytes, guard_seq)) != PCR_OK) return rc;
@@ -601,9 +688,11 @@
 	return PCR_OK;
 }
 
-void seed3_args(SeqSet &S, const Seed2Tables &Tg, const uint32_t *d_chunk_prefix, const uint8_t *d_spans, const pcr_ctx::S3Launch &L3, const IrrArgs2 &IA, Seed3Tables &T3, Seed3Set &Q3)
+void seed3_args(SeqSet &S, const Seed2Tables &Tg, const uint32_t *d_chunk_prefix, const uint8_t *d_spans, const uint4 *d_recs, const uint8_t *store,
+	const pcr_ctx::S3Launch &L3, const IrrArgs2 &IA, Seed3Tables &T3, Seed3Set &Q3)
 {
 	T3.seeds = Tg.seeds; T3.spans = d_spans; T3.chunk_prefix = d_chunk_prefix; T3.masks = Tg.masks; T3.floors = Tg.floors;
+	T3.recs = d_recs; T3.store = (const uint32_t *)store;
 	T3.n_seeds = Tg.n_seeds; T3.n_or = Tg.n_or; T3.or_base = Tg.or_base;
 	T3.pix_first = S.pix_first.p; T3.pix_last = S.pix_last.p; T3.pix_ent = S.pix_ent.p;
 	Q3 = Seed3Set{ S.valid_d(), S.blk_info.p, S.blk_local.p, S.d_active.p };
@@ -612,14 +701,14 @@
 }
 inline size_t seed3_lds(const Seed3Tables &T3)
 {
-	return (size_t)T3.n_or*sizeof(uint4) + 2*(size_t)T3.slice_cap*sizeof(uint32_t) + (((size_t)T3.n_or + 15) & ~size_t(15)) + (((size_t)T3.slice_cap + 15) & ~size_t(15)) + 16;
-}
-
-int launch_seed3_group(pcr_ctx *ctx, SeqSet &S, const Seed2Tables &Tg, const uint32_t *d_chunk_prefix, const uint8_t *d_spans, const pcr_ctx::S3Launch &L3, const IrrArgs2 &IA,
-	const HitSink &sink, const S2Clear &Z)
+	return (size_t)T3.n_or*sizeof(uint4)*(T3.recs ? 2 : 1) + 2*(size_t)T3.slice_cap*sizeof(uint32_t) + (((size_t)T3.n_or + 15) & ~size_t(15)) + (((size_t)T3.slice_cap + 15) & ~size_t(15)) + 16;
+}
+
+int launch_seed3_group(pcr_ctx *ctx, SeqSet &S, const Seed2Tables &Tg, const uint32_t *d_chunk_prefix, const uint8_t *d_spans, const uint4 *d_recs, const pcr_ctx::S3Launch &L3,
+	const IrrArgs2 &IA, const HitSink &sink, const S2Clear &Z)
 {
 	Seed3Tables T3; Seed3Set Q3;
-	seed3_args(S, Tg, d_chunk_prefix, d_spans, L3, IA, T3, Q3);
+	seed3_args(S, Tg, d_chunk_prefix, d_spans, d_recs, ctx->s3_store.p, L3, IA, T3, Q3);
 	const size_t dyn3 = seed3_lds(T3);
 	if(!ctx->s3_attr_set){
 		HIP_TRY(hipFuncSetAttribute((const void *)k_seed3<S3_WG_THREADS>, hipFuncAttributeMaxDynamicSharedMemorySize, 128*1024));
@@ -676,8 +765,9 @@
 	for(size_t g = 0;g < L.s2_group_end.size();++g){
 		Seed2Tables Tg = T.ST2;
 		const uint32_t or0 = L.s2_group_or[g], g_or = L.s2_group_nor[g];
-		const uint8_t *const d_spans = seed3 ? T.d_s3_spans + g_begin : nullptr;
-		Tg.seeds = T.ST2.seeds + g_begin; Tg.n_seeds = L.s2_group_end[g] - g_begin;
+		const bool res = seed3 && T.d_s3_recs;
+		const uint8_t *const d_spans = (seed3 && !res) ? T.d_s3_spans + g_begin : nullptr;
+		Tg.seeds = res ? nullptr : T.ST2.seeds + g_begin; Tg.n_seeds = L.s2_group_end[g] - g_begin;
 		Tg.masks = T.ST2.masks + (size_t)or0; Tg.floors = T.ST2.floors + or0; Tg.n_or = g_or; Tg.or_base = or0;
 		g_begin = L.s2_group_end[g];
 		if(Tg.n_seeds == 0){ g_prefix += 1u; continue; }
@@ -687,7 +777,7 @@
 			or0, or0 + g_or - 1, g + 1, L.s2_group_end.size(), sizeof(S2Shared), dyn);
 		const S2Clear Z = group_clear(T, fa, sink, first_launch);
 		if(seed3){
-			if((rc = launch_seed3_group(ctx, S, Tg, T.d_s3_prefix + g_prefix, d_spans, L.s3_launch[g], IA, sink, Z)) != PCR_OK) return rc;
+			if((rc = launch_seed3_group(ctx, S, Tg, res ? nullptr : T.d_s3_prefix + g_prefix, d_spans, res ? T.d_s3_recs + or0 : nullptr, L.s3_launch[g], IA, sink, Z)) != PCR_OK) return rc;
 			g_prefix += Tg.n_seeds + 1u;
 		}
 		else hipLaunchKernelGGL(k_seed2_of_ctx, sgrid, sblock, dyn, ctx->stream, S.tb_d(), S.valid_d(), S.tile_desc.p, S.n_tiles, Tg, S.d_active.p, ctx->d_cand_fwd, ctx->d_cand_floor,
@@ -821,14 +911,19 @@
 	SeqSet &S = ctx->sets[J.which];
 	HostTimer timer(ctx, 0);
 	if(ctx->timing) ++ctx->n_timed;
+	SubTimer sub(ctx);
 	pcrhost::build_candidates((const uint64_t *)pairs, n_pairs, J.opt5 != 0, J.opt3 != 0, J.thr, J.cand);
+	sub.lap(0);
 	const uint32_t ncand = (uint32_t)J.cand.size();
 	if(S.n == 0 || ncand == 0) return PCR_OK;
 	int rc;
 	if((rc = choose_scan_form(ctx, S, J.cand, J.opt5, J.opt3, J.min_len, J.P, J.L)) != PCR_OK) return rc;
 	if(ctx->debug_log) fprintf(stderr, "[pcramp] scan plan: form=%s, %u candidates, %zu seeded orientations (%zu seeds), %zu plain, %u/%u IUPAC tiles, %u-slot buckets\n",
 		form_name(J.P.form), ncand, J.P.or_seed.size(), J.P.n_seeds, J.P.or_plain.size(), S.n_degen_tiles, S.n_tiles, S.bucket_cap);
+	if(ctx->debug_log && J.P.form == ScanForm::Seed3) fprintf(stderr, "[pcramp] seed lists: %s, %zu blocks to upload, store epoch %u\n", J.L.s3_res ? "resident" : "flat", J.L.s3_up.size(), ctx->s3_store_epoch);
+	sub.restart();
 	prepare_tables(S, J, J.has_fa ? &J.fa : nullptr);
+	sub.lap(3);
 	return PCR_OK;
 }
 
@@ -904,6 +999,7 @@
 	if(S.n == 0 || ncand == 0){ S.have_db = true; S.n_touched = 0; return PCR_OK; }
 	HostTimer timer(ctx, 1);
 	int rc;
+	ship_s3_uploads(ctx, J.L);
 	StagedTables T;
 	if((rc = stage_pass(ctx, J, ctrl_was_clean, T)) != PCR_OK) return rc;
 
@@ -957,9 +1053,9 @@
 	for(uint32_t w = 0;w <= Gh;++w) st[w] = L3.W.start[2*w];
 	for(uint32_t w = Gh + 1;w <= S3_MAX_WG/2;++w) st[w] = st[Gh];
 	uint32_t cap = 2;
-	for(uint32_t w = 0;w < Gh;++w) cap = std::max(cap, std::min(st[w + 1] + 2u, ns + 1u) - st[w]);
+	for(uint32_t w = 0;w < Gh;++w) cap = std::max(cap, std::min((st[w + 1] & S3_START_MASK) + 2u, ns + 1u) - (st[w] & S3_START_MASK));
 	J.pair_slice_cap = cap;
-	return 17*(size_t)J.L.s2_group_nor[0] + 9*(size_t)cap + 64 <= S3_LDS_BUDGET;
+	return seed3_lds_bound(J.L.s2_group_nor[0], cap, J.L.s3_res) <= S3_LDS_BUDGET;
 }
 
 bool passes_can_pair(PassJob &A, PassJob &B)
@@ -977,6 +1073,7 @@
 	const bool ctrl_was_clean = begin_pass(S);
 	int rc;
 	HostTimer timer(ctx, 1);
+	ship_s3_uploads(ctx, J.L);
 	if((rc = stage_pass(ctx, J, ctrl_was_clean, H.T)) != PCR_OK) return rc;
 	timer.next(2);
 	if((rc = size_attempt(ctx, S, J, 0, H.sink)) != PCR_OK) return rc;
@@ -987,7 +1084,7 @@
 	Tg.n_seeds = L.s2_group_end[0]; Tg.masks = H.T.ST2.masks + (size_t)L.s2_group_or[0]; Tg.floors = H.T.ST2.floors + L.s2_group_or[0];
 	Tg.n_or = L.s2_group_nor[0]; Tg.or_base = L.s2_group_or[0];
 	H.scan.IA = group_irr_args(S, J.P, L.s2_group_offmask[0], true, J.P.s3_with_irr);
-	seed3_args(S, Tg, H.T.d_s3_prefix, H.T.d_s3_spans, L.s3_launch[0], H.scan.IA, H.scan.T3, H.scan.Q);
+	seed3_args(S, Tg, H.T.d_s3_prefix, H.T.d_s3_spans, H.T.d_s3_recs ? H.T.d_s3_recs + L.s2_group_or[0] : nullptr, ctx->s3_store.p, L.s3_launch[0], H.scan.IA, H.scan.T3, H.scan.Q);
 	H.scan.T3.per_wg *= 2u; H.scan.T3.slice_cap = J.pair_slice_cap; H.scan.T3.n_irr_wg = (H.scan.T3.n_irr_wg + 1u)/2u;
 	H.scan.cand_fwd = ctx->d_cand_fwd; H.scan.cand_floor = ctx->d_cand_floor; H.scan.sink = H.sink;
 	H.scan.Z = group_clear(H.T, &J.fa, H.sink, true);
@@ -1050,6 +1147,7 @@
 	J.ctrl_was_clean = begin_pass(ctx->sets[which]); J.begun = true;
 	int rc = plan_pass(ctx, J, pairs, n_pairs);
 	if(rc == PCR_OK) rc = run_pass(ctx, J, n_entries_out);
+	if(!J.L.s3_up.empty()) ctx->s3_store_stale.store(true, std::memory_order_relaxed);
 	if(fa){ const pcr_amplify_args *a = fa->a; *fa = J.fa; fa->a = a; }
 	return rc;
 }
@@ -1102,6 +1200,7 @@
 }
 void release_job(pcr_ctx *ctx, PassJob *J)
 {
+	if(!J->L.s3_up.empty()) ctx->s3_store_stale.store(true, std::memory_order_relaxed);
 	J->reset();
 	std::lock_guard<std::mutex> lk(ctx->job_m);
 	ctx->job_free.push_back(J);
@@ -1251,6 +1350,7 @@
 		J->ctrl_was_clean = begin_pass(S); J->begun = true;
 	}
 	rc = plan_pass(ctx, *J, pairs, n_pairs);
+	SubTimer sub(ctx);
 	if(rc == PCR_OK && !inline_pass && !pass_is_pipelinable(ctx, *J)){
 		inline_pass = true;
 		rc = flush_launcher(ctx);
@@ -1261,6 +1361,7 @@
 		return rc;
 	}
 	pcr_ctx::Pending p;
+	if(!ctx->pairs_spare.empty()){ p.pairs.swap(ctx->pairs_spare.back()); ctx->pairs_spare.pop_back(); }
 	p.which = (int)which; p.pairs.assign(pairs, pairs + n_pairs); p.opt5 = optimize_5; p.opt3 = optimize_3;
 	p.thr = select_threshold; p.min_len = min_oligo_length; p.args = *args; p.d_fr = d_bits_fr; p.d_rf = d_bits_rf;
 	if(!inline_pass){
@@ -1270,6 +1371,7 @@
 		ctx->pending.push_back(std::move(p));
 		++ctx->n_pipelined;
 		L->q.push(&ctx->lq_client, J, J->seq);
+		sub.lap(4);
 		return PCR_OK;
 	}
 	assert(ctx->lq_client.queued.load() == 0);
@@ -1313,7 +1415,8 @@
 		}
 		break;
 	}
-	return PCR_OK;
-}
-
-}
+	for(pcr_ctx::Pending &q : pend){ if(ctx->pairs_spare.size() < 64) ctx->pairs_spare.push_back(std::move(q.pairs)); }
+	return PCR_OK;
+}
+
+}
```

Measured after the change: 26.04 billion. Within noise of the previous version (-0.9%).
